# Xjh-UCAS/TAM-TR

Measured on AMD Instinct MI355X. Metric: images/sec fwd+bwd @640x640 bs=16/GPU, higher is better.
Workload: dtype bf16

## Files before the change

include/tamtr_hip.h:

```cpp
#ifndef TAMTR_HIP_H
#define TAMTR_HIP_H

#include <stdint.h>

#ifdef __cplusplus
extern "C" {
#endif

#define TAMTR_F32 0
#define TAMTR_BF16 1

#define TAMTR_OK 0
#define TAMTR_EINVAL (-1)
#define TAMTR_EUNSUP (-2)
#define TAMTR_ELAUNCH (-3)

int tamtr_abi_version(void);

int tamtr_maxsigmoid_gate_fwd(const void* x, const float* gk, const float* bias, const void* v, void* out, float* aw,
                              int32_t* arg, int B, int nh, int hc, int HW, int T, float scale, int dtype, void* stream);

int tamtr_maxsigmoid_gate_bwd(const void* dout, const void* x, const float* gk, const void* v, const float* aw,
                              const int32_t* arg, void* dx, void* dv, float* dlogit, int B, int nh, int hc, int HW, int T,
                              float scale, int dtype, void* stream);
int tamtr_maxsigmoid_gate_cl_fwd(const void* e, long long ld_e, const float* mean_rstd_e, const float* gamma_e, const float* beta_e,
                                 const void* v, const float* mean_rstd_v, const float* gamma_v, const float* beta_v, const float* gk,
                                 const float* bias, void* out, float* aw, int32_t* arg, int B, int nh, int hc, int HW, int T, float scale,
                                 int dtype, void* stream);

int tamtr_conv3x3_tiles(int B, int H, int W);
int tamtr_conv3x3_pack_weight(const void* w, void* wpk, int C1, int C2, int dtype, void* stream);
int tamtr_conv3x3_cl_stats_fwd(const void* x, long long ld_x, const void* wpk, void* y, float* running_mean, float* running_var,
                               float* mean_rstd, float* partials, int B, int H, int W, int C1, int C2, float eps, float momentum,
                               void* stream);
int tamtr_bn_finalize(const float* partials, float* mean_rstd, float* running_mean, float* running_var, int C, int S, float eps,
                      float momentum, void* stream);

int tamtr_msdeform_attn_fwd(const void* value, const int32_t* shapes_host, const float* loc, const float* aw, void* out,
                            int B, int L, int M, int D, int Q, int nl, int P, int dtype, void* stream);

int tamtr_msdeform_attn_bwd(const void* gout, const void* value, const int32_t* shapes_host, const float* loc,
                            const float* aw, float* gvalue, float* gloc, float* gaw, int B, int L, int M, int D, int Q,
                            int nl, int P, int dtype, void* stream);

int tamtr_msdeform_attn_bwd_sorted(const void* gout, const void* value, const int32_t* shapes_host, const float* loc,
                                   const float* aw, void* gvalue, float* gloc, float* gaw, float* colw, int B, int L, int M,
                                   int D, int Q, int nl, int P, long long ldg, int dtype, void* stream);

int tamtr_contrastive_logits_fwd(const void* x, const float* w, const float* logit_scale, const float* bias, float* logits,
                                 float* xinv, float* winv, int B, int Q, int K, int C, int dtype, void* stream);

int tamtr_contrastive_bwd_slabs(int Q);
int tamtr_contrastive_logits_bwd(const float* g, const void* x, const float* w, const float* logit_scale, const float* xinv,
                                 const float* winv, void* dx, float* dwhat, int B, int Q, int K, int C, int dtype,
                                 void* stream);

int tamtr_linear_bf16(const void* X, const void* W, const float* bias, void* Y, int M, int N, int K, void* stream);

int tamtr_selfattn_fwd(const void* q, const void* k, const void* v, const uint32_t* mask_bits, void* o, float* lse, int B,
                       int Q, int nh, int dh, int ldq, int ldk, int ldv, int dtype, void* stream);
int tamtr_selfattn_bwd(const void* go, const void* q, const void* k, const void* v, const void* o, const float* lse,
                       const uint32_t* mask_bits, void* gq, void* gk, void* gv, float* delta_ws, int B, int Q, int nh, int dh,
                       int ldq, int ldk, int ldv, int dtype, void* stream);

int tamtr_selective_scan_chunk(void);
int tamtr_selective_scan_fwd(const float* u, const float* delta, const float* A, const float* Bm, const float* Cm,
                             const float* D, const float* dbias, float* y, float* hstate, int B, int K, int Dk, int N, int L,
                             int xmode, void* stream);
int tamtr_selective_scan_bwd_slabs(int Dk);
int tamtr_selective_scan_row_sums(void);
int tamtr_selective_scan_bwd(const float* gy, const float* u, const float* delta, const float* A, const float* Bm,
                             const float* Cm, const float* D, const float* dbias, const float* hstate, float* gu,
                             float* gdelta, float* grow, float* gB, float* gC, float* ws, int B, int K, int Dk, int N, int L,
                             int xmode, void* stream);

int tamtr_selective_scan_dtproj_fwd(const void* u, const float* dtr, const float* Wdt, const float* A, const float* Bm,
                                    const float* Cm, const float* D, const float* dbias, void* y, float* hstate, int B, int K,
                                    int Dk, int N, int R, int L, int xmode, int planes_bf16, void* stream);
int tamtr_selective_scan_dtproj_bwd(const void* gy, const void* u, const float* dtr, const float* Wdt, const float* A,
                                    const float* Bm, const float* Cm, const float* D, const float* dbias, const float* hstate,
                                    void* gu, void* gdelta_ws, float* gdtr, float* grow, float* gB, float* gC, float* ws, int B,
                                    int K, int Dk, int N, int R, int L, int xmode, int bf16_flags, void* stream);

int tamtr_lsap_assign(const float* cost, const int32_t* group_sizes_host, int bs, int nq, int G, int64_t* batch_idx,
                      int64_t* query_idx, int64_t* gt_idx, void* stream);

int tamtr_cpam_fwd(const void* x, const void* p, void* out, float* s2, int32_t* arg, int B, int C, int H, int W, int dtype,
                   void* stream);

int tamtr_cpam_bwd(const void* gout, const void* x, const void* p, const float* s2, const int32_t* arg, void* dx_direct,
                   void* du_ws, void* dp, int B, int C, int H, int W, int dtype, void* stream);

int tamtr_cpam_cl_fwd(const void* x, void* p, uint8_t* code, void* out, float* s2, int32_t* arg, int B, int C, int H, int W, int dtype, void* stream);
int tamtr_cpam_cl_bwd(const void* gout, const void* x, const void* p, const uint8_t* code, const float* s2, const int32_t* arg, void* dxd_ws,
                      void* du_ws, void* dp_ws, void* dx, int B, int C, int H, int W, int dtype, void* stream);

int tamtr_dwconv_silu_cross_fwd(const void* x, long long x_pixel_stride, const float* weight, const float* bias, void* u2, int B,
                                int D, int H, int W, int dtype, int plane_dtype, void* stream);
int tamtr_dwconv_tiles(int H, int W);
int tamtr_dwconv_silu_cross_bwd(const void* g2, const void* x, long long x_pixel_stride, const float* weight, const float* bias,
                                void* gx, long long gx_pixel_stride, float* ws, int B, int D, int H, int W, int dtype, int plane_dtype,
                                void* stream);

int tamtr_cross_merge_fwd(const void* y4, float* ymT, int B, int D, int H, int W, int plane_dtype, void* stream);
int tamtr_cross_merge_bwd(const float* gymT, void* g2, int B, int D, int H, int W, int plane_dtype, void* stream);

int tamtr_ln_gate_blocks(long long ntok);
int tamtr_ln_gate_fwd(const float* x, const void* xz, long long xz_token_stride, const float* gamma, const float* beta, void* out,
                      float* stats, long long ntok, int D, float eps, int dtype, void* stream);
int tamtr_ln_gate_bwd(const void* gout, const float* x, const void* xz, long long xz_token_stride, const float* gamma,
                      const float* beta, const float* stats, float* gx, void* gxz, float* partials, long long ntok, int D, int dtype,
                      void* stream);

int tamtr_sum_n(const void* const* src, int n, void* out, long long n_elems, int dtype, void* stream);

int tamtr_colsum_blocks(long long M);
int tamtr_colsum_bf16(const void* X, float* partial, long long M, int N, void* stream);
int tamtr_slab_sum_rows(const void* in, float* out, int R, long long C, int dtype, void* stream);
int tamtr_fold_add(const float* g4, const void* m0, const void* m1, float* out, int B, long long n, int dtype, void* stream);

int tamtr_layernorm_fwd(const void* x, const float* gamma, const float* beta, void* out, float* stats, long long ntok, int D,
                        float eps, int dtype, void* stream);
int tamtr_layernorm_bwd(const void* gout, const void* x, const float* gamma, const float* stats, void* gx, float* partials,
                        long long ntok, int D, int dtype, void* stream);

int tamtr_bn_slices(int B, int HW);
int tamtr_bn_act_fwd(const void* x, const float* gamma, const float* beta, float* running_mean, float* running_var, void* y,
                     float* mean_rstd, float* partials, int B, int C, int HW, float eps, float momentum, int act, int dtype, void* stream);
int tamtr_bn_act_bwd(const void* gy, const void* x, const float* gamma, const float* beta, const float* mean_rstd, void* gx,
                     float* ggamma, float* gbeta, float* partials, int B, int C, int HW, int act, int dtype, void* stream);

int tamtr_bncl_blocks(long long N, int C, int dtype);
int tamtr_bncl_act_fwd(const void* x, const float* gamma, const float* beta, float* running_mean, float* running_var, const void* residual,
                       void* y, float* mean_rstd, float* partials, long long N, int C, float eps, float momentum, int act, int dtype,
                       void* stream);
int tamtr_bncl_stats(const void* x, float* running_mean, float* running_var, float* mean_rstd, float* partials, long long N, int C, float eps,
                     float momentum, int dtype, void* stream);
int tamtr_bncl2_act_fwd(const void* x1, const float* gamma1, const float* beta1, float* running_mean1, float* running_var1, const void* x2,
                        const float* gamma2, const float* beta2, float* running_mean2, float* running_var2, void* y, float* mean_rstd,
                        float* partials, long long N, int C, float eps, float momentum, int act, int dtype, void* stream);
int tamtr_bncl2_act_bwd(const void* gy, long long ldgy, const void* x1, const void* x2, const float* gamma1, const float* beta1,
                        const float* gamma2, const float* beta2, const float* mean_rstd, void* gx1, void* gx2, float* ggamma1, float* gbeta1,
                        float* ggamma2, float* gbeta2, float* partials, long long N, int C, int act, int dtype, void* stream);
int tamtr_bncl_act_bwd(const void* gy, long long ldgy, const void* x, const float* gamma, const float* beta, const float* mean_rstd,
                       void* gx, float* ggamma, float* gbeta, float* partials, long long N, int C, int act, int dtype, void* stream);

int tamtr_relayout(const void* src, void* dst, int B, int C, int HW, int ld, int to_nhwc, int dtype, void* stream);
int tamtr_resample2(const void* src, void* dst, int B, int H, int W, int C, int mode, int dtype, void* stream);
int tamtr_copy_rows(const void* src, long long lds, void* dst, long long ldd, long long N, int C, int dtype, void* stream);
int tamtr_cat_rows(const void* const* src, const long long* lds, const int* C, int n, void* dst, long long ldd, long long N, int dtype,
                   void* stream);

int tamtr_maxpool_out(int n, int k, int s, int p);
int tamtr_maxpool_fwd(const void* x, void* y, uint8_t* code, int B, int C, int H, int W, int k, int s, int p, int nhwc, int dtype,
                      void* stream);
int tamtr_maxpool_bwd(const void* gy, const uint8_t* code, const void* addend, void* gx, int B, int C, int H, int W, int k, int s, int p, int nhwc, int dtype,
                      void* stream);

int tamtr_img_augment_u8(const uint8_t* src, const double* inv_affine, const uint8_t* luts, const int32_t* flags, float* out, int B,
                         int SH, int SW, int H, int W, int border, void* stream);

int tamtr_optim_chunk(void);
int tamtr_optim_step(const void* const* p, const void* const* m, const void* const* v, const void* const* e, const void* const* shadow, float* step,
                     const long long* numel,
                     const unsigned char* group, const int* chunk_tensor, const long long* chunk_off, const void* const* grads, int ntensors,
                     int nchunks, float* partial, float* normcoef, const float* lr, const float* wd, int ngroups, float beta1, float beta2, float eps,
                     float max_norm, float ema_decay, int do_ema, void* stream);

int tamtr_xproj_dw_slices(int L);
int tamtr_xproj_fwd(const void* u2, const void* wcat, float* dtr, float* Bs, float* Cs, int B, int D, int L, int R, int plane_dtype, void* stream);
int tamtr_xproj_bwd_dx(const void* gu, const float* gdtr, const float* gB, const float* gC, const void* wT, void* gu2, int B, int D, int L, int R,
                       int plane_dtype, void* stream);
int tamtr_xproj_bwd_dw(const void* u2, const float* gdtr, const float* gB, const float* gC, float* part, int B, int D, int L, int R, int plane_dtype,
                       void* stream);

int tamtr_detr_blocks(int rows_per_layer);
int tamtr_detr_layers_fwd(const float* pb, const float* ps, const float* gt_bboxes, const long long* gt_cls, const long long* li, const long long* bi,
                          const long long* si, const long long* gi, int Lr, int B, int nq, int nc, int n, long long* tgt, float* score, float* pair_l1,
                          float* pair_riou, float* partial, float g_class, float g_bbox, float g_giou, float* out, void* stream);
int tamtr_detr_layers_bwd(const float* pb, const float* ps, const float* gt_bboxes, const long long* li, const long long* bi, const long long* si,
                          const long long* gi, const long long* tgt, const float* score, const float* up, int Lr, int B, int nq, int nc, int n,
                          float g_class, float g_bbox, float g_giou, float* gpb, float* gps, void* stream);
int tamtr_detr_match_cost(const float* ps, const float* pb, const float* gt_bboxes, const long long* gt_cls, long long rows, int nc, int G, float g_class,
                          float g_bbox, float g_giou, float alpha, float gamma, float* C, void* stream);

int tamtr_bncl_act_seg_fwd(const void* x, const float* gamma, const float* beta, float* running_mean, float* running_var, void* y, long long seg_rows,
                           long long seg_pitch, float* mean_rstd, float* partials, long long N, int C, float eps, float momentum, int act, int dtype,
                           void* stream);
int tamtr_bncl_act_seg_bwd(const void* gy, long long seg_rows, long long seg_pitch, const void* x, const float* gamma, const float* beta,
                           const float* mean_rstd, void* gx, float* ggamma, float* gbeta, float* partials, long long N, int C, int act, int dtype,
                           void* stream);

int tamtr_box_refine_fwd(const float* delta, const float* ref, float* out, long long n, void* stream);
int tamtr_box_refine_bwd(const float* gout, const float* out, const float* ref, float* gdelta, float* gref, long long n, void* stream);

int tamtr_graph_capture_census(void* stream, int* counts, int n_types);

int tamtr_detect_postprocess(const void* preds, int dtype, int B, int nq, int nd, const int32_t* orig_hw, float conf, float iou,
                             int single_cls, float max_wh, const int32_t* classes, int n_classes, float* out, int32_t* keep,
                             int32_t* counts, void* stream);

int tamtr_val_postprocess_match(const void* preds, int dtype, int B, int nq, int nd, float imgsz, float conf, float iou, int single_cls,
                                float max_wh, const float* lab_cls, const float* lab_box, const int32_t* lab_off, int M, const float* scale,
                                float* predn, uint8_t* correct, int32_t* counts, void* stream);

#ifdef __cplusplus
}
#endif
#endif
```

tam-tr_amd/_lib.py:

```python
import ctypes
import os
from ctypes import c_float, c_int, c_longlong, c_void_p

_HERE = os.path.dirname(os.path.abspath(__file__))
LIB_PATH = os.environ.get('TAMTR_HIP_LIB') or os.path.join(_HERE, 'csrc', 'libtamtr_hip.so')
ABI_VERSION = 36

F32, BF16 = 0, 1
_ERR = {-1: 'TAMTR_EINVAL (bad argument)', -2: 'TAMTR_EUNSUP (shape/dtype outside what the kernels are built for)',
        -3: 'TAMTR_ELAUNCH (HIP launch error)'}


class TamtrHipError(RuntimeError):
    pass


_P, _I, _F, _LL = c_void_p, c_int, c_float, c_longlong
_SIGS = {
    'tamtr_abi_version': [],
    'tamtr_maxsigmoid_gate_fwd': [_P, _P, _P, _P, _P, _P, _P, _I, _I, _I, _I, _I, _F, _I, _P],
    'tamtr_maxsigmoid_gate_bwd': [_P, _P, _P, _P, _P, _P, _P, _P, _P, _I, _I, _I, _I, _I, _F, _I, _P],
    'tamtr_msdeform_attn_fwd': [_P, _P, _P, _P, _P, _I, _I, _I, _I, _I, _I, _I, _I, _P],
    'tamtr_msdeform_attn_bwd': [_P, _P, _P, _P, _P, _P, _P, _P, _I, _I, _I, _I, _I, _I, _I, _I, _P],
    'tamtr_msdeform_attn_bwd_sorted': [_P, _P, _P, _P, _P, _P, _P, _P, _P, _I, _I, _I, _I, _I, _I, _I, _LL, _I, _P],
    'tamtr_contrastive_logits_fwd': [_P, _P, _P, _P, _P, _P, _P, _I, _I, _I, _I, _I, _P],
    'tamtr_contrastive_logits_bwd': [_P, _P, _P, _P, _P, _P, _P, _P, _I, _I, _I, _I, _I, _P],
    'tamtr_contrastive_bwd_slabs': [_I],
    'tamtr_linear_bf16': [_P, _P, _P, _P, _I, _I, _I, _P],
    'tamtr_selfattn_fwd': [_P, _P, _P, _P, _P, _P, _I, _I, _I, _I, _I, _I, _I, _I, _P],
    'tamtr_selfattn_bwd': [_P] * 11 + [_I, _I, _I, _I, _I, _I, _I, _I, _P],
    'tamtr_selective_scan_chunk': [],
    'tamtr_selective_scan_fwd': [_P, _P, _P, _P, _P, _P, _P, _P, _P, _I, _I, _I, _I, _I, _I, _P],
    'tamtr_selective_scan_bwd_slabs': [_I],
    'tamtr_selective_scan_row_sums': [],
    'tamtr_selective_scan_bwd': [_P] * 15 + [_I, _I, _I, _I, _I, _I, _P],
    'tamtr_selective_scan_dtproj_fwd': [_P] * 10 + [_I] * 8 + [_P],
    'tamtr_selective_scan_dtproj_bwd': [_P] * 17 + [_I] * 8 + [_P],
    'tamtr_lsap_assign': [_P, _P, _I, _I, _I, _P, _P, _P, _P],
    'tamtr_img_augment_u8': [_P, _P, _P, _P, _P, _I, _I, _I, _I, _I, _I, _P],
    'tamtr_cpam_fwd': [_P, _P, _P, _P, _P, _I, _I, _I, _I, _I, _P],
    'tamtr_cpam_cl_fwd': [_P, _P, _P, _P, _P, _P, _I, _I, _I, _I, _I, _P],
    'tamtr_cpam_bwd': [_P] * 8 + [_I, _I, _I, _I, _I, _P],
    'tamtr_cpam_cl_bwd': [_P] * 10 + [_I, _I, _I, _I, _I, _P],
    'tamtr_dwconv_silu_cross_fwd': [_P, _LL, _P, _P, _P, _I, _I, _I, _I, _I, _I, _P],
    'tamtr_dwconv_tiles': [_I, _I],
    'tamtr_cross_merge_fwd': [_P, _P, _I, _I, _I, _I, _I, _P],
    'tamtr_cross_merge_bwd': [_P, _P, _I, _I, _I, _I, _I, _P],
    'tamtr_ln_gate_blocks': [_LL],
    'tamtr_bn_slices': [_I, _I],
    'tamtr_maxpool_out': [_I, _I, _I, _I],
    'tamtr_maxpool_fwd': [_P, _P, _P, _I, _I, _I, _I, _I, _I, _I, _I, _I, _P],
    'tamtr_maxpool_bwd': [_P, _P, _P, _P, _I, _I, _I, _I, _I, _I, _I, _I, _I, _P],
    'tamtr_sum_n': [_P, _I, _P, _LL, _I, _P],
    'tamtr_colsum_blocks': [_LL],
    'tamtr_colsum_bf16': [_P, _P, _LL, _I, _P],
    'tamtr_fold_add': [_P, _P, _P, _P, _I, _LL, _I, _P],
    'tamtr_slab_sum_rows': [_P, _P, _I, _LL, _I, _P],
    'tamtr_graph_capture_census': [_P, _P, _I],
    'tamtr_box_refine_fwd': [_P, _P, _P, _LL, _P],
    'tamtr_box_refine_bwd': [_P, _P, _P, _P, _P, _LL, _P],
    'tamtr_bncl_act_seg_fwd': [_P, _P, _P, _P, _P, _P, _LL, _LL, _P, _P, _LL, _I, _F, _F, _I, _I, _P],
    'tamtr_bncl_act_seg_bwd': [_P, _LL, _LL, _P, _P, _P, _P, _P, _P, _P, _P, _LL, _I, _I, _I, _P],
    'tamtr_detr_blocks': [_I],
    'tamtr_detr_layers_fwd': [_P] * 8 + [_I] * 5 + [_P] * 5 + [_F, _F, _F, _P, _P],
    'tamtr_detr_layers_bwd': [_P] * 10 + [_I] * 5 + [_F, _F, _F, _P, _P, _P],
    'tamtr_detr_match_cost': [_P, _P, _P, _P, _LL, _I, _I, _F, _F, _F, _F, _F, _P, _P],
    'tamtr_xproj_dw_slices': [_I],
    'tamtr_xproj_fwd': [_P, _P, _P, _P, _P, _I, _I, _I, _I, _I, _P],
    'tamtr_xproj_bwd_dx': [_P, _P, _P, _P, _P, _P, _I, _I, _I, _I, _I, _P],
    'tamtr_xproj_bwd_dw': [_P, _P, _P, _P, _P, _I, _I, _I, _I, _I, _P],
    'tamtr_optim_chunk': [],
    'tamtr_optim_step': [_P] * 11 + [_I, _I, _P, _P, _P, _P, _I, _F, _F, _F, _F, _F, _I, _P],
    'tamtr_resample2': [_P, _P, _I, _I, _I, _I, _I, _I, _P],
    'tamtr_cat_rows': [_P, _P, _P, _I, _P, _LL, _LL, _I, _P],
    'tamtr_copy_rows': [_P, _LL, _P, _LL, _LL, _I, _I, _P],
    'tamtr_relayout': [_P, _P, _I, _I, _I, _I, _I, _I, _P],
    'tamtr_bncl_blocks': [_LL, _I, _I],
    'tamtr_bncl_act_fwd': [_P, _P, _P, _P, _P, _P, _P, _P, _P, _LL, _I, _F, _F, _I, _I, _P],
    'tamtr_bncl_stats': [_P, _P, _P, _P, _P, _LL, _I, _F, _F, _I, _P],
    'tamtr_bn_finalize': [_P, _P, _P, _P, _I, _I, _F, _F, _P],
    'tamtr_conv3x3_tiles': [_I, _I, _I],
    'tamtr_conv3x3_pack_weight': [_P, _P, _I, _I, _I, _P],
    'tamtr_conv3x3_cl_stats_fwd': [_P, _LL, _P, _P, _P, _P, _P, _P, _I, _I, _I, _I, _I, _F, _F, _P],
    'tamtr_maxsigmoid_gate_cl_fwd': [_P, _LL, _P, _P, _P, _P, _P, _P, _P, _P, _P, _P, _P, _P, _I, _I, _I, _I, _I, _F, _I, _P],
    'tamtr_bncl2_act_fwd': [_P, _P, _P, _P, _P, _P, _P, _P, _P, _P, _P, _P, _P, _LL, _I, _F, _F, _I, _I, _P],
    'tamtr_bncl2_act_bwd': [_P, _LL, _P, _P, _P, _P, _P, _P, _P, _P, _P, _P, _P, _P, _P, _P, _LL, _I, _I, _I, _P],
    'tamtr_bncl_act_bwd': [_P, _LL, _P, _P, _P, _P, _P, _P, _P, _P, _LL, _I, _I, _I, _P],
    'tamtr_bn_act_fwd': [_P, _P, _P, _P, _P, _P, _P, _P, _I, _I, _I, _F, _F, _I, _I, _P],
    'tamtr_bn_act_bwd': [_P, _P, _P, _P, _P, _P, _P, _P, _P, _I, _I, _I, _I, _I, _P],
    'tamtr_layernorm_fwd': [_P, _P, _P, _P, _P, _LL, _I, _F, _I, _P],
    'tamtr_layernorm_bwd': [_P, _P, _P, _P, _P, _P, _LL, _I, _I, _P],
    'tamtr_ln_gate_fwd': [_P, _P, _LL, _P, _P, _P, _P, _LL, _I, _F, _I, _P],
    'tamtr_ln_gate_bwd': [_P, _P, _P, _LL, _P, _P, _P, _P, _P, _P, _LL, _I, _I, _P],
    'tamtr_dwconv_silu_cross_bwd': [_P, _P, _LL, _P, _P, _P, _LL, _P, _I, _I, _I, _I, _I, _I, _P],
    'tamtr_detect_postprocess': [_P, _I, _I, _I, _I, _P, _F, _F, _I, _F, _P, _I, _P, _P, _P, _P],
    'tamtr_val_postprocess_match': [_P, _I, _I, _I, _I, _F, _F, _F, _I, _F, _P, _P, _P, _I, _P, _P, _P, _P, _P],
}
EXPORTS = tuple(_SIGS)
_lib = None


def lib():
    global _lib
    if _lib is None:
        if not os.path.exists(LIB_PATH):
            raise TamtrHipError(f'{LIB_PATH} not found: build it with `python -c "import __graft_entry__ as g; g.build()"` '
                                '(hipcc --offload-arch=gfx950). There is no CPU fallback.')
        h = ctypes.CDLL(LIB_PATH)
        for name, args in _SIGS.items():
            fn = getattr(h, name)
            fn.argtypes = args
            fn.restype = c_int
        if h.tamtr_abi_version() != ABI_VERSION:
            raise TamtrHipError(f'libtamtr_hip.so ABI {h.tamtr_abi_version()} != expected {ABI_VERSION}: rebuild')
        _lib = h
    return _lib


def call(name, *args):
    rc = getattr(lib(), name)(*args)
    if rc != 0:
        raise TamtrHipError(f'{name} failed: {_ERR.get(rc, rc)}')


def require_gpu(*tensors):
    for t in tensors:
        if t is not None and not t.is_cuda:
            raise TamtrHipError('TAM-TR HIP ops need tensors resident on an MI355X (got a CPU tensor); there is no CPU fallback')


def dtype_code(t):
    import torch
    if t.dtype == torch.float32:
        return F32
    if t.dtype == torch.bfloat16:
        return BF16
    raise TamtrHipError(f'unsupported activation dtype {t.dtype} (float32 and bfloat16 kernels are built)')


def stream_ptr():
    import torch
    return c_void_p(torch.cuda.current_stream().cuda_stream)


def ptr(t):
    return c_void_p(t.data_ptr()) if t is not None else c_void_p(0)
```

tam-tr_amd/backbone.py:

```python
import torch
import torch.nn as nn
import torch.nn.functional as F

def _conv(conv, x):
    if x.is_cuda:
        from . import ops
        return ops.conv2d_module(conv, x)
    return conv(x)


BN_EPS, BN_MOMENTUM = 1e-3, 0.03


def batchnorm(c):
    return nn.BatchNorm2d(c, eps=BN_EPS, momentum=BN_MOMENTUM)


def fold_bn(conv, bn):
    fused = nn.Conv2d(conv.in_channels, conv.out_channels, conv.kernel_size, conv.stride, conv.padding, conv.dilation, conv.groups,
                      bias=True).requires_grad_(False).to(conv.weight.device)
    with torch.no_grad():
        scale = bn.weight.div(torch.sqrt(bn.eps + bn.running_var))
        fused.weight.copy_((scale[:, None] * conv.weight.reshape(conv.out_channels, -1)).view(fused.weight.shape))
        b = torch.zeros(conv.out_channels, device=conv.weight.device) if conv.bias is None else conv.bias
        fused.bias.copy_(scale * b + (bn.bias - bn.weight.mul(bn.running_mean).div(torch.sqrt(bn.running_var + bn.eps))))
    return fused


class Conv(nn.Module):

    def __init__(self, c1, c2, k=1, s=1, p=None, g=1, d=1, act=True):
        super().__init__()
        if p is None:
            p = (d * (k - 1) + 1) // 2 if d > 1 else k // 2
        self.conv = nn.Conv2d(c1, c2, k, s, p, dilation=d, groups=g, bias=False)
        self.bn = batchnorm(c2)
        self.act = nn.SiLU() if act is True else act if isinstance(act, nn.Module) else nn.Identity()

    def fuse(self):
        if 'bn' in self._modules:
            self.conv = fold_bn(self.conv, self.bn)
            del self.bn

    def fusable(self, y):
        return ('bn' in self._modules and y.is_cuda and self.bn.training and self.bn.affine and type(self.act) in (nn.SiLU, nn.Identity)
                and y.dtype in (torch.bfloat16, torch.float32))

    def forward(self, x, residual=None):
        return self.post(_conv(self.conv, x), residual)

    def post(self, y, residual=None):
        if 'bn' not in self._modules:
            y = self.act(y)
            return y if residual is None else y + residual
        if self.fusable(y):
            from . import ops
            if ops.is_cl(y) and ops.bn_cl_ok(y.shape[1], y.dtype):
                B, C, H, W = y.shape
                res = None
                if residual is not None and ops.is_cl(residual) and residual.shape == y.shape:
                    res, residual = residual.permute(0, 2, 3, 1).reshape(B * H * W, C), None
                o = ops.bn_act(y.permute(0, 2, 3, 1).reshape(B * H * W, C), self.bn, isinstance(self.act, nn.SiLU), res)
                o = o.view(B, H, W, C).permute(0, 3, 1, 2)
                return o if residual is None else o + residual
            y = ops.bn_act(y, self.bn, isinstance(self.act, nn.SiLU))
        else:
            y = self.act(self.bn(y))
        return y if residual is None else y + residual


class RepConvN(nn.Module):

    def __init__(self, c1, c2, k=3, s=1, p=1, g=1, d=1, act=True, bn=False, deploy=False):
        super().__init__()
        assert k == 3 and p == 1
        self.conv1 = Conv(c1, c2, 3, s, p=1, g=g, act=False)
        self.conv2 = Conv(c1, c2, 1, s, p=0, g=g, act=False)
        self.act = nn.SiLU() if act is True else act if isinstance(act, nn.Module) else nn.Identity()

    def forward(self, x):
        if 'conv' in self._modules:
            return self.act(self.conv(x))
        c1, c2 = self.conv1, self.conv2
        if x.is_cuda and type(self.act) in (nn.SiLU, nn.Identity) and 'bn' in c1._modules and 'bn' in c2._modules:
            from . import ops
            y1, y2 = c1.conv(x), _conv(c2.conv, x)
            if (c1.fusable(y1) and c2.fusable(y2) and ops.is_cl(y1) and ops.is_cl(y2) and ops.bn_cl_ok(y1.shape[1], y1.dtype)
                    and c1.bn.track_running_stats and c2.bn.track_running_stats and c1.bn.eps == c2.bn.eps and c1.bn.momentum == c2.bn.momentum):
                B, C, H, W = y1.shape
                o = ops.bn2_act(y1.permute(0, 2, 3, 1).reshape(B * H * W, C), c1.bn, y2.permute(0, 2, 3, 1).reshape(B * H * W, C), c2.bn,
                                isinstance(self.act, nn.SiLU))
                return o.view(B, H, W, C).permute(0, 3, 1, 2)
            return self.act(c1.post(y1) + c2.post(y2))
        return self.act(self.conv1(x) + self.conv2(x))

    @staticmethod
    def _branch(branch):
        bn = branch.bn
        std = (bn.running_var + bn.eps).sqrt()
        return branch.conv.weight * (bn.weight / std).reshape(-1, 1, 1, 1), bn.bias - bn.running_mean * bn.weight / std

    def switch_to_deploy(self):
        if 'conv' in self._modules:
            return
        with torch.no_grad():
            (k3, b3), (k1, b1) = self._branch(self.conv1), self._branch(self.conv2)
            c = self.conv1.conv
            self.conv = nn.Conv2d(c.in_channels, c.out_channels, c.kernel_size, c.stride, c.padding, c.dilation, c.groups,
                                  bias=True).requires_grad_(False).to(c.weight.device)
            self.conv.weight.copy_(k3 + F.pad(k1, [1, 1, 1, 1]))
            self.conv.bias.copy_(b3 + b1)
        del self.conv1, self.conv2


class RepNBottleneck(nn.Module):
    def __init__(self, c1, c2, shortcut=True, g=1, k=(3, 3), e=0.5):
        super().__init__()
        c_ = int(c2 * e)
        self.cv1 = RepConvN(c1, c_, k[0], 1)
        self.cv2 = Conv(c_, c2, k[1], 1, g=g)
        self.add = shortcut and c1 == c2

    def forward(self, x):
        if self.add:
            return self.cv2(self.cv1(x), residual=x)
        return self.cv2(self.cv1(x))


class RepNCSP(nn.Module):
    def __init__(self, c1, c2, n=1, shortcut=True, g=1, e=0.5):
        super().__init__()
        c_ = int(c2 * e)
        self.cv1, self.cv2 = Conv(c1, c_, 1, 1), Conv(c1, c_, 1, 1)
        self.cv3 = Conv(2 * c_, c2, 1)
        self.m = nn.Sequential(*(RepNBottleneck(c_, c_, shortcut, g, e=1.0) for _ in range(n)))

    def forward(self, x):
        from . import ops
        return self.cv3(ops.cat_channels((self.m(self.cv1(x)), self.cv2(x))))


class RepNCSPELAN4(nn.Module):

    def __init__(self, c1, c2, c3, c4, c5=1):
        super().__init__()
        self.c = c3 // 2
        self.cv1 = Conv(c1, c3, 1, 1)
        self.cv2 = nn.Sequential(RepNCSP(c3 // 2, c4, c5), Conv(c4, c4, 3, 1))
        self.cv3 = nn.Sequential(RepNCSP(c4, c4, c5), Conv(c4, c4, 3, 1))
        self.cv4 = Conv(c3 + 2 * c4, c2, 1, 1)

    def branches(self, x):
        from . import ops
        y = list(ops.chunk2_channels(self.cv1(x)))
        y.append(self.cv2(ops.pack_channels(y[-1])))
        y.append(self.cv3(y[-1]))
        return y

    def forward(self, x):
        from . import ops
        return self.cv4(ops.cat_channels(self.branches(x)))


class SPPELAN(nn.Module):
    def __init__(self, c1, c2, c3):
        super().__init__()
        self.c = c3
        self.cv1 = Conv(c1, c3, 1, 1)
        self.cv5 = Conv(4 * c3, c2, 1, 1)

    def forward(self, x):
        from . import ops
        y = [self.cv1(x)]
        for _ in range(3):
            y.append(ops.max_pool2d(y[-1], 5, 1, 2) if y[-1].is_cuda else F.max_pool2d(y[-1], 5, 1, 2))
        return self.cv5(ops.cat_channels(y))


class CPAM(nn.Module):

    def __init__(self, c1, c2=None):
        super().__init__()

    def forward(self, x):
        from . import ops
        return ops.cpam(x)


class Upsample(nn.Upsample):

    def forward(self, x):
        if self.mode == 'nearest' and x.dim() == 4 and self.size is None and isinstance(self.scale_factor, (int, float)):
            if x.is_cuda and self.scale_factor in (0.5, 2.0):
                from . import ops
                y = ops.resample2(x, self.scale_factor == 2.0)
                if y is not None:
                    return y
            if self.scale_factor == 0.5 and x.shape[2] % 2 == 0 and x.shape[3] % 2 == 0:
                return x[..., ::2, ::2]
            if self.scale_factor == 2.0:
                B, C, H, W = x.shape
                if not x.is_contiguous() and x.is_contiguous(memory_format=torch.channels_last):
                    y = x.permute(0, 2, 3, 1)[:, :, None, :, None, :].expand(B, H, 2, W, 2, C).reshape(B, 2 * H, 2 * W, C)
                    return y.permute(0, 3, 1, 2)
                return x[:, :, :, None, :, None].expand(B, C, H, 2, W, 2).reshape(B, C, 2 * H, 2 * W)
        return super().forward(x)


class Concat(nn.Module):
    def __init__(self, dimension=1):
        super().__init__()
        self.d = dimension

    def forward(self, x):
        if self.d == 1:
            from . import ops
            return ops.cat_channels(x)
        return torch.cat(x, self.d)
```

tam-tr_amd/csrc/bn.hip:

```cpp
#include "common.h"

namespace {

constexpr int BN_THREADS = 256;
constexpr int BN_EPT = 16;
constexpr int BN_SLICE = BN_THREADS * BN_EPT;

template <typename T>
__device__ __forceinline__ void ld_slice(const T* __restrict__ p, int n, bool vec, float (&v)[BN_EPT], int (&cnt)) {
  const int base = threadIdx.x * BN_EPT;
  cnt = max(0, min(BN_EPT, n - base));
  if (vec && cnt == BN_EPT) {
#pragma unroll
    for (int q = 0; q < BN_EPT / 4; ++q) {
      float o[4];
      Elt<T>::ld4(p + base + 4 * q, o);
      v[4 * q] = o[0]; v[4 * q + 1] = o[1]; v[4 * q + 2] = o[2]; v[4 * q + 3] = o[3];
    }
  } else {
#pragma unroll
    for (int i = 0; i < BN_EPT; ++i) v[i] = i < cnt ? Elt<T>::ld(p + base + i) : 0.f;
  }
}

// ... 143 lines not shown
  const int n = min(BN_SLICE, HW - s * BN_SLICE);
  const size_t off = ((size_t)b * C + c) * HW + (size_t)s * BN_SLICE;
  const float mean = mean_rstd[2 * c], rstd = mean_rstd[2 * c + 1], g = gamma[c], be = beta[c];
  float xv[BN_EPT], gv[BN_EPT];
  int cnt;
  ld_slice<T>(x + off, n, vec, xv, cnt);
  ld_slice<T>(gy + off, n, vec, gv, cnt);
  float s1 = 0.f, s2 = 0.f;
#pragma unroll
  for (int i = 0; i < BN_EPT; ++i) {
    if (i < cnt) {
      const float xh = (xv[i] - mean) * rstd;
      const float dz = gv[i] * act_bwd(fmaf(xh, g, be), act);
      s1 += dz;
      s2 = fmaf(dz, xh, s2);
    }
  }
  s1 = block_sum(s1, s_red);
  s2 = block_sum(s2, s_red);
  if (threadIdx.x == 0) {
    float* o = part + ((size_t)c * S + (size_t)b * gridDim.x + s) * 2;
    o[0] = s1; o[1] = s2;
  }
}

template <typename T>
__global__ __launch_bounds__(BN_THREADS) void bn_bwd_apply_kernel(const T* __restrict__ gy, const T* __restrict__ x,
                                                                   const float* __restrict__ mean_rstd, const float* __restrict__ gamma,
                                                                   const float* __restrict__ beta, const float* __restrict__ part,
                                                                   T* __restrict__ gx, float* __restrict__ ggamma, float* __restrict__ gbeta,
                                                                   int C, int HW, int vec, int act, float inv_count) {
  __shared__ float s_red[BN_THREADS / WAVE];
  const int s = blockIdx.x, c = blockIdx.y, b = blockIdx.z, S = gridDim.x * gridDim.z;
  float p1 = 0.f, p2 = 0.f;
  for (int i = threadIdx.x; i < S; i += BN_THREADS) { p1 += part[((size_t)c * S + i) * 2]; p2 += part[((size_t)c * S + i) * 2 + 1]; }
  const float sum_dz = block_sum(p1, s_red), sum_dzx = block_sum(p2, s_red);
  if (s == 0 && b == 0 && threadIdx.x == 0) { ggamma[c] = sum_dzx; gbeta[c] = sum_dz; }
  const int n = min(BN_SLICE, HW - s * BN_SLICE);
  const size_t off = ((size_t)b * C + c) * HW + (size_t)s * BN_SLICE;
  const float mean = mean_rstd[2 * c], rstd = mean_rstd[2 * c + 1], g = gamma[c], be = beta[c];
  const float k1 = sum_dz * inv_count, k2 = sum_dzx * inv_count, gr = g * rstd;
  const int base = threadIdx.x * BN_EPT;
  const int cnt = max(0, min(BN_EPT, n - base));
  if (vec && cnt == BN_EPT) {
#pragma unroll
    for (int q = 0; q < BN_EPT / 4; ++q) {
      float xv[4], gv[4], o[4];
      Elt<T>::ld4(x + off + base + 4 * q, xv);
      Elt<T>::ld4(gy + off + base + 4 * q, gv);
#pragma unroll
      for (int i = 0; i < 4; ++i) {
        const float xh = (xv[i] - mean) * rstd;
        const float dz = gv[i] * act_bwd(fmaf(xh, g, be), act);
        o[i] = gr * (dz - k1 - xh * k2);
      }
      Elt<T>::st4(gx + off + base + 4 * q, o);
    }
  } else {
    for (int i = 0; i < cnt; ++i) {
      const float xh = (Elt<T>::ld(x + off + base + i) - mean) * rstd;
      const float dz = Elt<T>::ld(gy + off + base + i) * act_bwd(fmaf(xh, g, be), act);
      Elt<T>::st(gx + off + base + i, gr * (dz - k1 - xh * k2));
    }
  }
}

template <typename T, int V>
struct Vec;
template <>
struct Vec<float, 4> {
  static __device__ __forceinline__ void ld(const float* p, float (&o)[4]) { Elt<float>::ld4(p, o); }
  static __device__ __forceinline__ void st(float* p, const float (&v)[4]) { Elt<float>::st4(p, v); }
};
template <>
struct Vec<bf16_t, 4> {
  static __device__ __forceinline__ void ld(const bf16_t* p, float (&o)[4]) { Elt<bf16_t>::ld4(p, o); }
  static __device__ __forceinline__ void st(bf16_t* p, const float (&v)[4]) { Elt<bf16_t>::st4(p, v); }
};
template <>
struct Vec<bf16_t, 8> {
  static __device__ __forceinline__ void ld(const bf16_t* p, float (&o)[8]) {
    const uint4 t = *reinterpret_cast<const uint4*>(p);
    const uint32_t w[4] = {t.x, t.y, t.z, t.w};
#pragma unroll
    for (int i = 0; i < 4; ++i) { o[2 * i] = __uint_as_float(w[i] << 16); o[2 * i + 1] = __uint_as_float(w[i] & 0xffff0000u); }
  }
  static __device__ __forceinline__ void st(bf16_t* p, const float (&v)[8]) {
    uint32_t w[4];
#pragma unroll
    for (int i = 0; i < 4; ++i) w[i] = (uint32_t)f2bf(v[2 * i]) | ((uint32_t)f2bf(v[2 * i + 1]) << 16);
    *reinterpret_cast<uint4*>(p) = make_uint4(w[0], w[1], w[2], w[3]);
  }
};

constexpr int CL_UNROLL = 4;

template <int W>
__device__ __forceinline__ void fold_row_lanes(const float (&mine)[W], float* s_acc, float* s_col, int cg) {
#pragma unroll
  for (int j = 0; j < W; ++j) s_acc[threadIdx.x * W + j] = mine[j];
  __syncthreads();
  const int rl = BN_THREADS / cg;
  for (int o = threadIdx.x; o < cg * W; o += BN_THREADS) {
    const int g = o / W, j = o % W;
    float a = 0.f;
    for (int q = 0; q < rl; ++q) a += s_acc[(q * cg + g) * W + j];
    s_col[o] = a;
  }
  __syncthreads();
}

struct Seg { unsigned rows; size_t pitch; };
__device__ __forceinline__ size_t seg_addr(size_t e, int C, int cshift, size_t ld, Seg sg) {
  const size_t row = e >> cshift, col = e & (size_t)(C - 1);
  if (!sg.rows) return row * ld + col;
  const unsigned img = (unsigned)row / sg.rows;
  return (size_t)img * sg.pitch + ((unsigned)row - img * sg.rows) * ld + col;
}

template <typename T, int V>
__global__ __launch_bounds__(BN_THREADS) void bncl_stats_kernel(const T* __restrict__ x, float* __restrict__ part, size_t total, int C,
                                                                 int iters) {
  __shared__ float s_acc[BN_THREADS * 2 * V];
  __shared__ float s_col[2 * 1024];
  const size_t piece = (size_t)BN_THREADS * V, start = (size_t)blockIdx.x * iters * piece, end = min(total, start + iters * piece);
  const int cg = C / V, g = threadIdx.x % cg, S = gridDim.x;
  const T* home = x + start + (size_t)g * V;
  float k[V], acc[2 * V];
  Vec<T, V>::ld(home, k);
#pragma unroll
  for (int j = 0; j < 2 * V; ++j) acc[j] = 0.f;
  const size_t e0 = start + (size_t)threadIdx.x * V;
  for (int it = 0; it < iters; it += CL_UNROLL) {
    float v[CL_UNROLL][V];
#pragma unroll
    for (int u = 0; u < CL_UNROLL; ++u) {
      const size_t e = e0 + (size_t)(it + u) * piece;
      Vec<T, V>::ld(e < end ? x + e : home, v[u]);
    }
#pragma unroll
    for (int u = 0; u < CL_UNROLL; ++u)
#pragma unroll
      for (int j = 0; j < V; ++j) { const float d = v[u][j] - k[j]; acc[j] += d; acc[V + j] = fmaf(d, d, acc[V + j]); }
  }
  fold_row_lanes<2 * V>(acc, s_acc, s_col, cg);
  const float n = (float)((end - start) / C);
  for (int c = threadIdx.x; c < C; c += BN_THREADS) {
    const float s1 = s_col[(c / V) * 2 * V + c % V], s2 = s_col[(c / V) * 2 * V + V + c % V], m = s1 / n;
    float* o = part + ((size_t)c * S + blockIdx.x) * 3;
    o[0] = n; o[1] = Elt<T>::ld(x + start + c) + m; o[2] = s2 - s1 * m;
  }
}

template <typename T, int V>
__global__ __launch_bounds__(BN_THREADS) void bncl_apply_kernel(const T* __restrict__ x, const float* __restrict__ mean_rstd,
                                                                 const float* __restrict__ gamma, const float* __restrict__ beta,
                                                                 const T* __restrict__ res, T* __restrict__ y, size_t total, int C, int iters,
                                                                 int act, Seg ysg = Seg{0, 0}, int cshift = 0) {
  const size_t piece = (size_t)BN_THREADS * V, start = (size_t)blockIdx.x * iters * piece, end = min(total, start + iters * piece);
  const int c0 = (threadIdx.x % (C / V)) * V;
  const size_t home = start + c0;
  float mean[V], a[V], be[V];
#pragma unroll
  for (int j = 0; j < V; ++j) { mean[j] = mean_rstd[2 * (c0 + j)]; a[j] = mean_rstd[2 * (c0 + j) + 1] * gamma[c0 + j]; be[j] = beta[c0 + j]; }
  const size_t e0 = start + (size_t)threadIdx.x * V;
  for (int it = 0; it < iters; it += CL_UNROLL) {
    float v[CL_UNROLL][V];
#pragma unroll
    for (int u = 0; u < CL_UNROLL; ++u) {
      const size_t e = e0 + (size_t)(it + u) * piece;
      Vec<T, V>::ld(x + (e < end ? e : home), v[u]);
    }
#pragma unroll
    for (int u = 0; u < CL_UNROLL; ++u) {
      const size_t e = e0 + (size_t)(it + u) * piece;
#pragma unroll
      for (int j = 0; j < V; ++j) v[u][j] = act_fwd(fmaf(v[u][j] - mean[j], a[j], be[j]), act);
      if (res && e < end) {
        float r[V];
        Vec<T, V>::ld(res + e, r);
#pragma unroll
        for (int j = 0; j < V; ++j) v[u][j] += r[j];
      }
      if (e < end) Vec<T, V>::st(y + (ysg.rows ? seg_addr(e, C, cshift, (size_t)C, ysg) : e), v[u]);
    }
  }
}

template <typename T, int V>
__global__ __launch_bounds__(BN_THREADS) void bncl2_apply_kernel(const T* __restrict__ x1, const T* __restrict__ x2,
                                                                  const float* __restrict__ mr1, const float* __restrict__ mr2,
                                                                  const float* __restrict__ g1, const float* __restrict__ b1,
                                                                  const float* __restrict__ g2, const float* __restrict__ b2,
                                                                  T* __restrict__ y, size_t total, int C, int iters, int act) {
  const size_t piece = (size_t)BN_THREADS * V, start = (size_t)blockIdx.x * iters * piece, end = min(total, start + iters * piece);
  const int c0 = (threadIdx.x % (C / V)) * V;
  const size_t home = start + c0;
  float m1[V], a1[V], m2[V], a2[V], be[V];
#pragma unroll
  for (int j = 0; j < V; ++j) {
    m1[j] = mr1[2 * (c0 + j)]; a1[j] = mr1[2 * (c0 + j) + 1] * g1[c0 + j];
    m2[j] = mr2[2 * (c0 + j)]; a2[j] = mr2[2 * (c0 + j) + 1] * g2[c0 + j];
    be[j] = b1[c0 + j] + b2[c0 + j];
  }
  const size_t e0 = start + (size_t)threadIdx.x * V;
  for (int it = 0; it < iters; it += CL_UNROLL) {
    float v[CL_UNROLL][V], w[CL_UNROLL][V];
#pragma unroll
    for (int u = 0; u < CL_UNROLL; ++u) {
      const size_t e = e0 + (size_t)(it + u) * piece, ee = e < end ? e : home;
      Vec<T, V>::ld(x1 + ee, v[u]);
      Vec<T, V>::ld(x2 + ee, w[u]);
    }
#pragma unroll
    for (int u = 0; u < CL_UNROLL; ++u) {
      const size_t e = e0 + (size_t)(it + u) * piece;
#pragma unroll
      for (int j = 0; j < V; ++j) v[u][j] = act_fwd(fmaf(w[u][j] - m2[j], a2[j], fmaf(v[u][j] - m1[j], a1[j], be[j])), act);
      if (e < end) Vec<T, V>::st(y + e, v[u]);
    }
  }
}

template <typename T, int V>
__global__ __launch_bounds__(BN_THREADS) void bncl2_bwd_reduce_kernel(const T* __restrict__ gy, const T* __restrict__ x1, const T* __restrict__ x2,
                                                                       const float* __restrict__ mr1, const float* __restrict__ mr2,
                                                                       const float* __restrict__ g1, const float* __restrict__ b1,
                                                                       const float* __restrict__ g2, const float* __restrict__ b2,
                                                                       float* __restrict__ part, size_t total, int C, int iters, int act,
                                                                       size_t ldgy, int cshift) {
  __shared__ float s_acc[BN_THREADS * 3 * V];
  __shared__ float s_col[3 * 1024];
  const size_t piece = (size_t)BN_THREADS * V, start = (size_t)blockIdx.x * iters * piece, end = min(total, start + iters * piece);
  const int cg = C / V, c0 = (threadIdx.x % cg) * V, S = gridDim.x;
  const size_t home = start + c0;
  float m1[V], r1[V], m2[V], r2[V], ga1[V], ga2[V], be[V], acc[3 * V];
#pragma unroll
  for (int j = 0; j < V; ++j) {
    m1[j] = mr1[2 * (c0 + j)]; r1[j] = mr1[2 * (c0 + j) + 1]; m2[j] = mr2[2 * (c0 + j)]; r2[j] = mr2[2 * (c0 + j) + 1];
    ga1[j] = g1[c0 + j]; ga2[j] = g2[c0 + j]; be[j] = b1[c0 + j] + b2[c0 + j];
    acc[j] = 0.f; acc[V + j] = 0.f; acc[2 * V + j] = 0.f;
  }
  const size_t e0 = start + (size_t)threadIdx.x * V;
  for (int it = 0; it < iters; it += CL_UNROLL) {
    float xa[CL_UNROLL][V], xb[CL_UNROLL][V], gv[CL_UNROLL][V];
#pragma unroll
    for (int u = 0; u < CL_UNROLL; ++u) {
      const size_t e = e0 + (size_t)(it + u) * piece, ee = e < end ? e : home;
      Vec<T, V>::ld(x1 + ee, xa[u]);
      Vec<T, V>::ld(x2 + ee, xb[u]);
      Vec<T, V>::ld(gy + (ee >> cshift) * ldgy + (ee & (size_t)(C - 1)), gv[u]);
    }
#pragma unroll
    for (int u = 0; u < CL_UNROLL; ++u) {
      const float live = e0 + (size_t)(it + u) * piece < end ? 1.f : 0.f;
#pragma unroll
      for (int j = 0; j < V; ++j) {
        const float h1 = (xa[u][j] - m1[j]) * r1[j], h2 = (xb[u][j] - m2[j]) * r2[j];
        const float dz = live * gv[u][j] * act_bwd(fmaf(h2, ga2[j], fmaf(h1, ga1[j], be[j])), act);
        acc[j] += dz; acc[V + j] = fmaf(dz, h1, acc[V + j]); acc[2 * V + j] = fmaf(dz, h2, acc[2 * V + j]);
      }
    }
  }
  fold_row_lanes<3 * V>(acc, s_acc, s_col, cg);
  for (int c = threadIdx.x; c < C; c += BN_THREADS) {
    float* o = part + ((size_t)c * S + blockIdx.x) * 3;
    o[0] = s_col[(c / V) * 3 * V + c % V]; o[1] = s_col[(c / V) * 3 * V + V + c % V]; o[2] = s_col[(c / V) * 3 * V + 2 * V + c % V];
  }
}

__global__ __launch_bounds__(BN_THREADS) void bncl2_sum_kernel(const float* __restrict__ part, float* __restrict__ sums, float* __restrict__ gg1,
                                                                float* __restrict__ gb1, float* __restrict__ gg2, float* __restrict__ gb2, int S) {
  __shared__ float s_red[BN_THREADS / WAVE];
  const int c = blockIdx.x;
  float a = 0.f, b = 0.f, d = 0.f;
  for (int s = threadIdx.x; s < S; s += BN_THREADS) {
    const float* p = part + ((size_t)c * S + s) * 3;
    a += p[0]; b += p[1]; d += p[2];
  }
  a = block_sum(a, s_red); b = block_sum(b, s_red); d = block_sum(d, s_red);
  if (threadIdx.x == 0) { sums[3 * c] = a; sums[3 * c + 1] = b; sums[3 * c + 2] = d; gb1[c] = a; gb2[c] = a; gg1[c] = b; gg2[c] = d; }
}

template <typename T, int V>
__global__ __launch_bounds__(BN_THREADS) void bncl2_bwd_apply_kernel(const T* __restrict__ gy, const T* __restrict__ x1, const T* __restrict__ x2,
                                                                      const float* __restrict__ mr1, const float* __restrict__ mr2,
                                                                      const float* __restrict__ g1, const float* __restrict__ b1,
                                                                      const float* __restrict__ g2, const float* __restrict__ b2,
                                                                      const float* __restrict__ sums, T* __restrict__ gx1, T* __restrict__ gx2,
                                                                      size_t total, int C, int iters, int act, float inv_count, size_t ldgy,
                                                                      int cshift) {
  const size_t piece = (size_t)BN_THREADS * V, start = (size_t)blockIdx.x * iters * piece, end = min(total, start + iters * piece);
  const int c0 = (threadIdx.x % (C / V)) * V;
  const size_t home = start + c0;
  float m1[V], r1[V], m2[V], r2[V], ga1[V], ga2[V], be[V], k1[V], k2[V], k3[V];
#pragma unroll
  for (int j = 0; j < V; ++j) {
    m1[j] = mr1[2 * (c0 + j)]; r1[j] = mr1[2 * (c0 + j) + 1]; m2[j] = mr2[2 * (c0 + j)]; r2[j] = mr2[2 * (c0 + j) + 1];
    ga1[j] = g1[c0 + j]; ga2[j] = g2[c0 + j]; be[j] = b1[c0 + j] + b2[c0 + j];
    k1[j] = sums[3 * (c0 + j)] * inv_count; k2[j] = sums[3 * (c0 + j) + 1] * inv_count; k3[j] = sums[3 * (c0 + j) + 2] * inv_count;
  }
  const size_t e0 = start + (size_t)threadIdx.x * V;
  for (int it = 0; it < iters; it += CL_UNROLL / 2) {
    float xa[CL_UNROLL / 2][V], xb[CL_UNROLL / 2][V], gv[CL_UNROLL / 2][V];
#pragma unroll
    for (int u = 0; u < CL_UNROLL / 2; ++u) {
      const size_t e = e0 + (size_t)(it + u) * piece, ee = e < end ? e : home;
      Vec<T, V>::ld(x1 + ee, xa[u]);
      Vec<T, V>::ld(x2 + ee, xb[u]);
      Vec<T, V>::ld(gy + (ee >> cshift) * ldgy + (ee & (size_t)(C - 1)), gv[u]);
    }
#pragma unroll
    for (int u = 0; u < CL_UNROLL / 2; ++u) {
      const size_t e = e0 + (size_t)(it + u) * piece;
#pragma unroll
      for (int j = 0; j < V; ++j) {
        const float h1 = (xa[u][j] - m1[j]) * r1[j], h2 = (xb[u][j] - m2[j]) * r2[j];
        const float dz = gv[u][j] * act_bwd(fmaf(h2, ga2[j], fmaf(h1, ga1[j], be[j])), act);
        xa[u][j] = ga1[j] * r1[j] * (dz - k1[j] - h1 * k2[j]);
        xb[u][j] = ga2[j] * r2[j] * (dz - k1[j] - h2 * k3[j]);
      }
      if (e < end) { Vec<T, V>::st(gx1 + e, xa[u]); Vec<T, V>::st(gx2 + e, xb[u]); }
    }
  }
}

template <typename T, int V>
__global__ __launch_bounds__(BN_THREADS) void bncl_bwd_reduce_kernel(const T* __restrict__ gy, const T* __restrict__ x,
                                                                      const float* __restrict__ mean_rstd, const float* __restrict__ gamma,
                                                                      const float* __restrict__ beta, float* __restrict__ part, size_t total,
                                                                      int C, int iters, int act, size_t ldgy, int cshift, Seg gsg = Seg{0, 0}) {
  __shared__ float s_acc[BN_THREADS * 2 * V];
  __shared__ float s_col[2 * 1024];
  const size_t piece = (size_t)BN_THREADS * V, start = (size_t)blockIdx.x * iters * piece, end = min(total, start + iters * piece);
  const int cg = C / V, c0 = (threadIdx.x % cg) * V, S = gridDim.x;
  const size_t home = start + c0;
  float mean[V], rstd[V], gm[V], be[V], acc[2 * V];
#pragma unroll
  for (int j = 0; j < V; ++j) {
    mean[j] = mean_rstd[2 * (c0 + j)]; rstd[j] = mean_rstd[2 * (c0 + j) + 1]; gm[j] = gamma[c0 + j]; be[j] = beta[c0 + j];
    acc[j] = 0.f; acc[V + j] = 0.f;
  }
  const size_t e0 = start + (size_t)threadIdx.x * V;
  for (int it = 0; it < iters; it += CL_UNROLL) {
    float xv[CL_UNROLL][V], gv[CL_UNROLL][V];
#pragma unroll
    for (int u = 0; u < CL_UNROLL; ++u) {
      const size_t e = e0 + (size_t)(it + u) * piece, ee = e < end ? e : home;
      Vec<T, V>::ld(x + ee, xv[u]);
      Vec<T, V>::ld(gy + seg_addr(ee, C, cshift, ldgy, gsg), gv[u]);
    }
#pragma unroll
    for (int u = 0; u < CL_UNROLL; ++u) {
      const float live = e0 + (size_t)(it + u) * piece < end ? 1.f : 0.f;
#pragma unroll
      for (int j = 0; j < V; ++j) {
        const float xh = (xv[u][j] - mean[j]) * rstd[j];
        const float dz = live * gv[u][j] * act_bwd(fmaf(xh, gm[j], be[j]), act);
        acc[j] += dz; acc[V + j] = fmaf(dz, xh, acc[V + j]);
      }
    }
  }
  fold_row_lanes<2 * V>(acc, s_acc, s_col, cg);
  for (int c = threadIdx.x; c < C; c += BN_THREADS) {
    float* o = part + ((size_t)c * S + blockIdx.x) * 2;
    o[0] = s_col[(c / V) * 2 * V + c % V]; o[1] = s_col[(c / V) * 2 * V + V + c % V];
  }
}

__global__ __launch_bounds__(BN_THREADS) void bncl_sum_kernel(const float* __restrict__ part, float* __restrict__ sums, float* __restrict__ ggamma,
                                                               float* __restrict__ gbeta, int S) {
  __shared__ float s_red[BN_THREADS / WAVE];
  const int c = blockIdx.x;
  float a = 0.f, b = 0.f;
  for (int s = threadIdx.x; s < S; s += BN_THREADS) { a += part[((size_t)c * S + s) * 2]; b += part[((size_t)c * S + s) * 2 + 1]; }
  a = block_sum(a, s_red); b = block_sum(b, s_red);
  if (threadIdx.x == 0) { sums[2 * c] = a; sums[2 * c + 1] = b; gbeta[c] = a; ggamma[c] = b; }
}

template <typename T, int V>
__global__ __launch_bounds__(BN_THREADS) void bncl_bwd_apply_kernel(const T* __restrict__ gy, const T* __restrict__ x,
                                                                     const float* __restrict__ mean_rstd, const float* __restrict__ gamma,
                                                                     const float* __restrict__ beta, const float* __restrict__ sums,
                                                                     T* __restrict__ gx, size_t total, int C, int iters, int act,
                                                                     float inv_count, size_t ldgy, int cshift, Seg gsg = Seg{0, 0}) {
  const size_t piece = (size_t)BN_THREADS * V, start = (size_t)blockIdx.x * iters * piece, end = min(total, start + iters * piece);
  const int c0 = (threadIdx.x % (C / V)) * V;
  const size_t home = start + c0;
  float mean[V], rstd[V], gm[V], be[V], k1[V], k2[V];
#pragma unroll
  for (int j = 0; j < V; ++j) {
    mean[j] = mean_rstd[2 * (c0 + j)]; rstd[j] = mean_rstd[2 * (c0 + j) + 1]; gm[j] = gamma[c0 + j]; be[j] = beta[c0 + j];
    k1[j] = sums[2 * (c0 + j)] * inv_count; k2[j] = sums[2 * (c0 + j) + 1] * inv_count;
  }
  const size_t e0 = start + (size_t)threadIdx.x * V;
  for (int it = 0; it < iters; it += CL_UNROLL) {
    float xv[CL_UNROLL][V], gv[CL_UNROLL][V];
#pragma unroll
    for (int u = 0; u < CL_UNROLL; ++u) {
      const size_t e = e0 + (size_t)(it + u) * piece, ee = e < end ? e : home;
      Vec<T, V>::ld(x + ee, xv[u]);
      Vec<T, V>::ld(gy + seg_addr(ee, C, cshift, ldgy, gsg), gv[u]);
    }
#pragma unroll
    for (int u = 0; u < CL_UNROLL; ++u) {
      const size_t e = e0 + (size_t)(it + u) * piece;
#pragma unroll
      for (int j = 0; j < V; ++j) {
        const float xh = (xv[u][j] - mean[j]) * rstd[j];
        const float dz = gv[u][j] * act_bwd(fmaf(xh, gm[j], be[j]), act);
        gv[u][j] = gm[j] * rstd[j] * (dz - k1[j] - xh * k2[j]);
      }
      if (e < end) Vec<T, V>::st(gx + e, gv[u]);
    }
  }
}

}

extern "C" int tamtr_bn_slices(int B, int HW) { return B * ((HW + BN_SLICE - 1) / BN_SLICE); }

static int bn_check(const void* a, const void* b, int B, int C, int HW, int dtype, int act) {
  if (!a || !b || B <= 0 || C <= 0 || HW <= 0) return TAMTR_EINVAL;
  if ((dtype != TAMTR_F32 && dtype != TAMTR_BF16) || (act != 0 && act != 1)) return TAMTR_EINVAL;
  if (B > 65535 || C > 65535) return TAMTR_EUNSUP;
  return TAMTR_OK;
}
static int bn_vec(const void* p, const void* q, int HW, int dtype) {
  const int e = dtype == TAMTR_F32 ? 4 : 2;
  return HW % 4 == 0 && ((uintptr_t)p % (4 * e)) == 0 && (!q || ((uintptr_t)q % (4 * e)) == 0);
}

extern "C" int tamtr_bn_act_fwd(const void* x, const float* gamma, const float* beta, float* running_mean, float* running_var, void* y,
                                float* mean_rstd, float* partials, int B, int C, int HW, float eps, float momentum, int act, int dtype,
                                void* stream) {
  const int rc = bn_check(x, y, B, C, HW, dtype, act);
  if (rc) return rc;
  if (!gamma || !beta || !mean_rstd || !partials) return TAMTR_EINVAL;
  const int sh = (HW + BN_SLICE - 1) / BN_SLICE, vec = bn_vec(x, y, HW, dtype);
  const dim3 grid(sh, C, B);
  hipStream_t s = (hipStream_t)stream;
  if (dtype == TAMTR_F32) hipLaunchKernelGGL(bn_stats_kernel<float>, grid, dim3(BN_THREADS), 0, s, (const float*)x, partials, C, HW, vec);
  else hipLaunchKernelGGL(bn_stats_kernel<bf16_t>, grid, dim3(BN_THREADS), 0, s, (const bf16_t*)x, partials, C, HW, vec);
  if (dtype == TAMTR_F32)
    hipLaunchKernelGGL(bn_apply_kernel<float>, grid, dim3(BN_THREADS), 0, s, (const float*)x, partials, mean_rstd, running_mean, running_var,
                       gamma, beta, (float*)y, C, HW, vec, act, eps, momentum);
  else
    hipLaunchKernelGGL(bn_apply_kernel<bf16_t>, grid, dim3(BN_THREADS), 0, s, (const bf16_t*)x, partials, mean_rstd, running_mean,
                       running_var, gamma, beta, (bf16_t*)y, C, HW, vec, act, eps, momentum);
  return tamtr_launch_status();
}

extern "C" int tamtr_bn_act_bwd(const void* gy, const void* x, const float* gamma, const float* beta, const float* mean_rstd, void* gx,
                                float* ggamma, float* gbeta, float* partials, int B, int C, int HW, int act, int dtype, void* stream) {
  const int rc = bn_check(gy, x, B, C, HW, dtype, act);
  if (rc) return rc;
  if (!gamma || !beta || !mean_rstd || !gx || !ggamma || !gbeta || !partials) return TAMTR_EINVAL;
  const int sh = (HW + BN_SLICE - 1) / BN_SLICE, vec = bn_vec(x, gy, HW, dtype) && bn_vec(gx, nullptr, HW, dtype);
  const dim3 grid(sh, C, B);
  hipStream_t s = (hipStream_t)stream;
  const float inv = 1.f / ((float)B * (float)HW);
  if (dtype == TAMTR_F32) {
    hipLaunchKernelGGL(bn_bwd_reduce_kernel<float>, grid, dim3(BN_THREADS), 0, s, (const float*)gy, (const float*)x, mean_rstd, gamma, beta,
                       partials, C, HW, vec, act);
    hipLaunchKernelGGL(bn_bwd_apply_kernel<float>, grid, dim3(BN_THREADS), 0, s, (const float*)gy, (const float*)x, mean_rstd, gamma, beta,
                       partials, (float*)gx, ggamma, gbeta, C, HW, vec, act, inv);
  } else {
    hipLaunchKernelGGL(bn_bwd_reduce_kernel<bf16_t>, grid, dim3(BN_THREADS), 0, s, (const bf16_t*)gy, (const bf16_t*)x, mean_rstd, gamma,
                       beta, partials, C, HW, vec, act);
    hipLaunchKernelGGL(bn_bwd_apply_kernel<bf16_t>, grid, dim3(BN_THREADS), 0, s, (const bf16_t*)gy, (const bf16_t*)x, mean_rstd, gamma,
                       beta, partials, (bf16_t*)gx, ggamma, gbeta, C, HW, vec, act, inv);
  }
  return tamtr_launch_status();
}

static int bncl_vec(int C, int dtype) { return dtype == TAMTR_BF16 && C % 8 == 0 ? 8 : 4; }
static int bncl_iters(long long N, int C, int dtype) {
  const long long piece = (long long)BN_THREADS * bncl_vec(C, dtype), total = N * C;
  const long long it = (total / piece / 1024 + CL_UNROLL - 1) / CL_UNROLL * CL_UNROLL;
  return (int)(it < 4 ? 4 : it > 64 ? 64 : it);
}
extern "C" int tamtr_bncl_blocks(long long N, int C, int dtype) {
  if (N <= 0 || C <= 0) return 0;
  const long long chunk = (long long)bncl_iters(N, C, dtype) * BN_THREADS * bncl_vec(C, dtype);
  return (int)((N * C + chunk - 1) / chunk);
}

static int bncl_check(const void* a, const void* b, long long N, int C, int dtype, int act) {
  if (!a || !b || N <= 0 || C <= 0) return TAMTR_EINVAL;
  if ((dtype != TAMTR_F32 && dtype != TAMTR_BF16) || (act != 0 && act != 1)) return TAMTR_EINVAL;
  const int cg = C / bncl_vec(C, dtype);
  if (C % 4 || C > 1024 || cg > BN_THREADS || (BN_THREADS % cg) || N > 2000000000LL / C) return TAMTR_EUNSUP;
  if (((uintptr_t)a | (uintptr_t)b) % 16) return TAMTR_EUNSUP;
  return TAMTR_OK;
}

static int bncl_act_fwd_impl(const void* x, const float* gamma, const float* beta, float* running_mean, float* running_var,
                             const void* residual, void* y, float* mean_rstd, float* partials, long long N, int C, float eps,
                             float momentum, int act, int dtype, void* stream, Seg ysg, int cshift) {
  const int rc = bncl_check(x, y, N, C, dtype, act);
  if (rc) return rc;
  if (!gamma || !beta || !mean_rstd || !partials) return TAMTR_EINVAL;
  if (residual && (uintptr_t)residual % 16) return TAMTR_EUNSUP;
  const int S = tamtr_bncl_blocks(N, C, dtype), V = bncl_vec(C, dtype), iters = bncl_iters(N, C, dtype);
  const size_t total = (size_t)N * C;
  hipStream_t s = (hipStream_t)stream;
  if (dtype == TAMTR_F32) hipLaunchKernelGGL((bncl_stats_kernel<float, 4>), dim3(S), dim3(BN_THREADS), 0, s, (const float*)x, partials, total, C, iters);
  else if (V == 8) hipLaunchKernelGGL((bncl_stats_kernel<bf16_t, 8>), dim3(S), dim3(BN_THREADS), 0, s, (const bf16_t*)x, partials, total, C, iters);
  else hipLaunchKernelGGL((bncl_stats_kernel<bf16_t, 4>), dim3(S), dim3(BN_THREADS), 0, s, (const bf16_t*)x, partials, total, C, iters);
  hipLaunchKernelGGL(bn_finalize_kernel, dim3(C), dim3(BN_THREADS), 0, s, partials, mean_rstd, running_mean, running_var, S, eps, momentum);
  if (dtype == TAMTR_F32)
    hipLaunchKernelGGL((bncl_apply_kernel<float, 4>), dim3(S), dim3(BN_THREADS), 0, s, (const float*)x, mean_rstd, gamma, beta, (const float*)residual, (float*)y, total, C, iters, act, ysg, cshift);
  else if (V == 8)
    hipLaunchKernelGGL((bncl_apply_kernel<bf16_t, 8>), dim3(S), dim3(BN_THREADS), 0, s, (const bf16_t*)x, mean_rstd, gamma, beta, (const bf16_t*)residual, (bf16_t*)y, total, C, iters, act, ysg, cshift);
  else
    hipLaunchKernelGGL((bncl_apply_kernel<bf16_t, 4>), dim3(S), dim3(BN_THREADS), 0, s, (const bf16_t*)x, mean_rstd, gamma, beta, (const bf16_t*)residual, (bf16_t*)y, total, C, iters, act, ysg, cshift);
  return tamtr_launch_status();
}

extern "C" int tamtr_bncl_act_fwd(const void* x, const float* gamma, const float* beta, float* running_mean, float* running_var,
                                  const void* residual, void* y, float* mean_rstd, float* partials, long long N, int C, float eps,
                                  float momentum, int act, int dtype, void* stream) {
  return bncl_act_fwd_impl(x, gamma, beta, running_mean, running_var, residual, y, mean_rstd, partials, N, C, eps, momentum, act, dtype, stream,
                           Seg{0, 0}, 0);
}

extern "C" int tamtr_bncl_act_seg_fwd(const void* x, const float* gamma, const float* beta, float* running_mean, float* running_var, void* y,
                                      long long seg_rows, long long seg_pitch, float* mean_rstd, float* partials, long long N, int C, float eps,
                                      float momentum, int act, int dtype, void* stream) {
  if (seg_rows <= 0 || N % seg_rows || seg_pitch < seg_rows * C || seg_pitch % 8 || (C & (C - 1)) || seg_rows > 0x7fffffffLL) return TAMTR_EUNSUP;
  int cshift = 0;
  while ((1 << cshift) < C) ++cshift;
  return bncl_act_fwd_impl(x, gamma, beta, running_mean, running_var, nullptr, y, mean_rstd, partials, N, C, eps, momentum, act, dtype, stream,
                           Seg{(unsigned)seg_rows, (size_t)seg_pitch}, cshift);
}

static int bncl_act_bwd_impl(const void* gy, long long ldgy, const void* x, const float* gamma, const float* beta,
                             const float* mean_rstd, void* gx, float* ggamma, float* gbeta, float* partials, long long N, int C, int act,
                             int dtype, void* stream, Seg gsg) {
  const int rc = bncl_check(gy, x, N, C, dtype, act);
  if (rc) return rc;
  if (ldgy < C || ldgy % bncl_vec(C, dtype) || (C & (C - 1))) return TAMTR_EUNSUP;
  int cshift = 0;
  while ((1 << cshift) < C) ++cshift;
  if (!gamma || !beta || !mean_rstd || !gx || !ggamma || !gbeta || !partials || (uintptr_t)gx % 16) return TAMTR_EINVAL;
  const int S = tamtr_bncl_blocks(N, C, dtype), V = bncl_vec(C, dtype), iters = bncl_iters(N, C, dtype);
  const size_t total = (size_t)N * C;
  hipStream_t s = (hipStream_t)stream;
  float* sums = partials + (size_t)C * S * 2;
  const float inv = 1.f / (float)N;
  if (dtype == TAMTR_F32)
    hipLaunchKernelGGL((bncl_bwd_reduce_kernel<float, 4>), dim3(S), dim3(BN_THREADS), 0, s, (const float*)gy, (const float*)x, mean_rstd, gamma, beta, partials, total, C, iters, act, (size_t)ldgy, cshift, gsg);
  else if (V == 8)
    hipLaunchKernelGGL((bncl_bwd_reduce_kernel<bf16_t, 8>), dim3(S), dim3(BN_THREADS), 0, s, (const bf16_t*)gy, (const bf16_t*)x, mean_rstd, gamma, beta, partials, total, C, iters, act, (size_t)ldgy, cshift, gsg);
  else
    hipLaunchKernelGGL((bncl_bwd_reduce_kernel<bf16_t, 4>), dim3(S), dim3(BN_THREADS), 0, s, (const bf16_t*)gy, (const bf16_t*)x, mean_rstd, gamma, beta, partials, total, C, iters, act, (size_t)ldgy, cshift, gsg);
  hipLaunchKernelGGL(bncl_sum_kernel, dim3(C), dim3(BN_THREADS), 0, s, partials, sums, ggamma, gbeta, S);
  if (dtype == TAMTR_F32)
    hipLaunchKernelGGL((bncl_bwd_apply_kernel<float, 4>), dim3(S), dim3(BN_THREADS), 0, s, (const float*)gy, (const float*)x, mean_rstd, gamma, beta, sums, (float*)gx, total, C, iters, act, inv, (size_t)ldgy, cshift, gsg);
  else if (V == 8)
    hipLaunchKernelGGL((bncl_bwd_apply_kernel<bf16_t, 8>), dim3(S), dim3(BN_THREADS), 0, s, (const bf16_t*)gy, (const bf16_t*)x, mean_rstd, gamma, beta, sums, (bf16_t*)gx, total, C, iters, act, inv, (size_t)ldgy, cshift, gsg);
  else
    hipLaunchKernelGGL((bncl_bwd_apply_kernel<bf16_t, 4>), dim3(S), dim3(BN_THREADS), 0, s, (const bf16_t*)gy, (const bf16_t*)x, mean_rstd, gamma, beta, sums, (bf16_t*)gx, total, C, iters, act, inv, (size_t)ldgy, cshift, gsg);
  return tamtr_launch_status();
}

extern "C" int tamtr_bncl_act_bwd(const void* gy, long long ldgy, const void* x, const float* gamma, const float* beta,
                                  const float* mean_rstd, void* gx, float* ggamma, float* gbeta, float* partials, long long N, int C, int act,
                                  int dtype, void* stream) {
  return bncl_act_bwd_impl(gy, ldgy, x, gamma, beta, mean_rstd, gx, ggamma, gbeta, partials, N, C, act, dtype, stream, Seg{0, 0});
}

extern "C" int tamtr_bncl_act_seg_bwd(const void* gy, long long seg_rows, long long seg_pitch, const void* x, const float* gamma, const float* beta,
                                      const float* mean_rstd, void* gx, float* ggamma, float* gbeta, float* partials, long long N, int C, int act,
                                      int dtype, void* stream) {
  if (seg_rows <= 0 || N % seg_rows || seg_pitch < seg_rows * C || seg_pitch % 8 || seg_rows > 0x7fffffffLL) return TAMTR_EUNSUP;
  return bncl_act_bwd_impl(gy, C, x, gamma, beta, mean_rstd, gx, ggamma, gbeta, partials, N, C, act, dtype, stream,
                           Seg{(unsigned)seg_rows, (size_t)seg_pitch});
}

extern "C" int tamtr_bncl2_act_fwd(const void* x1, const float* gamma1, const float* beta1, float* running_mean1, float* running_var1,
                                   const void* x2, const float* gamma2, const float* beta2, float* running_mean2, float* running_var2,
                                   void* y, float* mean_rstd, float* partials, long long N, int C, float eps, float momentum, int act,
                                   int dtype, void* stream) {
  int rc = bncl_check(x1, y, N, C, dtype, act);
  if (!rc) rc = bncl_check(x2, y, N, C, dtype, act);
  if (rc) return rc;
  if (!gamma1 || !beta1 || !gamma2 || !beta2 || !mean_rstd || !partials) return TAMTR_EINVAL;
  const int S = tamtr_bncl_blocks(N, C, dtype), V = bncl_vec(C, dtype), iters = bncl_iters(N, C, dtype);
  const size_t total = (size_t)N * C;
  hipStream_t s = (hipStream_t)stream;
  float* mr2 = mean_rstd + 2 * (size_t)C;
  float* part2 = partials + (size_t)C * S * 3;
#define STATS(T, VV, X, P) hipLaunchKernelGGL((bncl_stats_kernel<T, VV>), dim3(S), dim3(BN_THREADS), 0, s, (const T*)X, P, total, C, iters)
#define APPLY(T, VV)                                                                                                                   \
  hipLaunchKernelGGL((bncl2_apply_kernel<T, VV>), dim3(S), dim3(BN_THREADS), 0, s, (const T*)x1, (const T*)x2, mean_rstd, mr2, gamma1, beta1, \
                     gamma2, beta2, (T*)y, total, C, iters, act)
  if (dtype == TAMTR_F32) { STATS(float, 4, x1, partials); STATS(float, 4, x2, part2); }
  else if (V == 8) { STATS(bf16_t, 8, x1, partials); STATS(bf16_t, 8, x2, part2); }
  else { STATS(bf16_t, 4, x1, partials); STATS(bf16_t, 4, x2, part2); }
  hipLaunchKernelGGL(bn_finalize_kernel, dim3(C), dim3(BN_THREADS), 0, s, partials, mean_rstd, running_mean1, running_var1, S, eps, momentum);
  hipLaunchKernelGGL(bn_finalize_kernel, dim3(C), dim3(BN_THREADS), 0, s, part2, mr2, running_mean2, running_var2, S, eps, momentum);
  if (dtype == TAMTR_F32) APPLY(float, 4); else if (V == 8) APPLY(bf16_t, 8); else APPLY(bf16_t, 4);
#undef STATS
#undef APPLY
  return tamtr_launch_status();
}

extern "C" int tamtr_bncl2_act_bwd(const void* gy, long long ldgy, const void* x1, const void* x2, const float* gamma1, const float* beta1,
                                   const float* gamma2, const float* beta2, const float* mean_rstd, void* gx1, void* gx2, float* ggamma1,
                                   float* gbeta1, float* ggamma2, float* gbeta2, float* partials, long long N, int C, int act, int dtype,
                                   void* stream) {
  int rc = bncl_check(gy, x1, N, C, dtype, act);
  if (!rc) rc = bncl_check(x2, gx1, N, C, dtype, act);
  if (rc) return rc;
  if (!gamma1 || !beta1 || !gamma2 || !beta2 || !mean_rstd || !gx2 || !ggamma1 || !gbeta1 || !ggamma2 || !gbeta2 || !partials ||
      (uintptr_t)gx2 % 16)
    return TAMTR_EINVAL;
  if (ldgy < C || ldgy % bncl_vec(C, dtype) || (C & (C - 1))) return TAMTR_EUNSUP;
  int cshift = 0;
  while ((1 << cshift) < C) ++cshift;
  const int S = tamtr_bncl_blocks(N, C, dtype), V = bncl_vec(C, dtype), iters = bncl_iters(N, C, dtype);
  const size_t total = (size_t)N * C;
  hipStream_t s = (hipStream_t)stream;
  const float* mr2 = mean_rstd + 2 * (size_t)C;
  float* sums = partials + (size_t)C * S * 3;
  const float inv = 1.f / (float)N;
#define RED(T, VV)                                                                                                                       \
  hipLaunchKernelGGL((bncl2_bwd_reduce_kernel<T, VV>), dim3(S), dim3(BN_THREADS), 0, s, (const T*)gy, (const T*)x1, (const T*)x2, mean_rstd, mr2, \
                     gamma1, beta1, gamma2, beta2, partials, total, C, iters, act, (size_t)ldgy, cshift)
#define APP(T, VV)                                                                                                                       \
  hipLaunchKernelGGL((bncl2_bwd_apply_kernel<T, VV>), dim3(S), dim3(BN_THREADS), 0, s, (const T*)gy, (const T*)x1, (const T*)x2, mean_rstd, mr2,  \
                     gamma1, beta1, gamma2, beta2, sums, (T*)gx1, (T*)gx2, total, C, iters, act, inv, (size_t)ldgy, cshift)
  if (dtype == TAMTR_F32) RED(float, 4); else if (V == 8) RED(bf16_t, 8); else RED(bf16_t, 4);
  hipLaunchKernelGGL(bncl2_sum_kernel, dim3(C), dim3(BN_THREADS), 0, s, partials, sums, ggamma1, gbeta1, ggamma2, gbeta2, S);
  if (dtype == TAMTR_F32) APP(float, 4); else if (V == 8) APP(bf16_t, 8); else APP(bf16_t, 4);
#undef RED
#undef APP
  return tamtr_launch_status();
}

extern "C" int tamtr_bn_finalize(const float* partials, float* mean_rstd, float* running_mean, float* running_var, int C, int S, float eps,
                                 float momentum, void* stream) {
  if (!partials || !mean_rstd || C <= 0 || S <= 0 || (!running_mean) != (!running_var)) return TAMTR_EINVAL;
  hipLaunchKernelGGL(bn_finalize_kernel, dim3(C), dim3(BN_THREADS), 0, (hipStream_t)stream, partials, mean_rstd, running_mean, running_var, S, eps,
                     momentum);
  return tamtr_launch_status();
}

extern "C" int tamtr_bncl_stats(const void* x, float* running_mean, float* running_var, float* mean_rstd, float* partials, long long N, int C,
                                float eps, float momentum, int dtype, void* stream) {
  const int rc = bncl_check(x, mean_rstd, N, C, dtype, 0);
  if (rc) return rc;
  if (!partials) return TAMTR_EINVAL;
  const int S = tamtr_bncl_blocks(N, C, dtype), V = bncl_vec(C, dtype), iters = bncl_iters(N, C, dtype);
  const size_t total = (size_t)N * C;
  hipStream_t s = (hipStream_t)stream;
  if (dtype == TAMTR_F32) hipLaunchKernelGGL((bncl_stats_kernel<float, 4>), dim3(S), dim3(BN_THREADS), 0, s, (const float*)x, partials, total, C, iters);
  else if (V == 8) hipLaunchKernelGGL((bncl_stats_kernel<bf16_t, 8>), dim3(S), dim3(BN_THREADS), 0, s, (const bf16_t*)x, partials, total, C, iters);
  else hipLaunchKernelGGL((bncl_stats_kernel<bf16_t, 4>), dim3(S), dim3(BN_THREADS), 0, s, (const bf16_t*)x, partials, total, C, iters);
  hipLaunchKernelGGL(bn_finalize_kernel, dim3(C), dim3(BN_THREADS), 0, s, partials, mean_rstd, running_mean, running_var, S, eps, momentum);
  return tamtr_launch_status();
}
```

tam-tr_amd/csrc/layout.hip:

```cpp
#include "common.h"

namespace {

constexpr int LT = 64;
constexpr int L_THREADS = 256;

template <typename E>
__global__ __launch_bounds__(L_THREADS) void transpose_tiles_kernel(const E* __restrict__ src, E* __restrict__ dst, int R, int S, int lds,
                                                                    int ldd, int vec) {
  __shared__ E tile[LT][LT + 4 / sizeof(E) + 1];
  const int s0 = blockIdx.x * LT, r0 = blockIdx.y * LT;
  const size_t splane = (size_t)blockIdx.z * R * lds, dplane = (size_t)blockIdx.z * S * ldd;
  const int q = (threadIdx.x % 16) * 4, row = threadIdx.x / 16;
#pragma unroll
  for (int k = 0; k < LT; k += 16) {
    const int r = r0 + row + k, s = s0 + q;
    if (r < R) {
      const E* p = src + splane + (size_t)r * lds + s;
      if (vec && s + 3 < S) {
        E v[4];
        __builtin_memcpy(v, __builtin_assume_aligned(p, 4 * sizeof(E)), 4 * sizeof(E));
#pragma unroll
        for (int i = 0; i < 4; ++i) tile[row + k][q + i] = v[i];
      } else {
        for (int i = 0; i < 4; ++i) if (s + i < S) tile[row + k][q + i] = p[i];
      }
    }
  }
  __syncthreads();
#pragma unroll
  for (int k = 0; k < LT; k += 16) {
    const int s = s0 + row + k, r = r0 + q;
    if (s < S) {
      E* p = dst + dplane + (size_t)s * ldd + r;
      if (vec && r + 3 < R) {
        E v[4];
#pragma unroll
        for (int i = 0; i < 4; ++i) v[i] = tile[q + i][row + k];
        __builtin_memcpy(__builtin_assume_aligned(p, 4 * sizeof(E)), v, 4 * sizeof(E));
      } else {
        for (int i = 0; i < 4; ++i) if (r + i < R) p[i] = tile[q + i][row + k];
      }
    }
  }
}

template <typename V>
__global__ __launch_bounds__(L_THREADS) void copy_rows_kernel(const V* __restrict__ src, V* __restrict__ dst, size_t n, int per_row, size_t lds,
                                                              size_t ldd) {
  const size_t i = (size_t)blockIdx.x * L_THREADS + threadIdx.x;
  if (i >= n) return;
  const size_t r = i / per_row, c = i % per_row;
  dst[r * ldd + c] = src[r * lds + c];
}

template <typename T, int V>
__global__ __launch_bounds__(L_THREADS) void resample2_kernel(const T* __restrict__ src, T* __restrict__ dst, int H, int W, int cv, int mode,
                                                              size_t n) {
  const size_t i = (size_t)blockIdx.x * L_THREADS + threadIdx.x;
  if (i >= n) return;
  const int c = (int)(i % cv);
  size_t r = i / cv;
  const int dw_ = (mode == 0) ? 2 * W : (mode == 2) ? W / 2 : W, dh_ = (mode == 0) ? 2 * H : (mode == 2) ? H / 2 : H;
  const int w = (int)(r % dw_); r /= dw_;
  const int h = (int)(r % dh_);
  const size_t b = r / dh_;
  typedef T vec_t __attribute__((ext_vector_type(V)));
  const vec_t* s = reinterpret_cast<const vec_t*>(src);
  vec_t* d = reinterpret_cast<vec_t*>(dst);
  if (mode == 0) {
    d[i] = s[((b * H + h / 2) * W + w / 2) * cv + c];
  } else if (mode == 2) {
    d[i] = s[((b * H + 2 * h) * W + 2 * w) * cv + c];
  } else if (mode == 3) {
    vec_t z;
#pragma unroll
    for (int u = 0; u < V; ++u) z[u] = 0;
    d[i] = ((h | w) & 1) ? z : s[((b * (H / 2) + h / 2) * (W / 2) + w / 2) * cv + c];
  } else {
    float acc[V];
#pragma unroll
    for (int u = 0; u < V; ++u) acc[u] = 0.f;
#pragma unroll
    for (int q = 0; q < 4; ++q) {
      const vec_t v = s[((b * 2 * H + 2 * h + q / 2) * (2 * W) + 2 * w + q % 2) * cv + c];
#pragma unroll
      for (int u = 0; u < V; ++u) acc[u] += sizeof(T) == 2 ? bf2f((bf16_t)v[u]) : __builtin_bit_cast(float, (uint32_t)v[u]);
    }
    vec_t o;
#pragma unroll
    for (int u = 0; u < V; ++u) o[u] = sizeof(T) == 2 ? (T)f2bf(acc[u]) : (T)__builtin_bit_cast(uint32_t, acc[u]);
    d[i] = o;
  }
}

}

extern "C" int tamtr_resample2(const void* src, void* dst, int B, int H, int W, int C, int mode, int dtype, void* stream) {
  if (!src || !dst || B <= 0 || H <= 0 || W <= 0 || C <= 0 || mode < 0 || mode > 3) return TAMTR_EINVAL;
  if (dtype != TAMTR_F32 && dtype != TAMTR_BF16) return TAMTR_EINVAL;
  const int v = dtype == TAMTR_F32 ? 4 : 8;
  if (C % v || ((uintptr_t)src | (uintptr_t)dst) % 16 || ((mode == 2 || mode == 3) && ((H | W) & 1))) return TAMTR_EUNSUP;
  const size_t rows = mode == 0 ? (size_t)B * 2 * H * 2 * W : mode == 2 ? (size_t)B * (H / 2) * (W / 2) : (size_t)B * H * W;
  const size_t n = rows * (C / v);
  const unsigned blocks = (unsigned)((n + L_THREADS - 1) / L_THREADS);
  hipStream_t s = (hipStream_t)stream;
  if (dtype == TAMTR_F32)
    hipLaunchKernelGGL((resample2_kernel<uint32_t, 4>), dim3(blocks), dim3(L_THREADS), 0, s, (const uint32_t*)src, (uint32_t*)dst, H, W, C / v, mode, n);
  else
    hipLaunchKernelGGL((resample2_kernel<uint16_t, 8>), dim3(blocks), dim3(L_THREADS), 0, s, (const uint16_t*)src, (uint16_t*)dst, H, W, C / v, mode, n);
  return tamtr_launch_status();
}

namespace {

struct CatArgs {
  const void* src[4];
  unsigned long long lds[4];
  unsigned int per_row[4];
  unsigned int off[4];
};
__global__ __launch_bounds__(L_THREADS) void cat_rows_kernel(CatArgs a, uint4* __restrict__ dst, size_t ldd, size_t N) {
  const int k = blockIdx.y;
  const size_t i = (size_t)blockIdx.x * L_THREADS + threadIdx.x, per = a.per_row[k];
  if (i >= N * per) return;
  const size_t r = i / per, c = i - r * per;
  dst[r * ldd + a.off[k] + c] = reinterpret_cast<const uint4*>(a.src[k])[r * a.lds[k] + c];
}

}

extern "C" int tamtr_cat_rows(const void* const* src, const long long* lds, const int* C, int n, void* dst, long long ldd, long long N, int dtype,
                              void* stream) {
  if (!src || !lds || !C || !dst || n < 1 || n > 4 || N <= 0) return TAMTR_EINVAL;
  if (dtype != TAMTR_F32 && dtype != TAMTR_BF16) return TAMTR_EINVAL;
  const int v = dtype == TAMTR_F32 ? 4 : 8;
  CatArgs a;
  unsigned off = 0, widest = 0;
  if (ldd % v || (uintptr_t)dst % 16) return TAMTR_EUNSUP;
  for (int k = 0; k < 4; ++k) {
    const int kk = k < n ? k : 0;
    if (k < n && (!src[k] || C[k] <= 0 || lds[k] < C[k])) return TAMTR_EINVAL;
    if (k < n && (C[k] % v || lds[k] % v || (uintptr_t)src[k] % 16)) return TAMTR_EUNSUP;
    a.src[k] = src[kk]; a.lds[k] = (unsigned long long)(lds[kk] / v); a.per_row[k] = k < n ? (unsigned)(C[k] / v) : 0u; a.off[k] = off;
    if (k < n) { off += (unsigned)(C[k] / v); widest = a.per_row[k] > widest ? a.per_row[k] : widest; }
  }
  if ((long long)off * v > ldd) return TAMTR_EINVAL;
  const size_t items = (size_t)N * widest;
  hipLaunchKernelGGL(cat_rows_kernel, dim3((unsigned)((items + L_THREADS - 1) / L_THREADS), n), dim3(L_THREADS), 0, (hipStream_t)stream, a,
                     (uint4*)dst, (size_t)ldd / v, (size_t)N);
  return tamtr_launch_status();
}

extern "C" int tamtr_copy_rows(const void* src, long long lds, void* dst, long long ldd, long long N, int C, int dtype, void* stream) {
  if (!src || !dst || N <= 0 || C <= 0 || lds < C || ldd < C) return TAMTR_EINVAL;
  if (dtype != TAMTR_F32 && dtype != TAMTR_BF16) return TAMTR_EINVAL;
  const int e = dtype == TAMTR_F32 ? 4 : 2, v = 16 / e;
  hipStream_t s = (hipStream_t)stream;
  const bool vec = C % v == 0 && lds % v == 0 && ldd % v == 0 && ((uintptr_t)src % 16) == 0 && ((uintptr_t)dst % 16) == 0;
  if (vec) {
    const size_t n = (size_t)N * (C / v);
    hipLaunchKernelGGL(copy_rows_kernel<uint4>, dim3((unsigned)((n + L_THREADS - 1) / L_THREADS)), dim3(L_THREADS), 0, s, (const uint4*)src,
                       (uint4*)dst, n, C / v, (size_t)lds / v, (size_t)ldd / v);
  } else if (e == 4) {
    const size_t n = (size_t)N * C;
    hipLaunchKernelGGL(copy_rows_kernel<uint32_t>, dim3((unsigned)((n + L_THREADS - 1) / L_THREADS)), dim3(L_THREADS), 0, s, (const uint32_t*)src,
                       (uint32_t*)dst, n, C, (size_t)lds, (size_t)ldd);
  } else {
    const size_t n = (size_t)N * C;
    hipLaunchKernelGGL(copy_rows_kernel<uint16_t>, dim3((unsigned)((n + L_THREADS - 1) / L_THREADS)), dim3(L_THREADS), 0, s, (const uint16_t*)src,
                       (uint16_t*)dst, n, C, (size_t)lds, (size_t)ldd);
  }
  return tamtr_launch_status();
}

extern "C" int tamtr_relayout(const void* src, void* dst, int B, int C, int HW, int ld, int to_nhwc, int dtype, void* stream) {
  if (!src || !dst || B <= 0 || C <= 0 || HW <= 0 || ld < C) return TAMTR_EINVAL;
  if (dtype != TAMTR_F32 && dtype != TAMTR_BF16) return TAMTR_EINVAL;
  const int R = to_nhwc ? C : HW, S = to_nhwc ? HW : C;
  const unsigned gx = (S + LT - 1) / LT, gy = (R + LT - 1) / LT;
  if (B > 65535 || gy > 65535) return TAMTR_EUNSUP;
  const int e = dtype == TAMTR_F32 ? 4 : 2;
  const int lds = to_nhwc ? HW : ld, ldd = to_nhwc ? ld : HW;
  const int vec = R % 4 == 0 && S % 4 == 0 && ld % 4 == 0 && ((uintptr_t)src % (4 * e)) == 0 && ((uintptr_t)dst % (4 * e)) == 0;
  hipStream_t s = (hipStream_t)stream;
  if (dtype == TAMTR_F32)
    hipLaunchKernelGGL(transpose_tiles_kernel<uint32_t>, dim3(gx, gy, B), dim3(L_THREADS), 0, s, (const uint32_t*)src, (uint32_t*)dst, R, S, lds, ldd, vec);
  else
    hipLaunchKernelGGL(transpose_tiles_kernel<uint16_t>, dim3(gx, gy, B), dim3(L_THREADS), 0, s, (const uint16_t*)src, (uint16_t*)dst, R, S, lds, ldd, vec);
  return tamtr_launch_status();
}
```

tam-tr_amd/csrc/pool.hip:

```cpp
#include "common.h"

namespace {

constexpr int P_THREADS = 256;

struct PoolGeom {
  int C, H, W, Ho, Wo, k, s, p, nhwc;
};

struct Where {
  int c, h, w;
  int unit;
};
__device__ __forceinline__ bool locate(const PoolGeom& g, int HH, int WW, Where& q) {
  const int i = blockIdx.x * P_THREADS + threadIdx.x;
  if (g.nhwc) {
    if (i >= WW * g.C) return false;
    q.c = i % g.C; q.w = i / g.C; q.h = blockIdx.y % HH;
    q.unit = blockIdx.y / HH;
  } else {
    if (i >= HH * WW) return false;
    q.w = i % WW; q.h = i / WW; q.c = 0;
    q.unit = blockIdx.y;
  }
  return true;
}
__device__ __forceinline__ size_t off(const PoolGeom& g, int WW, int c, int h, int w) {
  return g.nhwc ? ((size_t)h * WW + w) * g.C + c : (size_t)h * WW + w;
}
__device__ __forceinline__ size_t base(const PoolGeom& g, int unit, int HH, int WW) {
  return (size_t)unit * HH * WW * (g.nhwc ? g.C : 1);
}

template <typename T, int KS>
__global__ __launch_bounds__(P_THREADS) void maxpool_fwd_kernel(const T* __restrict__ x, T* __restrict__ y, uint8_t* __restrict__ code,
                                                                PoolGeom g) {
  if (KS) { g.k = KS / 16; g.s = KS % 16; g.p = g.k / 2; }
  Where q;
  if (!locate(g, g.Ho, g.Wo, q)) return;
  const T* xp = x + base(g, q.unit, g.H, g.W);
  const int h0 = q.h * g.s - g.p, w0 = q.w * g.s - g.p;
  float best = -INFINITY;
  int win = max(0, -h0) * g.k + max(0, -w0);
  for (int dh = 0; dh < g.k; ++dh) {
    const int h = h0 + dh;
    if (h < 0 || h >= g.H) continue;
    for (int dw = 0; dw < g.k; ++dw) {
      const int w = w0 + dw;
      if (w < 0 || w >= g.W) continue;
      const float v = Elt<T>::ld(xp + off(g, g.W, q.c, h, w));
      if (v > best || v != v) { best = v; win = dh * g.k + dw; }
    }
  }
  const size_t o = base(g, q.unit, g.Ho, g.Wo) + off(g, g.Wo, q.c, q.h, q.w);
  Elt<T>::st(y + o, best);
  code[o] = (uint8_t)win;
}

template <typename T, int KS>
__global__ __launch_bounds__(P_THREADS) void maxpool_bwd_kernel(const T* __restrict__ gy, const uint8_t* __restrict__ code,
                                                                const T* __restrict__ addend, T* __restrict__ gx, PoolGeom g) {
  if (KS) { g.k = KS / 16; g.s = KS % 16; g.p = g.k / 2; }
  Where q;
  if (!locate(g, g.H, g.W, q)) return;
  const size_t out_base = base(g, q.unit, g.Ho, g.Wo);
  const T* gyp = gy + out_base;
  const uint8_t* cp = code + out_base;
  const int h = q.h, w = q.w;
  const int oh_lo = max(0, (h + g.p - g.k + g.s) / g.s), oh_hi = min(g.Ho - 1, (h + g.p) / g.s);
  const int ow_lo = max(0, (w + g.p - g.k + g.s) / g.s), ow_hi = min(g.Wo - 1, (w + g.p) / g.s);
  const size_t i = base(g, q.unit, g.H, g.W) + off(g, g.W, q.c, h, w);
  float acc = addend ? Elt<T>::ld(addend + i) : 0.f;
  for (int oh = oh_lo; oh <= oh_hi; ++oh)
    for (int ow = ow_lo; ow <= ow_hi; ++ow) {
      const size_t o = off(g, g.Wo, q.c, oh, ow);
      const int mine = (h - (oh * g.s - g.p)) * g.k + (w - (ow * g.s - g.p));
      if (cp[o] == mine) acc += Elt<T>::ld(gyp + o);
    }
  Elt<T>::st(gx + i, acc);
}

template <typename T, int KS>
__global__ __launch_bounds__(P_THREADS) void maxpool_bwd4_kernel(const T* __restrict__ gy, const uint8_t* __restrict__ code,
                                                                 const T* __restrict__ addend, T* __restrict__ gx, PoolGeom g) {
  if (KS) { g.k = KS / 16; g.s = KS % 16; g.p = g.k / 2; }
  const int i4 = blockIdx.x * P_THREADS + threadIdx.x, w4 = g.W / 4;
  if (i4 >= g.H * w4) return;
  const int h = i4 / w4, wb = (i4 - h * w4) * 4;
  const size_t in_base = (size_t)blockIdx.y * g.H * g.W, out_base = (size_t)blockIdx.y * g.Ho * g.Wo;
  const T* gyp = gy + out_base;
  const uint8_t* cp = code + out_base;
  const int oh_lo = max(0, (h + g.p - g.k + g.s) / g.s), oh_hi = min(g.Ho - 1, (h + g.p) / g.s);
  float acc[4] = {0.f, 0.f, 0.f, 0.f};
  if (addend) Elt<T>::ld4(addend + in_base + (size_t)h * g.W + wb, acc);
#pragma unroll
  for (int j = 0; j < 4; ++j) {
    const int w = wb + j;
    const int ow_lo = max(0, (w + g.p - g.k + g.s) / g.s), ow_hi = min(g.Wo - 1, (w + g.p) / g.s);
    for (int oh = oh_lo; oh <= oh_hi; ++oh)
      for (int ow = ow_lo; ow <= ow_hi; ++ow) {
        const size_t o = (size_t)oh * g.Wo + ow;
        const int mine = (h - (oh * g.s - g.p)) * g.k + (w - (ow * g.s - g.p));
        if (cp[o] == mine) acc[j] += Elt<T>::ld(gyp + o);
      }
  }
  Elt<T>::st4(gx + in_base + (size_t)h * g.W + wb, acc);
}

int pool_geom(PoolGeom& g, int B, int C, int H, int W, int k, int s, int p, int nhwc) {
  if (B <= 0 || C <= 0 || H <= 0 || W <= 0 || k <= 0 || s <= 0 || p < 0) return TAMTR_EINVAL;
  if (k > 15 || 2 * p > k || H + 2 * p < k || W + 2 * p < k) return TAMTR_EUNSUP;
  g = PoolGeom{C, H, W, (H + 2 * p - k) / s + 1, (W + 2 * p - k) / s + 1, k, s, p, nhwc ? 1 : 0};
  return TAMTR_OK;
}

dim3 pool_grid(const PoolGeom& g, int B, int HH, int WW) {
  const long long per = g.nhwc ? (long long)WW * g.C : (long long)HH * WW, rows = g.nhwc ? (long long)B * HH : (long long)B * g.C;
  if (per > 0x7fffffffLL - P_THREADS || rows > 65535LL * 65535LL) return dim3(0);
  if (rows > 65535) return dim3(0);
  return dim3((unsigned)((per + P_THREADS - 1) / P_THREADS), (unsigned)rows);
}

}

extern "C" int tamtr_maxpool_out(int n, int k, int s, int p) { return (n + 2 * p - k) / s + 1; }

extern "C" int tamtr_maxpool_fwd(const void* x, void* y, uint8_t* code, int B, int C, int H, int W, int k, int s, int p, int nhwc,
                                 int dtype, void* stream) {
  PoolGeom g;
  const int rc = pool_geom(g, B, C, H, W, k, s, p, nhwc);
  if (rc) return rc;
  if (!x || !y || !code || (dtype != TAMTR_F32 && dtype != TAMTR_BF16)) return TAMTR_EINVAL;
  const dim3 grid = pool_grid(g, B, g.Ho, g.Wo);
  if (!grid.x) return TAMTR_EUNSUP;
  hipStream_t st = (hipStream_t)stream;
  const int ks = (p == k / 2 && ((k == 3 && s == 2) || (k == 5 && s == 1))) ? 16 * k + s : 0;
#define FWD(T, KS) hipLaunchKernelGGL((maxpool_fwd_kernel<T, KS>), grid, dim3(P_THREADS), 0, st, (const T*)x, (T*)y, code, g)
  if (dtype == TAMTR_F32) { if (ks == 50) FWD(float, 50); else if (ks == 81) FWD(float, 81); else FWD(float, 0); }
  else { if (ks == 50) FWD(bf16_t, 50); else if (ks == 81) FWD(bf16_t, 81); else FWD(bf16_t, 0); }
#undef FWD
  return tamtr_launch_status();
}

extern "C" int tamtr_maxpool_bwd(const void* gy, const uint8_t* code, const void* addend, void* gx, int B, int C, int H, int W, int k, int s, int p, int nhwc,
                                 int dtype, void* stream) {
  PoolGeom g;
  const int rc = pool_geom(g, B, C, H, W, k, s, p, nhwc);
  if (rc) return rc;
  if (!gy || !gx || !code || (dtype != TAMTR_F32 && dtype != TAMTR_BF16)) return TAMTR_EINVAL;
  const dim3 grid = pool_grid(g, B, H, W);
  if (!grid.x) return TAMTR_EUNSUP;
  hipStream_t st = (hipStream_t)stream;
  const int ks = (p == k / 2 && ((k == 3 && s == 2) || (k == 5 && s == 1))) ? 16 * k + s : 0;
  const int al = dtype == TAMTR_F32 ? 16 : 8;
  if (!g.nhwc && W % 4 == 0 && ((uintptr_t)gx % al) == 0 && (!addend || ((uintptr_t)addend % al) == 0) && (long long)B * C <= 65535) {
    const dim3 g4((unsigned)(((long long)H * (W / 4) + P_THREADS - 1) / P_THREADS), (unsigned)(B * C));
#define BWD4(T, KS) hipLaunchKernelGGL((maxpool_bwd4_kernel<T, KS>), g4, dim3(P_THREADS), 0, st, (const T*)gy, code, (const T*)addend, (T*)gx, g)
    if (dtype == TAMTR_F32) { if (ks == 50) BWD4(float, 50); else if (ks == 81) BWD4(float, 81); else BWD4(float, 0); }
    else { if (ks == 50) BWD4(bf16_t, 50); else if (ks == 81) BWD4(bf16_t, 81); else BWD4(bf16_t, 0); }
#undef BWD4
    return tamtr_launch_status();
  }
#define BWD(T, KS) hipLaunchKernelGGL((maxpool_bwd_kernel<T, KS>), grid, dim3(P_THREADS), 0, st, (const T*)gy, code, (const T*)addend, (T*)gx, g)
  if (dtype == TAMTR_F32) { if (ks == 50) BWD(float, 50); else if (ks == 81) BWD(float, 81); else BWD(float, 0); }
  else { if (ks == 50) BWD(bf16_t, 50); else if (ks == 81) BWD(bf16_t, 81); else BWD(bf16_t, 0); }
#undef BWD
  return tamtr_launch_status();
}
```

tam-tr_amd/model.py:

```python
import torch
import torch.nn as nn

from .backbone import CPAM, Concat, Conv, RepNCSPELAN4, SPPELAN, Upsample
from .head import ManbaWorldDecoder
from .hostio import stager
from .loss import RTDETRDetectionLoss
from .modules import TIAGELAN

TAMTR_SPEC = [
    [-1, 'Conv', [64, 3, 2]], [-1, 'Conv', [128, 3, 2]], [-1, 'RepNCSPELAN4', [256, 128, 64, 1]],
    [-1, 'Conv', [256, 3, 2]], [-1, 'RepNCSPELAN4', [512, 256, 128, 1]], [-1, 'Conv', [512, 3, 2]],
    [-1, 'RepNCSPELAN4', [512, 512, 256, 1]], [-1, 'Conv', [512, 3, 2]], [-1, 'RepNCSPELAN4', [512, 512, 256, 1]],
    [-1, 'SPPELAN', [512, 256]],
    [-1, 'Conv', [512, 1, 1]], [-1, 'Upsample', [2.0]], [6, 'Conv', [512, 1, 1]], [4, 'Conv', [512, 1, 1]],
    [-1, 'Upsample', [0.5]], [[-1, -3, -4], 'Concat', [1]], [-1, 'TIAGELAN', [512, 512, 256, 1, 8]], [-1, 'CPAM', []],
    [-1, 'Conv', [256, 1, 1]], [-1, 'Upsample', [2.0]], [4, 'Conv', [256, 1, 1]], [2, 'Conv', [256, 1, 1]],
    [-1, 'Upsample', [0.5]], [[-1, -3, -4], 'Concat', [1]], [-1, 'TIAGELAN', [256, 256, 128, 1, 4]], [-1, 'CPAM', []],
    [-1, 'Conv', [128, 1, 1]], [-1, 'Upsample', [2.0]], [2, 'Conv', [128, 1, 1]], [0, 'Conv', [128, 1, 1]],
    [-1, 'Upsample', [0.5]], [[-1, -3, -4], 'Concat', [1]], [-1, 'TIAGELAN', [128, 128, 64, 1, 2]], [-1, 'CPAM', []],
    [-1, 'Conv', [128, 3, 2]], [[-1, 24], 'Concat', [1]], [-1, 'TIAGELAN', [256, 256, 128, 1, 4]], [-1, 'CPAM', []],
    [-1, 'Conv', [256, 3, 2]], [[-1, 16], 'Concat', [1]], [-1, 'TIAGELAN', [512, 512, 256, 1, 8]],
    [[32, 36, 40], 'ManbaWorldDecoder', ['nc', 512, 100, 4, 8, 3]],
]


def build_graph(spec, ch=3, nc=10):
    chans, layers, save = [], [], []
    for i, (f, name, args) in enumerate(spec):
        cin = ch if i == 0 else (chans[f] if isinstance(f, int) else None)
        if name == 'Conv':
            m, c2 = Conv(cin, *args), args[0]
        elif name == 'RepNCSPELAN4':
            m, c2 = RepNCSPELAN4(cin, *args), args[0]
        elif name == 'TIAGELAN':
            m, c2 = TIAGELAN(cin, *args), args[0]
        elif name == 'SPPELAN':
            m, c2 = SPPELAN(cin, *args), args[0]
        elif name == 'Upsample':
            m, c2 = Upsample(None, args[0], 'nearest'), cin
        elif name == 'Concat':
            m, c2 = Concat(*args), sum(chans[j] for j in f)
        elif name == 'CPAM':
            m, c2 = CPAM(cin), cin
        elif name == 'ManbaWorldDecoder':
            a = [nc if v == 'nc' else v for v in args]
            m, c2 = ManbaWorldDecoder(a[0], [chans[j] for j in f], *a[1:]), None
        elif name == 'Detect':
            from .detect import Detect
            m, c2 = Detect(nc if args[0] == 'nc' else args[0], [chans[j] for j in f]), None
        else:
            raise ValueError(name)
        m.i, m.f, m.type = i, f, name
        m.np = sum(p.numel() for p in m.parameters())
        save.extend(x % i for x in ([f] if isinstance(f, int) else f) if x != -1)
        layers.append(m)
        chans.append(c2)
    return nn.Sequential(*layers), sorted(set(save))


import os
_CHANNELS_LAST = os.environ.get('TAMTR_CHANNELS_LAST', '0' if os.environ.get('TAMTR_DETERMINISTIC') == '1' else '1') != '0'


class _CastGroup(torch.autograd.Function):

    @staticmethod
    def forward(ctx, *ws):
        ctx.set_materialize_grads(False)
        outs = [torch.empty_like(w, dtype=torch.bfloat16) for w in ws]
        torch._foreach_copy_(outs, list(ws))
        return tuple(outs)

    @staticmethod
    def backward(ctx, *gs):
        live = [i for i, g in enumerate(gs) if g is not None]
        outs = [torch.empty_like(gs[i], dtype=torch.float32) for i in live]
        if live:
            torch._foreach_copy_(outs, [gs[i] for i in live])
        res = [None] * len(gs)
        for i, o in zip(live, outs):
            res[i] = o
        return tuple(res)


class _ShadowGroup(torch.autograd.Function):

    @staticmethod
    def forward(ctx, n, *ts):
        ctx.set_materialize_grads(False)
        return tuple(s.view_as(s) for s in ts[n:])

    @staticmethod
    def backward(ctx, *gs):
        return (None,) + _CastGroup.backward(ctx, *gs) + (None,) * len(gs)


def _cast_group(masters):
    from . import ops
    sh = [ops.bf16_shadow(p) for p in masters]
    if all(s is not None for s in sh):
        return _ShadowGroup.apply(len(masters), *masters, *sh)
    return _CastGroup.apply(*masters)


def _conv_weight_names(m):
    names = getattr(m, '_tamtr_conv_names', None)
    if names is None:
        names = [f'{n}.weight' if n else 'weight' for n, sub in m.named_modules() if isinstance(sub, nn.Conv2d)]
        m._tamtr_conv_names = names
    return names


class _StaticPart(nn.Module):

    def __init__(self, model):
        super().__init__()
        head = model.model[-1]
        self.trunk, self.vss, self.proj = nn.ModuleList(model.model[:-1]), head.VSSBlocks, head.input_proj
        object.__setattr__(self, '_owner', model)

    def forward(self, img, txt, drop_scales):
        return self._owner.token_memory(img, txt, autocast_cache=False, drop_scales=drop_scales)[0]


class RTDETRDetectionWorldModel(nn.Module):

    def __init__(self, cfg=None, ch=3, nc=10, verbose=False):
        super().__init__()
        self.yaml = {'nc': nc, 'ch': ch, 'spec': 'TAMTR'}
        self.nc = nc
        self.names = {i: f'{i}' for i in range(nc)}
        self.txt_feats = torch.randn(1, nc, 512)
        self.model, self.save = build_graph(cfg or TAMTR_SPEC, ch, nc)
        self.channels_last = False
        self.set_channels_last(_CHANNELS_LAST)
        self.stride = torch.Tensor([32])
        self.autocast_dtype = None

    def set_channels_last(self, flag=True):
        self.release_static_part()
        fmt = torch.channels_last if flag else torch.contiguous_format
        for m in self.model[:-1].modules():
            if isinstance(m, nn.Conv2d) and m.kernel_size != (1, 1):
                m.weight.data = m.weight.data.contiguous(memory_format=fmt)
        self.channels_last = bool(flag)
        return self

    def forward(self, x, *args, **kwargs):
        if isinstance(x, dict):
            return self.loss(x, *args, **kwargs)
        return self.predict(x, *args, **kwargs)

    def init_criterion(self):
        return RTDETRDetectionLoss(nc=self.nc, use_vfl=True)

    def set_text_features(self, txt_feats):
        self.txt_feats = txt_feats.reshape(-1, txt_feats.shape[-2], txt_feats.shape[-1])
        self.model[-1].nc = self.txt_feats.shape[1]

    def fuse(self, verbose=False):
        from .backbone import Conv, RepConvN
        if not self.is_fused():
            for m in list(self.modules()):
                if isinstance(m, RepConvN):
                    m.switch_to_deploy()
            for m in list(self.modules()):
                if isinstance(m, Conv):
                    m.fuse()
                if hasattr(m, '_tamtr_conv_names'):
                    del m._tamtr_conv_names
        return self

    def is_fused(self, thresh=10):
        return sum(isinstance(v, nn.BatchNorm2d) for v in self.modules()) < thresh

    def token_memory(self, x, txt, autocast_cache=True, drop_scales=None):
        head = self.model[-1]
        with torch.autocast('cuda', dtype=self.autocast_dtype or torch.bfloat16, enabled=self.autocast_dtype is not None,
                            cache_enabled=autocast_cache):
            if self.channels_last and x.is_cuda:
                x = x.contiguous(memory_format=torch.channels_last)
            from . import ops
            counters = ops.begin_bn_counter_batch() if self.training else None
            y = []
            grouped_cast = self.autocast_dtype == torch.bfloat16 and x.is_cuda and torch.is_grad_enabled()
            for m in self.model[:-1]:
                if m.f != -1:
                    x = y[m.f] if isinstance(m.f, int) else [x if j == -1 else y[j] for j in m.f]
                args = (x, txt) if isinstance(m, TIAGELAN) else (x,)
                names = _conv_weight_names(m) if grouped_cast else ()
                if names:
                    masters = [m.get_parameter(n) for n in names]
                    w16 = _cast_group(masters)
                    for c, p in zip(w16, masters):
                        c._tamtr_master = p
                    x = torch.func.functional_call(m, dict(zip(names, w16)), args)
                else:
                    x = m(*args)
                y.append(x if m.i in self.save else None)
            feats, shapes = head.encode([y[j] for j in head.f], drop_scales)
            if counters is not None:
                ops.end_bn_counter_batch()
        return feats, shapes

    def capture_static_part(self, img, txt_feats, warmup=3, verify=True, log=None):
        import torch.version
        from .graphs import GraphedPart, VALIDATED_HIP
        self.release_static_part()
        part = _StaticPart(self)
        part.train(self.training)
        txt = txt_feats.to(device=img.device, dtype=torch.float32)
        if len(txt) != len(img):
            txt = txt.repeat(len(img), 1, 1)
        saved = [b.detach().clone() for b in part.buffers()]
        head = self.model[-1]
        dp = torch.ones(head.num_Blocks, 2, len(img), device=img.device)
        with torch.no_grad():
            _, shapes = self.token_memory(img, txt, drop_scales=dp)
        graphed = GraphedPart(part, (img.detach(), txt.detach(), dp), warmup=warmup, log=log)
        try:
            import time
            t0 = time.perf_counter()
            self.static_part_check = graphed.verify() if verify else None
            if log is not None and verify:
                log(f'graph capture: replay check against eager execution {time.perf_counter() - t0:.1f} s')
        finally:
            with torch.no_grad():
                for b, v in zip(part.buffers(), saved):
                    b.copy_(v)
        if verify and not self.static_part_check['ok']:
            chk = self.static_part_check
            msg = (f"HIP-graph replay of the static part does not reproduce eager execution (token memory rel {chk['out_rel_max']:.2e} / bound "
                   f"{chk['bound_out']:.1e}, all gradients rel {chk['grad_l2_rel_max']:.2e} / bound {chk['bound_grad_l2']:.1e}, worst informative tensor "
                   f"{chk['replays'][-1]['worst_informative_grad']} at {chk['replays'][-1]['worst_informative_over_bound']:.1f} x its bound; "
                   f"HIP {torch.version.hip}): running eagerly")
            (log or print)(msg)
            raise RuntimeError(msg)
        if verify and not self.static_part_check['conclusive']:
            chk = self.static_part_check
            msg = (f"HIP-graph replay check inconclusive: eager execution itself is not reproducible here (whole-gradient difference between two "
                   f"eager runs {chk['eager_noise_grad_l2']:.2e}, replay against eager {chk['grad_l2_rel_max']:.2e}); only finiteness and order of "
                   "magnitude could be checked - TAMTR_DETERMINISTIC=1 or the shipped convolution tables give a conclusive comparison")
            if verify != 'loose':
                (log or print)(msg + ": running eagerly (capture_static_part(verify='loose') accepts such a capture)")
                raise RuntimeError(msg)
            if log is not None:
                log(msg + " - accepted (verify='loose')")
        if log is not None and not any(str(torch.version.hip).startswith(v) for v in VALIDATED_HIP):
            log(f'HIP-graph replay: runtime {torch.version.hip} is not one this package was validated on {VALIDATED_HIP}; the replay check passed')
        self._static = (graphed, tuple(img.shape), img.dtype, self.autocast_dtype, self.training, shapes, tuple(txt.shape))
        return self

    def release_static_part(self):
        self._static = None

    def predict(self, x, profile=False, visualize=False, batch=None, augment=False, txt_feats=None):
        txt = (self.txt_feats if txt_feats is None else txt_feats).to(device=x.device, dtype=torch.float32)
        if len(txt) != len(x):
            txt = txt.repeat(len(x), 1, 1)
        head = self.model[-1]
        st = getattr(self, '_static', None)
        dp = head.draw_drop_scales(len(x), x.device) if self.training and x.is_cuda else None
        if st is not None and st[1:5] == (tuple(x.shape), x.dtype, self.autocast_dtype, self.training) and st[6] == tuple(txt.shape) \
                and torch.is_grad_enabled():
            feats, shapes = st[0](x, txt, dp), st[5]
        else:
            feats, shapes = self.token_memory(x, txt, drop_scales=dp)
        with torch.autocast('cuda', dtype=self.autocast_dtype or torch.bfloat16, enabled=self.autocast_dtype is not None):
            return head.decode(feats, shapes, txt.clone(), batch)

    def loss(self, batch, preds=None):
        if not hasattr(self, 'criterion'):
            self.criterion = self.init_criterion()
        img = batch['img']
        dev = img.device
        host = {'cls': batch['cls'].detach().cpu().long().view(-1), 'bboxes': batch['bboxes'].detach().cpu().float(),
                'batch_idx': batch['batch_idx'].detach().cpu().long().view(-1)}
        counts = torch.bincount(host['batch_idx'], minlength=len(img)).tolist()
        st = stager()
        st.next_step()
        targets = {k: (batch[k].to(dev, host[k].dtype).view(host[k].shape) if batch[k].is_cuda else st.h2d(host[k], dev)) for k in host}
        targets.update(gt_groups=counts, host=host)
        preds = self.predict(img, batch=targets, txt_feats=batch['txt_feats']) if preds is None else preds
        dec_bboxes, dec_scores, enc_bboxes, enc_scores, dn_meta = preds if self.training else preds[1]
        dn_bboxes = dn_scores = None
        if dn_meta is not None:
            dn_bboxes, dec_bboxes = torch.split(dec_bboxes, dn_meta['dn_num_split'], dim=2)
            dn_scores, dec_scores = torch.split(dec_scores, dn_meta['dn_num_split'], dim=2)
        dec_bboxes = torch.cat([enc_bboxes.unsqueeze(0).to(dec_bboxes.dtype), dec_bboxes])
        dec_scores = torch.cat([enc_scores.unsqueeze(0).to(dec_scores.dtype), dec_scores])
        terms = self.criterion((dec_bboxes, dec_scores), targets, dn_bboxes=dn_bboxes, dn_scores=dn_scores, dn_meta=dn_meta)
        self.last_loss_terms = {k: v.detach() for k, v in terms.items()}
        items = torch.stack([terms[k].detach() for k in ('loss_giou', 'loss_class', 'loss_bbox')])
        return torch.stack(list(terms.values())).sum(), items
```

tam-tr_amd/modules.py:

```python
import copy
import math

import torch
import torch.nn as nn
import torch.nn.functional as F

from . import ops
from .backbone import Conv, RepNCSPELAN4


class MaxSigmoidAttnBlock(nn.Module):

    def __init__(self, c1, c2, nh=1, ec=128, gc=512, scale=False):
        super().__init__()
        self.nh = nh
        self.hc = c2 // nh
        self.ec = Conv(c1, ec, k=1, act=False) if c1 != ec else None
        self.gl = nn.Linear(gc, ec)
        self.bias = nn.Parameter(torch.zeros(nh))
        self.proj_conv = Conv(c1, c2, k=3, s=1, act=False)
        self.scale = nn.Parameter(torch.ones(1, nh, 1, 1)) if scale else 1.0

    def forward(self, x, guide):
        bs, _, h, w = x.shape
        gk = self.gl(guide)
        pc = self.proj_conv
        if (self.ec is None and not torch.is_grad_enabled() and not isinstance(self.scale, torch.Tensor) and 'bn' in pc._modules
                and pc.bn.training and pc.bn.affine and isinstance(pc.act, nn.Identity) and ops.gate_cl_ok(x, x.shape[1], self.nh)):
            if ops.conv3x3_cl_ok(x, pc.conv) and ops.bn_cl_ok(pc.conv.out_channels, x.dtype):
                v_raw, stats = ops.conv3x3_cl_stats(x, pc.conv, pc.bn)
                return ops.maxsigmoid_gate_cl(x, gk, self.bias, v_raw, stats, pc.bn, self.nh, 1.0)
            v_raw = pc.conv(x)
            if ops.is_cl(v_raw) and v_raw.dtype == x.dtype and ops.bn_cl_ok(v_raw.shape[1], v_raw.dtype):
                stats = ops.bn_stats_cl(v_raw.permute(0, 2, 3, 1).reshape(bs * h * w, -1), pc.bn)
                return ops.maxsigmoid_gate_cl(x, gk, self.bias, v_raw, stats, pc.bn, self.nh, 1.0)
            v = pc.post(v_raw)
            return ops.maxsigmoid_gate(x if x.dtype == v.dtype else x.to(v.dtype), gk, self.bias, v, self.nh, 1.0)
        embed = self.ec(x) if self.ec is not None else x
        v = self.proj_conv(x)
        if embed.dtype != v.dtype:
            embed = embed.to(v.dtype)
        out = ops.maxsigmoid_gate(embed, gk, self.bias, v, self.nh, 1.0)
        if isinstance(self.scale, torch.Tensor):
            out = (out.view(bs, self.nh, -1, h, w) * self.scale.unsqueeze(2).to(out.dtype)).view(bs, -1, h, w)
        return out


class TIAGELAN(RepNCSPELAN4):
    use_attn_output = False

    def __init__(self, c1, c2, c3, c4, c5=1, nh=8):
        super().__init__(c1, c2, c3, c4, c5)
        self.attn = MaxSigmoidAttnBlock(c4, c4, nh=nh, ec=c4)

    def forward(self, x, guide):
        y = self.branches(x)
        if self.use_attn_output:
            y[-3] = self.attn(y[-3], guide)
        else:
            with torch.no_grad():
                self.attn(y[-3].detach(), guide.detach())
        return self.cv4(ops.cat_channels(y))


class MLP(nn.Module):
    def __init__(self, input_dim, hidden_dim, output_dim, num_layers):
        super().__init__()
        self.num_layers = num_layers
        dims = [input_dim] + [hidden_dim] * (num_layers - 1) + [output_dim]
        self.layers = nn.ModuleList(nn.Linear(a, b) for a, b in zip(dims[:-1], dims[1:]))

    def forward(self, x):
        for i, lin in enumerate(self.layers):
            x = ops.linear(x, lin)
            if i + 1 < self.num_layers:
                x = F.relu(x)
        return x


class ContrastiveHeadMLP(nn.Module):

    def __init__(self):
        super().__init__()
        self.bias = nn.Parameter(torch.tensor([-10.0]))
        self.logit_scale = nn.Parameter(torch.ones([]) * math.log(1 / 0.07))

    def forward(self, x, w):
        return ops.contrastive_logits(x, w, self.logit_scale, self.bias)


class MSDeformAttn(nn.Module):

    def __init__(self, d_model=256, n_levels=4, n_heads=8, n_points=4):
        super().__init__()
        if d_model % n_heads != 0:
            raise ValueError(f'd_model must be divisible by n_heads, but got {d_model} and {n_heads}')
        self.im2col_step = 64
        self.d_model, self.n_levels, self.n_heads, self.n_points = d_model, n_levels, n_heads, n_points
        self.sampling_offsets = nn.Linear(d_model, n_heads * n_levels * n_points * 2)
        self.attention_weights = nn.Linear(d_model, n_heads * n_levels * n_points)
        self.value_proj = nn.Linear(d_model, d_model)
        self.output_proj = nn.Linear(d_model, d_model)
        self._reset_parameters()

    def _reset_parameters(self):
        nn.init.zeros_(self.sampling_offsets.weight)
        th = torch.arange(self.n_heads, dtype=torch.float32) * (2.0 * math.pi / self.n_heads)
        ring = torch.stack([th.cos(), th.sin()], -1)
        ring = ring / ring.abs().max(-1, keepdim=True).values
        ring = ring.view(self.n_heads, 1, 1, 2) * torch.arange(1, self.n_points + 1, dtype=torch.float32).view(1, 1, -1, 1)
        with torch.no_grad():
            self.sampling_offsets.bias.copy_(ring.expand(-1, self.n_levels, -1, -1).reshape(-1))
        nn.init.zeros_(self.attention_weights.weight)
        nn.init.zeros_(self.attention_weights.bias)
        for lin in (self.value_proj, self.output_proj):
            nn.init.xavier_uniform_(lin.weight)
            nn.init.zeros_(lin.bias)

    def project_value(self, value):
        bs, len_v = value.shape[:2]
        if value.dtype == torch.bfloat16:
            v = ops.linear_bf16(value, self.value_proj.weight, self.value_proj.bias)
        else:
            v = F.linear(value, self.value_proj.weight, self.value_proj.bias)
        return v.view(bs, len_v, self.n_heads, self.d_model // self.n_heads)

    def forward(self, query, refer_bbox, value, value_shapes, value_mask=None):
        bs, len_q = query.shape[:2]
        len_v = value.shape[1]
        assert sum(s[0] * s[1] for s in value_shapes) == len_v
        paired = value_mask is None and ops.value_proj_msda_ok(value, self.value_proj, self.n_heads, len_q, self.n_points)
        if paired:
            v = None
        elif value_mask is not None:
            v = F.linear(value, self.value_proj.weight, self.value_proj.bias).masked_fill(value_mask[..., None], 0.0)
            v = v.view(bs, len_v, self.n_heads, -1)
        else:
            v = self.project_value(value)
        q32 = ops.shared_bf16(query.float(), self.sampling_offsets, self.attention_weights)
        off = ops.linear(q32, self.sampling_offsets) if q32.dtype == torch.bfloat16 else \
            F.linear(q32, self.sampling_offsets.weight.float(), self.sampling_offsets.bias.float())
        off = off.float().view(bs, len_q, self.n_heads, self.n_levels, self.n_points, 2)
        aw = ops.linear(q32, self.attention_weights) if q32.dtype == torch.bfloat16 else \
            F.linear(q32, self.attention_weights.weight.float(), self.attention_weights.bias.float())
        aw = F.softmax(aw.float().view(bs, len_q, self.n_heads, -1), -1).view(bs, len_q, self.n_heads, self.n_levels, self.n_points)
        ref = refer_bbox.float()
        n = ref.shape[-1]
        if n == 2:
            norm = torch.as_tensor(value_shapes, dtype=torch.float32, device=query.device).flip(-1)
            loc = ref[:, :, None, :, None, :] + off / norm[None, None, None, :, None, :]
        elif n == 4:
            loc = torch.addcmul(ref[:, :, None, :, None, :2], off, ref[:, :, None, :, None, 2:] * (0.5 / self.n_points))
        else:
            raise ValueError(f'Last dim of reference_points must be 2 or 4, but got {n}.')
        out = ops.value_proj_msda(value, self.value_proj, self.n_heads, value_shapes, loc, aw) if paired else ops.ms_deform_attn_core(v, value_shapes, loc, aw)
        return ops.linear(out.to(query.dtype), self.output_proj)


class _SelfAttention(nn.Module):

    def __init__(self, d_model, n_heads):
        super().__init__()
        self.embed_dim, self.num_heads = d_model, n_heads
        self.in_proj_weight = nn.Parameter(torch.empty(3 * d_model, d_model))
        self.in_proj_bias = nn.Parameter(torch.zeros(3 * d_model))
        self.out_proj = nn.Linear(d_model, d_model)
        nn.init.xavier_uniform_(self.in_proj_weight)
        nn.init.zeros_(self.out_proj.bias)

    def forward(self, qk, v, attn_mask=None):
        B, Q, C = qk.shape
        w, b = self.in_proj_weight, self.in_proj_bias
        qk_p = ops.linear_rows(qk, w, b, 0, 2 * C)
        v_p = ops.linear_rows(v, w, b, 2 * C, 3 * C)
        q, k = qk_p[..., :C], qk_p[..., C:]
        o = ops.self_attention(q, k, v_p, self.num_heads, attn_mask)
        return ops.linear(o, self.out_proj)


class DeformableTransformerDecoderLayer(nn.Module):
    def __init__(self, d_model=256, n_heads=8, d_ffn=1024, dropout=0., act=nn.ReLU(), n_levels=4, n_points=4):
        super().__init__()
        if dropout != 0.:
            raise NotImplementedError('TAM-TR trains with dropout=0 (head.py:1026); non-zero dropout is not built')
        self.self_attn = _SelfAttention(d_model, n_heads)
        self.norm1 = nn.LayerNorm(d_model)
        self.cross_attn = MSDeformAttn(d_model, n_levels, n_heads, n_points)
        self.norm2 = nn.LayerNorm(d_model)
        self.linear1 = nn.Linear(d_model, d_ffn)
        self.act = act
        self.linear2 = nn.Linear(d_ffn, d_model)
        self.norm3 = nn.LayerNorm(d_model)

    @staticmethod
    def with_pos_embed(tensor, pos):
        return tensor if pos is None else tensor + pos

    def forward_ffn(self, tgt):
        return ops.layer_norm_module(self.norm3, tgt + ops.linear(self.act(ops.linear(tgt, self.linear1)), self.linear2))

    def forward(self, embed, refer_bbox, feats, shapes, padding_mask=None, attn_mask=None, query_pos=None):
        qk = self.with_pos_embed(embed, query_pos)
        embed = ops.layer_norm_module(self.norm1, embed + self.self_attn(qk, embed, attn_mask))
        t = self.cross_attn(self.with_pos_embed(embed, query_pos), refer_bbox.unsqueeze(2), feats, shapes, padding_mask)
        embed = ops.layer_norm_module(self.norm2, embed + t)
        return self.forward_ffn(embed)


def inverse_sigmoid(x, eps=1e-5):
    x = x.clamp(min=0, max=1)
    return torch.log(x.clamp(min=eps) / (1 - x).clamp(min=eps))


class TextDeformableTransformerDecoder(nn.Module):
    def __init__(self, hidden_dim, decoder_layer, num_layers, eval_idx=-1):
# ... 70 lines not shown
```

tam-tr_amd/ops.py:

```python
import ctypes
import math

import torch

from . import _lib
from ._lib import call, dtype_code, ptr, require_gpu, stream_ptr
import os as _os

_PROJ_CONV_LIB = _os.environ.get('TAMTR_PROJ_CONV') == 'miopen'

_I, _F = ctypes.c_int, ctypes.c_float

KERNEL_EVENTS = {}


def _c(t):
    return t if t.is_contiguous() else t.contiguous()


def _is_cl(t):
    return t.dim() == 4 and not t.is_contiguous() and t.is_contiguous(memory_format=torch.channels_last)


def is_cl(t):
    return _is_cl(t)


def _cl_pitch(t):
    if t.dim() != 4:
        return 0
    B, C, H, W = t.shape
    sb, sc, sh, sw = t.stride()
    ok = sc == 1 and sw >= C and sh == W * sw and (B == 1 or sb == H * W * sw)
    return sw if ok else 0


class _Relayout(torch.autograd.Function):

    @staticmethod
    def forward(ctx, x, to_nchw):
        require_gpu(x)
        ctx.to_nchw = to_nchw
        return _relayout(x, to_nchw)

    @staticmethod
    def backward(ctx, g):
        if ctx.to_nchw:
            return (_relayout(g, False) if g.is_contiguous() else g.contiguous(memory_format=torch.channels_last)), None
        return (_relayout(g, True) if _cl_pitch(g) else g.contiguous()), None


def _relayout(x, to_nchw):
    B, C, H, W = x.shape
    if x.dtype not in (torch.float32, torch.bfloat16):
        return x.contiguous() if to_nchw else x.contiguous(memory_format=torch.channels_last)
    out = torch.empty(x.shape, dtype=x.dtype, device=x.device, memory_format=torch.contiguous_format if to_nchw else torch.channels_last)
    call('tamtr_relayout', ptr(x), ptr(out), B, C, H * W, _cl_pitch(x) if to_nchw else C, 0 if to_nchw else 1, dtype_code(x), stream_ptr())
    return out


def to_nchw(x):
    if x.is_contiguous():
        return x
    return _Relayout.apply(x, True) if (x.is_cuda and _cl_pitch(x)) else x.contiguous()


class _CatChannels(torch.autograd.Function):

    @staticmethod
    def forward(ctx, *maps):
        B, _, H, W = maps[0].shape
        widths = [m.shape[1] for m in maps]
        out = torch.empty((B, sum(widths), H, W), dtype=maps[0].dtype, device=maps[0].device, memory_format=torch.channels_last)
        ct, e, v = sum(widths), maps[0].element_size(), 16 // maps[0].element_size()
        N = B * H * W
        pitches = [_cl_pitch(m) for m in maps]
        if all(c % v == 0 and ld % v == 0 and m.data_ptr() % 16 == 0 for m, c, ld in zip(maps, widths, pitches)):
            for i in range(0, len(maps), 4):
                grp = list(range(i, min(i + 4, len(maps))))
                n = len(grp)
                src = (ctypes.c_void_p * n)(*[maps[j].data_ptr() for j in grp])
                lds = (ctypes.c_longlong * n)(*[pitches[j] for j in grp])
                cs = (ctypes.c_int * n)(*[widths[j] for j in grp])
                call('tamtr_cat_rows', ctypes.cast(src, ctypes.c_void_p), ctypes.cast(lds, ctypes.c_void_p), ctypes.cast(cs, ctypes.c_void_p), n,
                     out.data_ptr() + sum(widths[:i]) * e, ct, N, dtype_code(maps[0]), stream_ptr())
        else:
            off = 0
            for m, c, ld in zip(maps, widths, pitches):
                call('tamtr_copy_rows', ptr(m), ld, out.data_ptr() + off * e, ct, N, c, dtype_code(m), stream_ptr())
                off += c
        ctx.widths = widths
        return out

    @staticmethod
    def backward(ctx, g):
        return tuple(g.split(ctx.widths, 1))


def cat_channels(maps):
    maps = list(maps)
    if len(maps) > 1 and all(m.is_cuda and m.dim() == 4 and m.dtype == maps[0].dtype and m.dtype in (torch.float32, torch.bfloat16)
                             and m.shape[0] == maps[0].shape[0] and m.shape[2:] == maps[0].shape[2:] and _cl_pitch(m) and not m.is_contiguous()
                             for m in maps):
        return _CatChannels.apply(*maps)
    return torch.cat(maps, 1)


class _ChunkChannels(torch.autograd.Function):

    @staticmethod
    def forward(ctx, x):
        h = x.shape[1] // 2
        return x[:, :h], x[:, h:]

    @staticmethod
    def backward(ctx, g0, g1):
        return cat_channels([g0, g1])


def chunk2_channels(x):
    if x.is_cuda and _is_cl(x) and x.shape[1] % 2 == 0 and x.dtype in (torch.float32, torch.bfloat16) and x.requires_grad:
        return _ChunkChannels.apply(x)
    return x.chunk(2, 1)


class _PackChannels(torch.autograd.Function):

    @staticmethod
    def forward(ctx, x):
        B, C, H, W = x.shape
        out = torch.empty((B, C, H, W), dtype=x.dtype, device=x.device, memory_format=torch.channels_last)
        call('tamtr_copy_rows', ptr(x), _cl_pitch(x), ptr(out), C, B * H * W, C, dtype_code(x), stream_ptr())
        return out

    @staticmethod
    def backward(ctx, g):
        return g


def pack_channels(x):
    if x.is_cuda and x.dim() == 4 and not _is_cl(x) and not x.is_contiguous() and _cl_pitch(x) and x.dtype in (torch.float32, torch.bfloat16):
        return _PackChannels.apply(x)
    return x


class _Resample2(torch.autograd.Function):

    @staticmethod
    def forward(ctx, x, up):
        B, C, H, W = x.shape
        ctx.cfg = (up, B, C, H, W)
        Ho, Wo = (2 * H, 2 * W) if up else (H // 2, W // 2)
        out = torch.empty((B, C, Ho, Wo), dtype=x.dtype, device=x.device, memory_format=torch.channels_last)
        call('tamtr_resample2', ptr(x), ptr(out), B, H, W, C, 0 if up else 2, dtype_code(x), stream_ptr())
        return out

    @staticmethod
    def backward(ctx, g):
        up, B, C, H, W = ctx.cfg
        g = g if _is_cl(g) else (pack_channels(g) if _cl_pitch(g) else g.contiguous(memory_format=torch.channels_last))
        gx = torch.empty((B, C, H, W), dtype=g.dtype, device=g.device, memory_format=torch.channels_last)
        call('tamtr_resample2', ptr(g), ptr(gx), B, H, W, C, 1 if up else 3, dtype_code(g), stream_ptr())
        return gx, None


def resample2(x, up):
    v = 8 if x.dtype == torch.bfloat16 else 4
    if x.is_cuda and _is_cl(x) and x.dtype in (torch.float32, torch.bfloat16) and x.shape[1] % v == 0 and (up or (x.shape[2] % 2 == 0 and x.shape[3] % 2 == 0)):
        return _Resample2.apply(x, bool(up))
    return None


def to_channels_last(x):
    if x.dim() != 4 or _is_cl(x):
        return x
    return _Relayout.apply(x, False) if (x.is_contiguous() and x.is_cuda) else x.contiguous(memory_format=torch.channels_last)


class _MaxPool(torch.autograd.Function):

    @staticmethod
    def forward(ctx, x, k, s, p):
        require_gpu(x)
        nhwc = _is_cl(x)
        if not nhwc:
            x = _c(x)
        B, C, H, W = x.shape
        Ho, Wo = (H + 2 * p - k) // s + 1, (W + 2 * p - k) // s + 1
        fmt = torch.channels_last if nhwc else torch.contiguous_format
        y = torch.empty((B, C, Ho, Wo), dtype=x.dtype, device=x.device, memory_format=fmt)
        code = torch.empty((B, C, Ho, Wo), dtype=torch.uint8, device=x.device, memory_format=fmt)
        call('tamtr_maxpool_fwd', ptr(x), ptr(y), ptr(code), B, C, H, W, k, s, p, int(nhwc), dtype_code(x), stream_ptr())
        ctx.save_for_backward(code)
        ctx.cfg = (B, C, H, W, k, s, p, nhwc, x.dtype)
        return y

    @staticmethod
    def backward(ctx, gy):
        code, = ctx.saved_tensors
        B, C, H, W, k, s, p, nhwc, dt = ctx.cfg
        gy = gy.to(dt)
        gy = (pack_channels(gy) if _cl_pitch(gy) else gy.contiguous(memory_format=torch.channels_last)) if nhwc else _c(gy)
        gx = torch.empty((B, C, H, W), dtype=dt, device=gy.device, memory_format=torch.channels_last if nhwc else torch.contiguous_format)
        call('tamtr_maxpool_bwd', ptr(gy), ptr(code), None, ptr(gx), B, C, H, W, k, s, p, int(nhwc), dtype_code(gy), stream_ptr())
        return gx, None, None, None


def max_pool2d(x, k, s, p):
    if x.is_cuda and x.dim() == 4 and x.dtype in (torch.float32, torch.bfloat16) and k <= 15 and 2 * p <= k:
        return _MaxPool.apply(x, int(k), int(s), int(p))
    return torch.nn.functional.max_pool2d(x, k, s, p)


class _MaxSigmoidGate(torch.autograd.Function):

    @staticmethod
    def forward(ctx, x, gk, bias, v, nh, scale):
        require_gpu(x, gk, bias, v)
        B, C, H, W = x.shape
        T = gk.shape[1]
        hc = C // nh
        x, v = to_nchw(x), to_nchw(v)
        gk32, b32 = _c(gk.float()), _c(bias.float())
        out = torch.empty_like(x)
        aw = torch.empty(B, nh, H * W, device=x.device, dtype=torch.float32)
        arg = torch.empty(B, nh, H * W, device=x.device, dtype=torch.int32)
        call('tamtr_maxsigmoid_gate_fwd', ptr(x), ptr(gk32), ptr(b32), ptr(v), ptr(out), ptr(aw), ptr(arg), B, nh, hc, H * W, T,
             _F(scale), dtype_code(x), stream_ptr())
        ctx.save_for_backward(x, gk32, v, aw, arg)
        ctx.cfg = (nh, hc, T, scale, gk.dtype, bias.dtype)
        return out

    @staticmethod
    def backward(ctx, dout):
        x, gk32, v, aw, arg = ctx.saved_tensors
        nh, hc, T, scale, gk_dt, b_dt = ctx.cfg
        B, C, H, W = x.shape
        HW = H * W
        dout = _c(dout.to(x.dtype))
        dx, dv = torch.empty_like(x), torch.empty_like(x)
        dlogit = torch.empty(B, nh, HW, device=x.device, dtype=torch.float32)
        call('tamtr_maxsigmoid_gate_bwd', ptr(dout), ptr(x), ptr(gk32), ptr(v), ptr(aw), ptr(arg), ptr(dx), ptr(dv), ptr(dlogit),
             B, nh, hc, HW, T, _F(scale), dtype_code(x), stream_ptr())
        sel = torch.zeros(B, nh, T, HW, device=x.device, dtype=torch.float32)
        sel.scatter_(2, arg.long().unsqueeze(2), dlogit.unsqueeze(2))
        dgk = torch.matmul(sel, x.view(B, nh, hc, HW).float().transpose(2, 3))
        dgk = dgk.permute(0, 2, 1, 3).reshape(B, T, C)
        dbias = dlogit.sum((0, 2)) * math.sqrt(hc)
        return dx, dgk.to(gk_dt), dbias.to(b_dt), dv, None, None


def gate_cl_ok(x, C, nh):
    hc = C // nh if nh else 0
    lpr, lph = C // 8, hc // 8
    return (x.is_cuda and x.dtype in (torch.float32, torch.bfloat16) and _cl_pitch(x) and nh * hc == C and C % 8 == 0 and hc % 8 == 0
            and 0 < lpr <= 64 and lpr & (lpr - 1) == 0 and lph & (lph - 1) == 0 and _cl_pitch(x) % (16 // x.element_size()) == 0
            and x.data_ptr() % 16 == 0)


@torch.no_grad()
def bn_stats_cl(x2d, bn):
    require_gpu(x2d)
    x2d = _c(x2d)
    N, C = x2d.shape
    mom = _bn_tick(bn)
    mr = torch.empty(C, 2, device=x2d.device, dtype=torch.float32)
    part = torch.empty(C * _lib.lib().tamtr_bncl_blocks(N, C, dtype_code(x2d)) * 3, device=x2d.device, dtype=torch.float32)
    rm, rv = (bn.running_mean, bn.running_var) if bn.track_running_stats else (None, None)
    call('tamtr_bncl_stats', ptr(x2d), ptr(rm), ptr(rv), ptr(mr), ptr(part), N, C, float(bn.eps), float(mom), dtype_code(x2d), stream_ptr())
    return mr


def conv3x3_cl_ok(x, conv):
    if _PROJ_CONV_LIB or not (x.is_cuda and x.dtype == torch.bfloat16 and x.dim() == 4):
        return False
    ld = _cl_pitch(x)
    return (isinstance(conv, torch.nn.Conv2d) and conv.kernel_size == (3, 3) and conv.stride == (1, 1) and conv.padding == (1, 1)
            and conv.dilation == (1, 1) and conv.groups == 1 and conv.bias is None and conv.padding_mode == 'zeros'
            and conv.in_channels == x.shape[1] and conv.in_channels % 32 == 0 and conv.out_channels % 64 == 0
            and ld and ld % 8 == 0 and x.data_ptr() % 16 == 0 and conv.weight.dtype in (torch.float32, torch.bfloat16))


@torch.no_grad()
def conv3x3_cl_stats(x, conv, bn):
    require_gpu(x)
    B, C1, H, W = x.shape
    C2 = conv.out_channels
    w = _c(conv.weight)
    wpk = torch.empty(9 * C1 * C2, device=x.device, dtype=torch.bfloat16)
    call('tamtr_conv3x3_pack_weight', ptr(w), ptr(wpk), C1, C2, dtype_code(w), stream_ptr())
    y = torch.empty((B, C2, H, W), dtype=torch.bfloat16, device=x.device, memory_format=torch.channels_last)
    mom = _bn_tick(bn)
    mr = torch.empty(C2, 2, device=x.device, dtype=torch.float32)
    part = torch.empty(C2 * _lib.lib().tamtr_conv3x3_tiles(B, H, W) * 3, device=x.device, dtype=torch.float32)
    rm, rv = (bn.running_mean, bn.running_var) if bn.track_running_stats else (None, None)
    call('tamtr_conv3x3_cl_stats_fwd', ptr(x), _cl_pitch(x), ptr(wpk), ptr(y), ptr(rm), ptr(rv), ptr(mr), ptr(part), B, H, W, C1, C2,
         float(bn.eps), float(mom), stream_ptr())
    return y, mr


@torch.no_grad()
def maxsigmoid_gate_cl(e, gk, bias, v_raw, v_stats, v_bn, nh, scale=1.0):
    require_gpu(e, gk, bias, v_raw)
    B, C, H, W = e.shape
    v_raw = v_raw if _is_cl(v_raw) else v_raw.contiguous(memory_format=torch.channels_last)
    out = torch.empty((B, C, H, W), dtype=e.dtype, device=e.device, memory_format=torch.channels_last)
    gk32, b32 = _c(gk.float()), _c(bias.float())
    ga, be = _c(v_bn.weight.float()), _c(v_bn.bias.float())
    call('tamtr_maxsigmoid_gate_cl_fwd', ptr(e), _cl_pitch(e), None, None, None, ptr(v_raw), ptr(v_stats), ptr(ga), ptr(be), ptr(gk32), ptr(b32),
         ptr(out), None, None, B, nh, C // nh, H * W, gk.shape[1], _F(scale), dtype_code(e), stream_ptr())
    return out


def maxsigmoid_gate(x, gk, bias, v, nh, scale=1.0):
    return _MaxSigmoidGate.apply(x, gk, bias, v, int(nh), float(scale))


_MSDA_ATOMICS = _os.environ.get('TAMTR_MSDA_ATOMICS') == '1'


def deterministic():
    return _os.environ.get('TAMTR_DETERMINISTIC') == '1' or torch.are_deterministic_algorithms_enabled()


_WARNED = set()


def _atomic_fallback(what):
    if not deterministic():
        return
    if torch.are_deterministic_algorithms_enabled() and not torch.is_deterministic_algorithms_warn_only_enabled():
        raise _lib.TamtrHipError(f'deterministic mode: {what}')
    if what not in _WARNED:
        _WARNED.add(what)
        import warnings
        warnings.warn(f'{what}; running the float-atomic kernel, this step is not bitwise reproducible '
                      '(torch.use_deterministic_algorithms(True) without warn_only raises here instead)', UserWarning, stacklevel=3)


def msda_sorted_ok(Q, P, D):
    return Q * P * 4 <= 8192 and D % 8 == 0 and D <= 256


class _MSDeformCore(torch.autograd.Function):
    @staticmethod
    def forward(ctx, value, shapes, loc, aw):
        require_gpu(value, loc, aw)
        B, L, M, D = value.shape
        _, Q, _, nl, P, _ = loc.shape
        value = _c(value)
        loc32, aw32 = _c(loc.float()), _c(aw.float())
        sh = (ctypes.c_int32 * (2 * nl))(*[int(v) for hw in shapes for v in hw])
        out = torch.empty(B, Q, M * D, device=value.device, dtype=value.dtype)
        call('tamtr_msdeform_attn_fwd', ptr(value), ctypes.cast(sh, ctypes.c_void_p), ptr(loc32), ptr(aw32), ptr(out), B, L, M, D,
             Q, nl, P, dtype_code(value), stream_ptr())
        ctx.save_for_backward(value, loc32, aw32)
        ctx.cfg = (sh, nl, P, loc.dtype, aw.dtype)
        return out

    @staticmethod
    def backward(ctx, gout):
        value, loc32, aw32 = ctx.saved_tensors
        sh, nl, P, loc_dt, aw_dt = ctx.cfg
# ... 1297 lines not shown
        x = _c(x)
        B, C, H, W = x.shape
        Hp, Wp = (H - 1) // 2 + 1, (W - 1) // 2 + 1
        p = torch.empty(B, C, Hp, Wp, dtype=x.dtype, device=x.device)
        idx = torch.empty(B, C, Hp, Wp, dtype=torch.uint8, device=x.device)
        call('tamtr_maxpool_fwd', ptr(x), ptr(p), ptr(idx), B, C, H, W, 3, 2, 1, 0, dtype_code(x), stream_ptr())
        out = torch.empty_like(x)
        s2 = torch.empty(B, 8, H, W, device=x.device, dtype=torch.float32)
        arg = torch.empty(B, 8, H, W, device=x.device, dtype=torch.int32)
        call('tamtr_cpam_fwd', ptr(x), ptr(p), ptr(out), ptr(s2), ptr(arg), B, C, H, W, dtype_code(x), stream_ptr())
        ctx.save_for_backward(x, p, idx, s2, arg)
        return out

    @staticmethod
    def backward(ctx, gout):
        x, p, idx, s2, arg = ctx.saved_tensors
        B, C, H, W = x.shape
        gout = _c(gout.to(x.dtype))
        dxd, du, dp = torch.empty_like(x), torch.empty_like(x), torch.empty_like(p)
        call('tamtr_cpam_bwd', ptr(gout), ptr(x), ptr(p), ptr(s2), ptr(arg), ptr(dxd), ptr(du), ptr(dp), B, C, H, W, dtype_code(x),
             stream_ptr())
        dx = torch.empty_like(x)
        call('tamtr_maxpool_bwd', ptr(dp), ptr(idx), ptr(dxd), ptr(dx), B, C, H, W, 3, 2, 1, 0, dtype_code(x), stream_ptr())
        return dx


class _CPAMCL(torch.autograd.Function):

    @staticmethod
    def forward(ctx, x):
        require_gpu(x)
        B, C, H, W = x.shape
        Hp, Wp = H // 2, W // 2
        cl = torch.channels_last
        p = torch.empty((B, C, Hp, Wp), dtype=x.dtype, device=x.device, memory_format=cl)
        idx = torch.empty((B, C, Hp, Wp), dtype=torch.uint8, device=x.device, memory_format=cl)
        out = torch.empty_like(x, memory_format=cl)
        s2 = torch.empty(B, H, W, 8, device=x.device, dtype=torch.float32)
        arg = torch.empty(B, H, W, 8, device=x.device, dtype=torch.int32)
        call('tamtr_cpam_cl_fwd', ptr(x), ptr(p), ptr(idx), ptr(out), ptr(s2), ptr(arg), B, C, H, W, dtype_code(x), stream_ptr())
        ctx.save_for_backward(x, p, idx, s2, arg)
        return out

    @staticmethod
    def backward(ctx, gout):
        x, p, idx, s2, arg = ctx.saved_tensors
        B, C, H, W = x.shape
        gout = gout.to(x.dtype)
        if not _is_cl(gout):
            gout = gout.contiguous(memory_format=torch.channels_last)
        cl = torch.channels_last
        dxd, du, dp = torch.empty_like(x, memory_format=cl), torch.empty_like(x, memory_format=cl), torch.empty_like(p, memory_format=cl)
        dx = torch.empty_like(x, memory_format=cl)
        call('tamtr_cpam_cl_bwd', ptr(gout), ptr(x), ptr(p), ptr(idx), ptr(s2), ptr(arg), ptr(dxd), ptr(du), ptr(dp), ptr(dx), B, C, H, W, dtype_code(x),
             stream_ptr())
        return dx


def cpam_cl_ok(x):
    if not (x.is_cuda and x.dim() == 4 and x.dtype in (torch.float32, torch.bfloat16) and _is_cl(x) and x.data_ptr() % 16 == 0):
        return False
    B, C, H, W = x.shape
    V = 8 if x.dtype == torch.bfloat16 else 4
    lpc = C // (8 * V)
    return (H % 2 == 0 and W % 2 == 0 and C % (8 * V) == 0 and lpc >= 1 and lpc & (lpc - 1) == 0 and lpc <= 64 and C // V <= 256 and 256 % (C // V) == 0
            and _os.environ.get('TAMTR_CPAM') != 'nchw')


def cpam(x):
    if cpam_cl_ok(x):
        return _CPAMCL.apply(x)
    if _is_cl(x):
        return to_channels_last(_CPAM.apply(to_nchw(x)))
    return _CPAM.apply(x)


class _LayerNorm(torch.autograd.Function):

    @staticmethod
    def forward(ctx, x, gamma, beta, eps):
        require_gpu(x, gamma, beta)
        x = _c(x)
        D = x.shape[-1]
        ntok = x.numel() // D
        g32, b32 = _c(gamma.float()), _c(beta.float())
        out = torch.empty_like(x)
        stats = torch.empty(ntok, 2, device=x.device, dtype=torch.float32)
        call('tamtr_layernorm_fwd', ptr(x), ptr(g32), ptr(b32), ptr(out), ptr(stats), ntok, D, float(eps), dtype_code(x), stream_ptr())
        ctx.save_for_backward(x, g32, stats)
        ctx.cfg = (gamma.dtype, beta.dtype)
        return out

    @staticmethod
    def backward(ctx, gout):
        x, g32, stats = ctx.saved_tensors
        D = x.shape[-1]
        ntok = x.numel() // D
        gout = _c(gout.to(x.dtype))
        gx = torch.empty_like(x)
        part = torch.empty(_lib.lib().tamtr_ln_gate_blocks(ntok), 2, D, device=x.device, dtype=torch.float32)
        call('tamtr_layernorm_bwd', ptr(gout), ptr(x), ptr(g32), ptr(stats), ptr(gx), ptr(part), ntok, D, dtype_code(x), stream_ptr())
        gsum = slab_sum(part)
        return gx, gsum[0].to(ctx.cfg[0]), gsum[1].to(ctx.cfg[1]), None


def layer_norm(x, gamma, beta, eps=1e-5):
    return _LayerNorm.apply(x, gamma, beta, eps)


def layer_norm_module(norm, x):
    D = x.shape[-1]
    if (x.is_cuda and x.dtype in (torch.float32, torch.bfloat16) and len(norm.normalized_shape) == 1 and norm.elementwise_affine and norm.bias is not None
            and D in (32, 64, 128, 256, 512, 1024) and _os.environ.get('TAMTR_DECODER_LN') != 'torch'):
        return _LayerNorm.apply(x, norm.weight, norm.bias, norm.eps)
    return norm(x)


class _BNAct(torch.autograd.Function):

    @staticmethod
    def forward(ctx, x, gamma, beta, running_mean, running_var, eps, momentum, silu):
        require_gpu(x, gamma, beta)
        x = _c(x)
        B, C = x.shape[:2]
        HW = x.numel() // (B * C)
        g32, b32 = _c(gamma.float()), _c(beta.float())
        y = torch.empty_like(x)
        mr = torch.empty(C, 2, device=x.device, dtype=torch.float32)
        part = torch.empty(C * _lib.lib().tamtr_bn_slices(B, HW) * 3, device=x.device, dtype=torch.float32)
        call('tamtr_bn_act_fwd', ptr(x), ptr(g32), ptr(b32), ptr(running_mean), ptr(running_var), ptr(y), ptr(mr), ptr(part), B, C, HW,
             float(eps), float(momentum), int(bool(silu)), dtype_code(x), stream_ptr())
        ctx.save_for_backward(x, g32, b32, mr)
        ctx.cfg = (int(bool(silu)), gamma.dtype, beta.dtype)
        return y

    @staticmethod
    def backward(ctx, gy):
        x, g32, b32, mr = ctx.saved_tensors
        act, g_dt, b_dt = ctx.cfg
        B, C = x.shape[:2]
        HW = x.numel() // (B * C)
        gy = _c(gy.to(x.dtype))
        gx = torch.empty_like(x)
        gg, gb = torch.empty(C, device=x.device, dtype=torch.float32), torch.empty(C, device=x.device, dtype=torch.float32)
        part = torch.empty(C * _lib.lib().tamtr_bn_slices(B, HW) * 2, device=x.device, dtype=torch.float32)
        call('tamtr_bn_act_bwd', ptr(gy), ptr(x), ptr(g32), ptr(b32), ptr(mr), ptr(gx), ptr(gg), ptr(gb), ptr(part), B, C, HW, act,
             dtype_code(x), stream_ptr())
        return gx, gg.to(g_dt), gb.to(b_dt), None, None, None, None, None


class _BNActCL(torch.autograd.Function):

    @staticmethod
    def forward(ctx, x, gamma, beta, running_mean, running_var, eps, momentum, silu, residual=None):
        require_gpu(x, gamma, beta)
        x = _c(x)
        N, C = x.shape
        g32, b32 = _c(gamma.float()), _c(beta.float())
        y = torch.empty_like(x)
        mr = torch.empty(C, 2, device=x.device, dtype=torch.float32)
        part = torch.empty(C * _lib.lib().tamtr_bncl_blocks(N, C, dtype_code(x)) * 3, device=x.device, dtype=torch.float32)
        res = None if residual is None else _c(residual.to(x.dtype))
        call('tamtr_bncl_act_fwd', ptr(x), ptr(g32), ptr(b32), ptr(running_mean), ptr(running_var), ptr(res), ptr(y), ptr(mr), ptr(part), N, C,
             float(eps), float(momentum), int(bool(silu)), dtype_code(x), stream_ptr())
        ctx.save_for_backward(x, g32, b32, mr)
        ctx.cfg = (int(bool(silu)), gamma.dtype, beta.dtype, None if residual is None else residual.dtype)
        return y

    @staticmethod
    def backward(ctx, gy):
        x, g32, b32, mr = ctx.saved_tensors
        act, g_dt, b_dt, res_dt = ctx.cfg
        N, C = x.shape
        g_res = None if res_dt is None else gy.to(res_dt)
        gy = _gy_rows(gy, x)
        gx = torch.empty_like(x)
        gg, gb = torch.empty(C, device=x.device, dtype=torch.float32), torch.empty(C, device=x.device, dtype=torch.float32)
        part = torch.empty(C * _lib.lib().tamtr_bncl_blocks(N, C, dtype_code(x)) * 2 + 2 * C, device=x.device, dtype=torch.float32)
        call('tamtr_bncl_act_bwd', ptr(gy), gy.stride(0), ptr(x), ptr(g32), ptr(b32), ptr(mr), ptr(gx), ptr(gg), ptr(gb), ptr(part), N, C, act,
             dtype_code(x), stream_ptr())
        return gx, gg.to(g_dt), gb.to(b_dt), None, None, None, None, None, g_res


def _gy_rows(gy, x):
    C = x.shape[1]
    gy = gy.to(x.dtype)
    v = 8 if (x.dtype == torch.bfloat16 and C % 8 == 0) else 4
    if not (gy.stride(1) == 1 and gy.stride(0) >= C and gy.stride(0) % v == 0 and gy.data_ptr() % 16 == 0 and (C & (C - 1)) == 0):
        gy = gy.contiguous()
    return gy


class _BN2ActCL(torch.autograd.Function):

    @staticmethod
    def forward(ctx, x1, ga1, be1, rm1, rv1, x2, ga2, be2, rm2, rv2, eps, momentum, silu):
        require_gpu(x1, x2, ga1, ga2)
        x1, x2 = _c(x1), _c(x2)
        N, C = x1.shape
        p1 = [_c(t.float()) for t in (ga1, be1, ga2, be2)]
        y = torch.empty_like(x1)
        mr = torch.empty(2, C, 2, device=x1.device, dtype=torch.float32)
        part = torch.empty(2 * C * _lib.lib().tamtr_bncl_blocks(N, C, dtype_code(x1)) * 3, device=x1.device, dtype=torch.float32)
        call('tamtr_bncl2_act_fwd', ptr(x1), ptr(p1[0]), ptr(p1[1]), ptr(rm1), ptr(rv1), ptr(x2), ptr(p1[2]), ptr(p1[3]), ptr(rm2), ptr(rv2),
             ptr(y), ptr(mr), ptr(part), N, C, float(eps), float(momentum), int(bool(silu)), dtype_code(x1), stream_ptr())
        ctx.save_for_backward(x1, x2, *p1, mr)
        ctx.cfg = (int(bool(silu)), ga1.dtype, be1.dtype, ga2.dtype, be2.dtype)
        return y

    @staticmethod
    def backward(ctx, gy):
        x1, x2, g1, b1, g2, b2, mr = ctx.saved_tensors
        act, dt_g1, dt_b1, dt_g2, dt_b2 = ctx.cfg
        N, C = x1.shape
        gy = _gy_rows(gy, x1)
        gx1, gx2 = torch.empty_like(x1), torch.empty_like(x2)
        gg = torch.empty(4, C, device=x1.device, dtype=torch.float32)
        part = torch.empty(C * _lib.lib().tamtr_bncl_blocks(N, C, dtype_code(x1)) * 3 + 3 * C, device=x1.device, dtype=torch.float32)
        call('tamtr_bncl2_act_bwd', ptr(gy), gy.stride(0), ptr(x1), ptr(x2), ptr(g1), ptr(b1), ptr(g2), ptr(b2), ptr(mr), ptr(gx1), ptr(gx2),
             gg[0].data_ptr(), gg[1].data_ptr(), gg[2].data_ptr(), gg[3].data_ptr(), ptr(part), N, C, act, dtype_code(x1), stream_ptr())
        return (gx1, gg[0].to(dt_g1), gg[1].to(dt_b1), None, None, gx2, gg[2].to(dt_g2), gg[3].to(dt_b2), None, None, None, None, None)


class _BNCatCL(torch.autograd.Function):

    @staticmethod
    def forward(ctx, B, eps, moms, n, *args):
        ys, gammas, betas, rms, rvs = (args[k * n:(k + 1) * n] for k in range(5))
        require_gpu(*ys)
        ys = [_c(y) for y in ys]
        C, dt = ys[0].shape[1], ys[0].dtype
        Ls = [y.shape[0] // B for y in ys]
        Lt = sum(Ls)
        feats = torch.empty(B, Lt, C, device=ys[0].device, dtype=dt)
        saved, off = [], 0
        for y, ga, be, rm, rv, mom, L in zip(ys, gammas, betas, rms, rvs, moms, Ls):
            N = B * L
            g32, b32 = _c(ga.float()), _c(be.float())
            mr = torch.empty(C, 2, device=y.device, dtype=torch.float32)
            part = torch.empty(C * _lib.lib().tamtr_bncl_blocks(N, C, dtype_code(y)) * 3, device=y.device, dtype=torch.float32)
            call('tamtr_bncl_act_seg_fwd', ptr(y), ptr(g32), ptr(b32), ptr(rm), ptr(rv), feats.data_ptr() + off * C * feats.element_size(), L, Lt * C,
                 ptr(mr), ptr(part), N, C, float(eps), float(mom), 0, dtype_code(y), stream_ptr())
            saved += [y, g32, b32, mr]
            off += L
        ctx.save_for_backward(*saved)
        ctx.cfg = (B, n, Ls, [g.dtype for g in gammas], [b.dtype for b in betas])
        return feats

    @staticmethod
    def backward(ctx, gf):
        B, n, Ls, gdt, bdt = ctx.cfg
        saved = ctx.saved_tensors
        Lt = sum(Ls)
        C = saved[0].shape[1]
        gf = _c(gf.to(saved[0].dtype))
        gxs, ggs, gbs, off = [], [], [], 0
        for i, L in enumerate(Ls):
            y, g32, b32, mr = saved[4 * i:4 * i + 4]
            N = B * L
            gx = torch.empty_like(y)
            gg, gb = torch.empty(C, device=y.device, dtype=torch.float32), torch.empty(C, device=y.device, dtype=torch.float32)
            part = torch.empty(C * _lib.lib().tamtr_bncl_blocks(N, C, dtype_code(y)) * 2 + 2 * C, device=y.device, dtype=torch.float32)
            call('tamtr_bncl_act_seg_bwd', gf.data_ptr() + off * C * gf.element_size(), L, Lt * C, ptr(y), ptr(g32), ptr(b32), ptr(mr), ptr(gx), ptr(gg),
                 ptr(gb), ptr(part), N, C, 0, dtype_code(y), stream_ptr())
            gxs.append(gx); ggs.append(gg.to(gdt[i])); gbs.append(gb.to(bdt[i]))
            off += L
        return (None, None, None, None, *gxs, *ggs, *gbs, *([None] * (2 * n)))


def bn_cat_cl(ys, bns, B):
    moms = [_bn_tick(bn) for bn in bns]
    n = len(ys)
    return _BNCatCL.apply(int(B), float(bns[0].eps), tuple(float(m) for m in moms), n, *ys, *[bn.weight for bn in bns], *[bn.bias for bn in bns],
                          *[bn.running_mean for bn in bns], *[bn.running_var for bn in bns])


def bn_cat_cl_ok(ys, bns):
    C = ys[0].shape[1]
    return (all(y.is_cuda and y.dim() == 2 and y.shape[1] == C and y.dtype == ys[0].dtype and y.dtype in (torch.float32, torch.bfloat16) for y in ys)
            and C & (C - 1) == 0 and bn_cl_ok(C, ys[0].dtype) and all(bn.training and bn.track_running_stats and bn.affine and bn.eps == bns[0].eps for bn in bns)
            and _os.environ.get('TAMTR_BN_CAT') != 'torch')


_BN_COUNTERS = None


def begin_bn_counter_batch():
    global _BN_COUNTERS
    _BN_COUNTERS = []
    return _BN_COUNTERS


def end_bn_counter_batch():
    global _BN_COUNTERS
    pending, _BN_COUNTERS = _BN_COUNTERS, None
    if pending:
        torch._foreach_add_(pending, 1)


def bn_cl_ok(C, dtype):
    v = 8 if dtype == torch.bfloat16 and C % 8 == 0 else 4
    return C % 4 == 0 and C <= 1024 and C // v <= 256 and 256 % (C // v) == 0


def _bn_tick(bn):
    if bn.track_running_stats:
        if _BN_COUNTERS is not None and bn.momentum is not None:
            _BN_COUNTERS.append(bn.num_batches_tracked)
        else:
            bn.num_batches_tracked += 1
    return bn.momentum if bn.momentum is not None else 1.0 / float(bn.num_batches_tracked)


def bn_act(x, bn, silu, residual=None):
    mom = _bn_tick(bn)
    rm, rv = (bn.running_mean, bn.running_var) if bn.track_running_stats else (None, None)
    if x.dim() == 2:
        return _BNActCL.apply(x, bn.weight, bn.bias, rm, rv, bn.eps, mom, silu, residual)
    y = _BNAct.apply(x, bn.weight, bn.bias, rm, rv, bn.eps, mom, silu)
    return y if residual is None else y + residual


def bn2_act(x1, bn1, x2, bn2, silu):
    if bn1.eps != bn2.eps or bn1.momentum != bn2.momentum or not (bn1.track_running_stats and bn2.track_running_stats):
        raise _lib.TamtrHipError('bn2_act: the two BatchNorms must share eps / momentum and track running statistics')
    mom = _bn_tick(bn1)
    _bn_tick(bn2)
    return _BN2ActCL.apply(x1, bn1.weight, bn1.bias, bn1.running_mean, bn1.running_var, x2, bn2.weight, bn2.bias, bn2.running_mean,
                           bn2.running_var, bn1.eps, mom, silu)
```

Before: 214.8.

## Write branch outputs directly into preallocated concat buffers to skip channel concat copies

```diff
diff --git a/include/tamtr_hip.h b/include/tamtr_hip.h
--- a/include/tamtr_hip.h
+++ b/include/tamtr_hip.h
@@ -134,6 +134,12 @@
 int tamtr_bncl_act_fwd(const void* x, const float* gamma, const float* beta, float* running_mean, float* running_var, const void* residual,
                        void* y, float* mean_rstd, float* partials, long long N, int C, float eps, float momentum, int act, int dtype,
                        void* stream);
+int tamtr_bncl_act_ld_fwd(const void* x, const float* gamma, const float* beta, float* running_mean, float* running_var, const void* residual,
+                          void* y, long long ldy, float* mean_rstd, float* partials, long long N, int C, float eps, float momentum, int act,
+                          int dtype, void* stream);
+int tamtr_bncl2_act_ld_fwd(const void* x1, const float* gamma1, const float* beta1, float* running_mean1, float* running_var1, const void* x2,
+                           const float* gamma2, const float* beta2, float* running_mean2, float* running_var2, void* y, long long ldy,
+                           float* mean_rstd, float* partials, long long N, int C, float eps, float momentum, int act, int dtype, void* stream);
 int tamtr_bncl_stats(const void* x, float* running_mean, float* running_var, float* mean_rstd, float* partials, long long N, int C, float eps,
                      float momentum, int dtype, void* stream);
 int tamtr_bncl2_act_fwd(const void* x1, const float* gamma1, const float* beta1, float* running_mean1, float* running_var1, const void* x2,
@@ -147,6 +153,7 @@
 
 int tamtr_relayout(const void* src, void* dst, int B, int C, int HW, int ld, int to_nhwc, int dtype, void* stream);
 int tamtr_resample2(const void* src, void* dst, int B, int H, int W, int C, int mode, int dtype, void* stream);
+int tamtr_resample2_ld(const void* src, void* dst, long long ldd, int B, int H, int W, int C, int mode, int dtype, void* stream);
 int tamtr_copy_rows(const void* src, long long lds, void* dst, long long ldd, long long N, int C, int dtype, void* stream);
 int tamtr_cat_rows(const void* const* src, const long long* lds, const int* C, int n, void* dst, long long ldd, long long N, int dtype,
                    void* stream);
@@ -154,6 +161,8 @@
 int tamtr_maxpool_out(int n, int k, int s, int p);
 int tamtr_maxpool_fwd(const void* x, void* y, uint8_t* code, int B, int C, int H, int W, int k, int s, int p, int nhwc, int dtype,
                       void* stream);
+int tamtr_maxpool_fwd_ld(const void* x, long long ldx, void* y, long long ldy, uint8_t* code, int B, int C, int H, int W, int k, int s, int p,
+                         int dtype, void* stream);
 int tamtr_maxpool_bwd(const void* gy, const uint8_t* code, const void* addend, void* gx, int B, int C, int H, int W, int k, int s, int p, int nhwc, int dtype,
                       void* stream);
 
diff --git a/tam-tr_amd/_lib.py b/tam-tr_amd/_lib.py
--- a/tam-tr_amd/_lib.py
+++ b/tam-tr_amd/_lib.py
@@ -77,6 +77,10 @@
     'tamtr_relayout': [_P, _P, _I, _I, _I, _I, _I, _I, _P],
     'tamtr_bncl_blocks': [_LL, _I, _I],
     'tamtr_bncl_act_fwd': [_P, _P, _P, _P, _P, _P, _P, _P, _P, _LL, _I, _F, _F, _I, _I, _P],
+    'tamtr_bncl_act_ld_fwd': [_P, _P, _P, _P, _P, _P, _P, _LL, _P, _P, _LL, _I, _F, _F, _I, _I, _P],
+    'tamtr_bncl2_act_ld_fwd': [_P, _P, _P, _P, _P, _P, _P, _P, _P, _P, _P, _LL, _P, _P, _LL, _I, _F, _F, _I, _I, _P],
+    'tamtr_resample2_ld': [_P, _P, _LL, _I, _I, _I, _I, _I, _I, _P],
+    'tamtr_maxpool_fwd_ld': [_P, _LL, _P, _LL, _P, _I, _I, _I, _I, _I, _I, _I, _I, _P],
     'tamtr_bncl_stats': [_P, _P, _P, _P, _P, _LL, _I, _F, _F, _I, _P],
     'tamtr_bn_finalize': [_P, _P, _P, _P, _I, _I, _F, _F, _P],
     'tamtr_conv3x3_tiles': [_I, _I, _I],
diff --git a/tam-tr_amd/backbone.py b/tam-tr_amd/backbone.py
--- a/tam-tr_amd/backbone.py
+++ b/tam-tr_amd/backbone.py
@@ -46,10 +46,10 @@
         return ('bn' in self._modules and y.is_cuda and self.bn.training and self.bn.affine and type(self.act) in (nn.SiLU, nn.Identity)
                 and y.dtype in (torch.bfloat16, torch.float32))
 
-    def forward(self, x, residual=None):
-        return self.post(_conv(self.conv, x), residual)
-
-    def post(self, y, residual=None):
+    def forward(self, x, residual=None, out=None):
+        return self.post(_conv(self.conv, x), residual, out)
+
+    def post(self, y, residual=None, out=None):
         if 'bn' not in self._modules:
             y = self.act(y)
             return y if residual is None else y + residual
@@ -60,7 +60,9 @@
                 res = None
                 if residual is not None and ops.is_cl(residual) and residual.shape == y.shape:
                     res, residual = residual.permute(0, 2, 3, 1).reshape(B * H * W, C), None
-                o = ops.bn_act(y.permute(0, 2, 3, 1).reshape(B * H * W, C), self.bn, isinstance(self.act, nn.SiLU), res)
+                if residual is not None:
+                    out = None
+                o = ops.bn_act(y.permute(0, 2, 3, 1).reshape(B * H * W, C), self.bn, isinstance(self.act, nn.SiLU), res, out)
                 o = o.view(B, H, W, C).permute(0, 3, 1, 2)
                 return o if residual is None else o + residual
             y = ops.bn_act(y, self.bn, isinstance(self.act, nn.SiLU))
@@ -78,7 +80,7 @@
         self.conv2 = Conv(c1, c2, 1, s, p=0, g=g, act=False)
         self.act = nn.SiLU() if act is True else act if isinstance(act, nn.Module) else nn.Identity()
 
-    def forward(self, x):
+    def forward(self, x, out=None):
         if 'conv' in self._modules:
             return self.act(self.conv(x))
         c1, c2 = self.conv1, self.conv2
@@ -89,7 +91,7 @@
                     and c1.bn.track_running_stats and c2.bn.track_running_stats and c1.bn.eps == c2.bn.eps and c1.bn.momentum == c2.bn.momentum):
                 B, C, H, W = y1.shape
                 o = ops.bn2_act(y1.permute(0, 2, 3, 1).reshape(B * H * W, C), c1.bn, y2.permute(0, 2, 3, 1).reshape(B * H * W, C), c2.bn,
-                                isinstance(self.act, nn.SiLU))
+                                isinstance(self.act, nn.SiLU), out)
                 return o.view(B, H, W, C).permute(0, 3, 1, 2)
             return self.act(c1.post(y1) + c2.post(y2))
         return self.act(self.conv1(x) + self.conv2(x))
@@ -121,10 +123,10 @@
         self.cv2 = Conv(c_, c2, k[1], 1, g=g)
         self.add = shortcut and c1 == c2
 
-    def forward(self, x):
+    def forward(self, x, out=None):
         if self.add:
-            return self.cv2(self.cv1(x), residual=x)
-        return self.cv2(self.cv1(x))
+            return self.cv2(self.cv1(x), residual=x, out=out)
+        return self.cv2(self.cv1(x), out=out)
 
 
 class RepNCSP(nn.Module):
@@ -137,7 +139,12 @@
 
     def forward(self, x):
         from . import ops
-        return self.cv3(ops.cat_channels((self.m(self.cv1(x)), self.cv2(x))))
+        c_ = self.cv2.conv.out_channels
+        buf = ops.cat_buffer(x, (c_, c_))
+        a = self.cv1(x) if len(self.m) else self.cv1(x, out=(buf, 0))
+        for i, b in enumerate(self.m):
+            a = b(a, out=(buf, 0)) if i == len(self.m) - 1 else b(a)
+        return self.cv3(ops.cat_channels((a, self.cv2(x, out=(buf, c_))), out=buf))
 
 
 class RepNCSPELAN4(nn.Module):
@@ -152,14 +159,20 @@
 
     def branches(self, x):
         from . import ops
-        y = list(ops.chunk2_channels(self.cv1(x)))
+        c3, c4 = self.cv1.conv.out_channels, self.cv3[-1].conv.out_channels
+        buf = ops.cat_buffer(x, (c3, c4, c4))
+        y = list(ops.chunk2_channels(self.cv1(x, out=(buf, 0))))
         y.append(self.cv2(ops.pack_channels(y[-1])))
-        y.append(self.cv3(y[-1]))
-        return y
-
-    def forward(self, x):
-        from . import ops
-        return self.cv4(ops.cat_channels(self.branches(x)))
+        t = y[-1]
+        for i, m in enumerate(self.cv3):
+            t = m(t, out=(buf, c3 + c4)) if i == len(self.cv3) - 1 else m(t)
+        y.append(t)
+        return y, buf
+
+    def forward(self, x):
+        from . import ops
+        y, buf = self.branches(x)
+        return self.cv4(ops.cat_channels(y, out=buf))
 
 
 class SPPELAN(nn.Module):
@@ -171,10 +184,12 @@
 
     def forward(self, x):
         from . import ops
-        y = [self.cv1(x)]
-        for _ in range(3):
-            y.append(ops.max_pool2d(y[-1], 5, 1, 2) if y[-1].is_cuda else F.max_pool2d(y[-1], 5, 1, 2))
-        return self.cv5(ops.cat_channels(y))
+        c = self.cv1.conv.out_channels
+        buf = ops.cat_buffer(x, (c,) * 4)
+        y = [self.cv1(x, out=(buf, 0))]
+        for i in range(3):
+            y.append(ops.max_pool2d(y[-1], 5, 1, 2, out=(buf, (i + 1) * c)) if y[-1].is_cuda else F.max_pool2d(y[-1], 5, 1, 2))
+        return self.cv5(ops.cat_channels(y, out=buf))
 
 
 class CPAM(nn.Module):
@@ -189,11 +204,11 @@
 
 class Upsample(nn.Upsample):
 
-    def forward(self, x):
+    def forward(self, x, out=None):
         if self.mode == 'nearest' and x.dim() == 4 and self.size is None and isinstance(self.scale_factor, (int, float)):
             if x.is_cuda and self.scale_factor in (0.5, 2.0):
                 from . import ops
-                y = ops.resample2(x, self.scale_factor == 2.0)
+                y = ops.resample2(x, self.scale_factor == 2.0, out)
                 if y is not None:
                     return y
             if self.scale_factor == 0.5 and x.shape[2] % 2 == 0 and x.shape[3] % 2 == 0:
@@ -212,8 +227,8 @@
         super().__init__()
         self.d = dimension
 
-    def forward(self, x):
+    def forward(self, x, out=None):
         if self.d == 1:
             from . import ops
-            return ops.cat_channels(x)
+            return ops.cat_channels(x, out=out)
         return torch.cat(x, self.d)
diff --git a/tam-tr_amd/csrc/bn.hip b/tam-tr_amd/csrc/bn.hip
--- a/tam-tr_amd/csrc/bn.hip
+++ b/tam-tr_amd/csrc/bn.hip
@@ -319,7 +319,7 @@
   }
 }
 
-template <typename T, int V>
+template <typename T, int V, bool LD = false>
 __global__ __launch_bounds__(BN_THREADS) void bncl_apply_kernel(const T* __restrict__ x, const float* __restrict__ mean_rstd,
                                                                  const float* __restrict__ gamma, const float* __restrict__ beta,
                                                                  const T* __restrict__ res, T* __restrict__ y, size_t total, int C, int iters,
@@ -349,17 +349,20 @@
 #pragma unroll
         for (int j = 0; j < V; ++j) v[u][j] += r[j];
       }
-      if (e < end) Vec<T, V>::st(y + (ysg.rows ? seg_addr(e, C, cshift, (size_t)C, ysg) : e), v[u]);
-    }
-  }
-}
-
-template <typename T, int V>
+      if (LD) {
+        if (e < end) Vec<T, V>::st(y + (e >> cshift) * ysg.pitch + (e & (size_t)(C - 1)), v[u]);
+      } else if (e < end) Vec<T, V>::st(y + (ysg.rows ? seg_addr(e, C, cshift, (size_t)C, ysg) : e), v[u]);
+    }
+  }
+}
+
+template <typename T, int V, bool LD = false>
 __global__ __launch_bounds__(BN_THREADS) void bncl2_apply_kernel(const T* __restrict__ x1, const T* __restrict__ x2,
                                                                   const float* __restrict__ mr1, const float* __restrict__ mr2,
                                                                   const float* __restrict__ g1, const float* __restrict__ b1,
                                                                   const float* __restrict__ g2, const float* __restrict__ b2,
-                                                                  T* __restrict__ y, size_t total, int C, int iters, int act) {
+                                                                  T* __restrict__ y, size_t total, int C, int iters, int act,
+                                                                  size_t ldy = 0, int cshift = 0) {
   const size_t piece = (size_t)BN_THREADS * V, start = (size_t)blockIdx.x * iters * piece, end = min(total, start + iters * piece);
   const int c0 = (threadIdx.x % (C / V)) * V;
   const size_t home = start + c0;
@@ -384,7 +387,7 @@
       const size_t e = e0 + (size_t)(it + u) * piece;
 #pragma unroll
       for (int j = 0; j < V; ++j) v[u][j] = act_fwd(fmaf(w[u][j] - m2[j], a2[j], fmaf(v[u][j] - m1[j], a1[j], be[j])), act);
-      if (e < end) Vec<T, V>::st(y + e, v[u]);
+      if (e < end) Vec<T, V>::st(y + (LD ? (e >> cshift) * ldy + (e & (size_t)(C - 1)) : e), v[u]);
     }
   }
 }
@@ -664,7 +667,7 @@
 
 static int bncl_act_fwd_impl(const void* x, const float* gamma, const float* beta, float* running_mean, float* running_var,
                              const void* residual, void* y, float* mean_rstd, float* partials, long long N, int C, float eps,
-                             float momentum, int act, int dtype, void* stream, Seg ysg, int cshift) {
+                             float momentum, int act, int dtype, void* stream, Seg ysg, int cshift, long long ldy = 0) {
   const int rc = bncl_check(x, y, N, C, dtype, act);
   if (rc) return rc;
   if (!gamma || !beta || !mean_rstd || !partials) return TAMTR_EINVAL;
@@ -676,12 +679,16 @@
   else if (V == 8) hipLaunchKernelGGL((bncl_stats_kernel<bf16_t, 8>), dim3(S), dim3(BN_THREADS), 0, s, (const bf16_t*)x, partials, total, C, iters);
   else hipLaunchKernelGGL((bncl_stats_kernel<bf16_t, 4>), dim3(S), dim3(BN_THREADS), 0, s, (const bf16_t*)x, partials, total, C, iters);
   hipLaunchKernelGGL(bn_finalize_kernel, dim3(C), dim3(BN_THREADS), 0, s, partials, mean_rstd, running_mean, running_var, S, eps, momentum);
-  if (dtype == TAMTR_F32)
-    hipLaunchKernelGGL((bncl_apply_kernel<float, 4>), dim3(S), dim3(BN_THREADS), 0, s, (const float*)x, mean_rstd, gamma, beta, (const float*)residual, (float*)y, total, C, iters, act, ysg, cshift);
-  else if (V == 8)
-    hipLaunchKernelGGL((bncl_apply_kernel<bf16_t, 8>), dim3(S), dim3(BN_THREADS), 0, s, (const bf16_t*)x, mean_rstd, gamma, beta, (const bf16_t*)residual, (bf16_t*)y, total, C, iters, act, ysg, cshift);
-  else
-    hipLaunchKernelGGL((bncl_apply_kernel<bf16_t, 4>), dim3(S), dim3(BN_THREADS), 0, s, (const bf16_t*)x, mean_rstd, gamma, beta, (const bf16_t*)residual, (bf16_t*)y, total, C, iters, act, ysg, cshift);
+#define APPLY(T, VV, L)                                                                                                                \
+  hipLaunchKernelGGL((bncl_apply_kernel<T, VV, L>), dim3(S), dim3(BN_THREADS), 0, s, (const T*)x, mean_rstd, gamma, beta, (const T*)residual, \
+                     (T*)y, total, C, iters, act, ysg, cshift)
+  if (ldy) {
+    ysg = Seg{0, (size_t)ldy};
+    if (dtype == TAMTR_F32) APPLY(float, 4, true); else if (V == 8) APPLY(bf16_t, 8, true); else APPLY(bf16_t, 4, true);
+  } else {
+    if (dtype == TAMTR_F32) APPLY(float, 4, false); else if (V == 8) APPLY(bf16_t, 8, false); else APPLY(bf16_t, 4, false);
+  }
+#undef APPLY
   return tamtr_launch_status();
 }
 
@@ -690,6 +697,27 @@
                                   float momentum, int act, int dtype, void* stream) {
   return bncl_act_fwd_impl(x, gamma, beta, running_mean, running_var, residual, y, mean_rstd, partials, N, C, eps, momentum, act, dtype, stream,
                            Seg{0, 0}, 0);
+}
+
+static int bncl_ld_check(long long ldy, int C, int dtype) {
+  if (C <= 0 || ldy < C || ldy > 0x7fffffffLL) return TAMTR_EINVAL;
+  if ((C & (C - 1)) || ldy % bncl_vec(C, dtype)) return TAMTR_EUNSUP;
+  return TAMTR_OK;
+}
+static int bncl_shift(int C) {
+  int cshift = 0;
+  while ((1 << cshift) < C) ++cshift;
+  return cshift;
+}
+
+extern "C" int tamtr_bncl_act_ld_fwd(const void* x, const float* gamma, const float* beta, float* running_mean, float* running_var,
+                                     const void* residual, void* y, long long ldy, float* mean_rstd, float* partials, long long N, int C,
+                                     float eps, float momentum, int act, int dtype, void* stream) {
+  if (dtype != TAMTR_F32 && dtype != TAMTR_BF16) return TAMTR_EINVAL;
+  const int rc = bncl_ld_check(ldy, C, dtype);
+  if (rc) return rc;
+  return bncl_act_fwd_impl(x, gamma, beta, running_mean, running_var, residual, y, mean_rstd, partials, N, C, eps, momentum, act, dtype, stream,
+                           Seg{0, 0}, bncl_shift(C), ldy);
 }
 
 extern "C" int tamtr_bncl_act_seg_fwd(const void* x, const float* gamma, const float* beta, float* running_mean, float* running_var, void* y,
@@ -746,10 +774,10 @@
                            Seg{(unsigned)seg_rows, (size_t)seg_pitch});
 }
 
-extern "C" int tamtr_bncl2_act_fwd(const void* x1, const float* gamma1, const float* beta1, float* running_mean1, float* running_var1,
-                                   const void* x2, const float* gamma2, const float* beta2, float* running_mean2, float* running_var2,
-                                   void* y, float* mean_rstd, float* partials, long long N, int C, float eps, float momentum, int act,
-                                   int dtype, void* stream) {
+static int bncl2_act_fwd_impl(const void* x1, const float* gamma1, const float* beta1, float* running_mean1, float* running_var1,
+                              const void* x2, const float* gamma2, const float* beta2, float* running_mean2, float* running_var2,
+                              void* y, long long ldy, float* mean_rstd, float* partials, long long N, int C, float eps, float momentum, int act,
+                              int dtype, void* stream) {
   int rc = bncl_check(x1, y, N, C, dtype, act);
   if (!rc) rc = bncl_check(x2, y, N, C, dtype, act);
   if (rc) return rc;
@@ -762,16 +790,40 @@
 #define STATS(T, VV, X, P) hipLaunchKernelGGL((bncl_stats_kernel<T, VV>), dim3(S), dim3(BN_THREADS), 0, s, (const T*)X, P, total, C, iters)
 #define APPLY(T, VV)                                                                                                                   \
   hipLaunchKernelGGL((bncl2_apply_kernel<T, VV>), dim3(S), dim3(BN_THREADS), 0, s, (const T*)x1, (const T*)x2, mean_rstd, mr2, gamma1, beta1, \
-                     gamma2, beta2, (T*)y, total, C, iters, act)
+                     gamma2, beta2, (T*)y, total, C, iters, act, (size_t)0, 0)
+#define APPLY_LD(T, VV)                                                                                                                \
+  hipLaunchKernelGGL((bncl2_apply_kernel<T, VV, true>), dim3(S), dim3(BN_THREADS), 0, s, (const T*)x1, (const T*)x2, mean_rstd, mr2, gamma1, \
+                     beta1, gamma2, beta2, (T*)y, total, C, iters, act, (size_t)ldy, bncl_shift(C))
   if (dtype == TAMTR_F32) { STATS(float, 4, x1, partials); STATS(float, 4, x2, part2); }
   else if (V == 8) { STATS(bf16_t, 8, x1, partials); STATS(bf16_t, 8, x2, part2); }
   else { STATS(bf16_t, 4, x1, partials); STATS(bf16_t, 4, x2, part2); }
   hipLaunchKernelGGL(bn_finalize_kernel, dim3(C), dim3(BN_THREADS), 0, s, partials, mean_rstd, running_mean1, running_var1, S, eps, momentum);
   hipLaunchKernelGGL(bn_finalize_kernel, dim3(C), dim3(BN_THREADS), 0, s, part2, mr2, running_mean2, running_var2, S, eps, momentum);
-  if (dtype == TAMTR_F32) APPLY(float, 4); else if (V == 8) APPLY(bf16_t, 8); else APPLY(bf16_t, 4);
+  if (ldy) { if (dtype == TAMTR_F32) APPLY_LD(float, 4); else if (V == 8) APPLY_LD(bf16_t, 8); else APPLY_LD(bf16_t, 4); }
+  else if (dtype == TAMTR_F32) APPLY(float, 4); else if (V == 8) APPLY(bf16_t, 8); else APPLY(bf16_t, 4);
 #undef STATS
 #undef APPLY
+#undef APPLY_LD
   return tamtr_launch_status();
+}
+
+extern "C" int tamtr_bncl2_act_fwd(const void* x1, const float* gamma1, const float* beta1, float* running_mean1, float* running_var1,
+                                   const void* x2, const float* gamma2, const float* beta2, float* running_mean2, float* running_var2,
+                                   void* y, float* mean_rstd, float* partials, long long N, int C, float eps, float momentum, int act,
+                                   int dtype, void* stream) {
+  return bncl2_act_fwd_impl(x1, gamma1, beta1, running_mean1, running_var1, x2, gamma2, beta2, running_mean2, running_var2, y, 0, mean_rstd,
+                            partials, N, C, eps, momentum, act, dtype, stream);
+}
+
+extern "C" int tamtr_bncl2_act_ld_fwd(const void* x1, const float* gamma1, const float* beta1, float* running_mean1, float* running_var1,
+                                      const void* x2, const float* gamma2, const float* beta2, float* running_mean2, float* running_var2,
+                                      void* y, long long ldy, float* mean_rstd, float* partials, long long N, int C, float eps, float momentum,
+                                      int act, int dtype, void* stream) {
+  if (dtype != TAMTR_F32 && dtype != TAMTR_BF16) return TAMTR_EINVAL;
+  const int rc = bncl_ld_check(ldy, C, dtype);
+  if (rc) return rc;
+  return bncl2_act_fwd_impl(x1, gamma1, beta1, running_mean1, running_var1, x2, gamma2, beta2, running_mean2, running_var2, y, ldy, mean_rstd,
+                            partials, N, C, eps, momentum, act, dtype, stream);
 }
 
 extern "C" int tamtr_bncl2_act_bwd(const void* gy, long long ldgy, const void* x1, const void* x2, const float* gamma1, const float* beta1,
diff --git a/tam-tr_amd/csrc/layout.hip b/tam-tr_amd/csrc/layout.hip
--- a/tam-tr_amd/csrc/layout.hip
+++ b/tam-tr_amd/csrc/layout.hip
@@ -54,13 +54,14 @@
   dst[r * ldd + c] = src[r * lds + c];
 }
 
-template <typename T, int V>
+template <typename T, int V, bool LD = false>
 __global__ __launch_bounds__(L_THREADS) void resample2_kernel(const T* __restrict__ src, T* __restrict__ dst, int H, int W, int cv, int mode,
-                                                              size_t n) {
-  const size_t i = (size_t)blockIdx.x * L_THREADS + threadIdx.x;
-  if (i >= n) return;
-  const int c = (int)(i % cv);
-  size_t r = i / cv;
+                                                              size_t n, size_t ldv = 0) {
+  const size_t j = (size_t)blockIdx.x * L_THREADS + threadIdx.x;
+  if (j >= n) return;
+  const int c = (int)(j % cv);
+  size_t r = j / cv;
+  const size_t i = LD ? r * ldv + c : j;
   const int dw_ = (mode == 0) ? 2 * W : (mode == 2) ? W / 2 : W, dh_ = (mode == 0) ? 2 * H : (mode == 2) ? H / 2 : H;
   const int w = (int)(r % dw_); r /= dw_;
   const int h = (int)(r % dh_);
@@ -112,6 +113,22 @@
   return tamtr_launch_status();
 }
 
+extern "C" int tamtr_resample2_ld(const void* src, void* dst, long long ldd, int B, int H, int W, int C, int mode, int dtype, void* stream) {
+  if (!src || !dst || B <= 0 || H <= 0 || W <= 0 || C <= 0 || mode < 0 || mode > 3 || ldd < C) return TAMTR_EINVAL;
+  if (dtype != TAMTR_F32 && dtype != TAMTR_BF16) return TAMTR_EINVAL;
+  const int v = dtype == TAMTR_F32 ? 4 : 8;
+  if (C % v || ldd % v || ((uintptr_t)src | (uintptr_t)dst) % 16 || ((mode == 2 || mode == 3) && ((H | W) & 1))) return TAMTR_EUNSUP;
+  const size_t rows = mode == 0 ? (size_t)B * 2 * H * 2 * W : mode == 2 ? (size_t)B * (H / 2) * (W / 2) : (size_t)B * H * W;
+  const size_t n = rows * (C / v);
+  const unsigned blocks = (unsigned)((n + L_THREADS - 1) / L_THREADS);
+  hipStream_t s = (hipStream_t)stream;
+  if (dtype == TAMTR_F32)
+    hipLaunchKernelGGL((resample2_kernel<uint32_t, 4, true>), dim3(blocks), dim3(L_THREADS), 0, s, (const uint32_t*)src, (uint32_t*)dst, H, W, C / v, mode, n, (size_t)(ldd / v));
+  else
+    hipLaunchKernelGGL((resample2_kernel<uint16_t, 8, true>), dim3(blocks), dim3(L_THREADS), 0, s, (const uint16_t*)src, (uint16_t*)dst, H, W, C / v, mode, n, (size_t)(ldd / v));
+  return tamtr_launch_status();
+}
+
 namespace {
 
 struct CatArgs {
diff --git a/tam-tr_amd/csrc/pool.hip b/tam-tr_amd/csrc/pool.hip
--- a/tam-tr_amd/csrc/pool.hip
+++ b/tam-tr_amd/csrc/pool.hip
@@ -55,6 +55,31 @@
   const size_t o = base(g, q.unit, g.Ho, g.Wo) + off(g, g.Wo, q.c, q.h, q.w);
   Elt<T>::st(y + o, best);
   code[o] = (uint8_t)win;
+}
+
+template <typename T, int KS>
+__global__ __launch_bounds__(P_THREADS) void maxpool_fwd_ld_kernel(const T* __restrict__ x, T* __restrict__ y, uint8_t* __restrict__ code,
+                                                                   PoolGeom g, int ldx, int ldy) {
+  if (KS) { g.k = KS / 16; g.s = KS % 16; g.p = g.k / 2; }
+  Where q;
+  if (!locate(g, g.Ho, g.Wo, q)) return;
+  const T* xp = x + (size_t)q.unit * g.H * g.W * ldx + q.c;
+  const int h0 = q.h * g.s - g.p, w0 = q.w * g.s - g.p;
+  float best = -INFINITY;
+  int win = max(0, -h0) * g.k + max(0, -w0);
+  for (int dh = 0; dh < g.k; ++dh) {
+    const int h = h0 + dh;
+    if (h < 0 || h >= g.H) continue;
+    for (int dw = 0; dw < g.k; ++dw) {
+      const int w = w0 + dw;
+      if (w < 0 || w >= g.W) continue;
+      const float v = Elt<T>::ld(xp + ((size_t)h * g.W + w) * ldx);
+      if (v > best || v != v) { best = v; win = dh * g.k + dw; }
+    }
+  }
+  const size_t pix = ((size_t)q.unit * g.Ho + q.h) * g.Wo + q.w;
+  Elt<T>::st(y + pix * ldy + q.c, best);
+  code[pix * g.C + q.c] = (uint8_t)win;
 }
 
 template <typename T, int KS>
@@ -142,6 +167,24 @@
   return tamtr_launch_status();
 }
 
+extern "C" int tamtr_maxpool_fwd_ld(const void* x, long long ldx, void* y, long long ldy, uint8_t* code, int B, int C, int H, int W, int k, int s,
+                                    int p, int dtype, void* stream) {
+  PoolGeom g;
+  const int rc = pool_geom(g, B, C, H, W, k, s, p, 1);
+  if (rc) return rc;
+  if (!x || !y || !code || (dtype != TAMTR_F32 && dtype != TAMTR_BF16) || ldx < C || ldy < C) return TAMTR_EINVAL;
+  if (ldx > 0x7fffffffLL || ldy > 0x7fffffffLL) return TAMTR_EUNSUP;
+  const dim3 grid = pool_grid(g, B, g.Ho, g.Wo);
+  if (!grid.x) return TAMTR_EUNSUP;
+  hipStream_t st = (hipStream_t)stream;
+  const int ks = (p == k / 2 && ((k == 3 && s == 2) || (k == 5 && s == 1))) ? 16 * k + s : 0;
+#define FWD(T, KS) hipLaunchKernelGGL((maxpool_fwd_ld_kernel<T, KS>), grid, dim3(P_THREADS), 0, st, (const T*)x, (T*)y, code, g, (int)ldx, (int)ldy)
+  if (dtype == TAMTR_F32) { if (ks == 50) FWD(float, 50); else if (ks == 81) FWD(float, 81); else FWD(float, 0); }
+  else { if (ks == 50) FWD(bf16_t, 50); else if (ks == 81) FWD(bf16_t, 81); else FWD(bf16_t, 0); }
+#undef FWD
+  return tamtr_launch_status();
+}
+
 extern "C" int tamtr_maxpool_bwd(const void* gy, const uint8_t* code, const void* addend, void* gx, int B, int C, int H, int W, int k, int s, int p, int nhwc,
                                  int dtype, void* stream) {
   PoolGeom g;
diff --git a/tam-tr_amd/model.py b/tam-tr_amd/model.py
--- a/tam-tr_amd/model.py
+++ b/tam-tr_amd/model.py
@@ -111,6 +111,42 @@
     return names
 
 
+def _row_channels(rows, i):
+    m = rows[i]
+    if isinstance(m, Conv):
+        return m.conv.out_channels
+    if isinstance(m, RepNCSPELAN4):
+        return m.cv4.conv.out_channels
+    if isinstance(m, SPPELAN):
+        return m.cv5.conv.out_channels
+    src = [m.i - 1 if j == -1 else j % m.i for j in ([m.f] if isinstance(m.f, int) else m.f)]
+    return sum(_row_channels(rows, j) for j in src) if isinstance(m, Concat) else _row_channels(rows, src[0])
+
+
+def concat_plan(rows):
+    src = {m.i: [m.i - 1 if j == -1 else j % m.i for j in ([m.f] if isinstance(m.f, int) else m.f)] for m in rows if m.i > 0}
+    readers = {}
+    for i, js in src.items():
+        for j in js:
+            readers.setdefault(j, []).append(i)
+    dest, widths = {}, {}
+    for m in rows:
+        if isinstance(m, Concat) and m.d == 1:
+            widths[m.i] = [_row_channels(rows, j) for j in src[m.i]]
+            for k, j in enumerate(src[m.i]):
+                if readers[j] == [m.i] and isinstance(rows[j], (Conv, Upsample)):
+                    dest[j] = (m.i, sum(widths[m.i][:k]))
+    return dest, widths
+
+
+def _row_out_hw(m, x):
+    H, W = x.shape[2:]
+    if isinstance(m, Upsample):
+        return int(H * m.scale_factor), int(W * m.scale_factor)
+    c = m.conv
+    return tuple((n + 2 * c.padding[a] - c.dilation[a] * (c.kernel_size[a] - 1) - 1) // c.stride[a] + 1 for a, n in ((0, H), (1, W)))
+
+
 class _StaticPart(nn.Module):
 
     def __init__(self, model):
@@ -184,19 +220,29 @@
             counters = ops.begin_bn_counter_batch() if self.training else None
             y = []
             grouped_cast = self.autocast_dtype == torch.bfloat16 and x.is_cuda and torch.is_grad_enabled()
+            dest, widths = concat_plan(self.model[:-1]) if x.is_cuda and ops._CAT_INPLACE else ({}, {})
+            cat_maps = {}
             for m in self.model[:-1]:
                 if m.f != -1:
                     x = y[m.f] if isinstance(m.f, int) else [x if j == -1 else y[j] for j in m.f]
                 args = (x, txt) if isinstance(m, TIAGELAN) else (x,)
+                kw = {}
+                if m.i in dest:
+                    c, off = dest[m.i]
+                    if c not in cat_maps:
+                        cat_maps[c] = ops.cat_buffer(x, widths[c], _row_out_hw(m, x))
+                    kw = {'out': (cat_maps[c], off)}
+                elif m.i in cat_maps:
+                    kw = {'out': cat_maps.pop(m.i)}
                 names = _conv_weight_names(m) if grouped_cast else ()
                 if names:
                     masters = [m.get_parameter(n) for n in names]
                     w16 = _cast_group(masters)
                     for c, p in zip(w16, masters):
                         c._tamtr_master = p
-                    x = torch.func.functional_call(m, dict(zip(names, w16)), args)
+                    x = torch.func.functional_call(m, dict(zip(names, w16)), args, kw)
                 else:
-                    x = m(*args)
+                    x = m(*args, **kw)
                 y.append(x if m.i in self.save else None)
             feats, shapes = head.encode([y[j] for j in head.f], drop_scales)
             if counters is not None:
diff --git a/tam-tr_amd/modules.py b/tam-tr_amd/modules.py
--- a/tam-tr_amd/modules.py
+++ b/tam-tr_amd/modules.py
@@ -54,13 +54,13 @@
         self.attn = MaxSigmoidAttnBlock(c4, c4, nh=nh, ec=c4)
 
     def forward(self, x, guide):
-        y = self.branches(x)
+        y, buf = self.branches(x)
         if self.use_attn_output:
             y[-3] = self.attn(y[-3], guide)
         else:
             with torch.no_grad():
                 self.attn(y[-3].detach(), guide.detach())
-        return self.cv4(ops.cat_channels(y))
+        return self.cv4(ops.cat_channels(y, out=buf))
 
 
 class MLP(nn.Module):
diff --git a/tam-tr_amd/ops.py b/tam-tr_amd/ops.py
--- a/tam-tr_amd/ops.py
+++ b/tam-tr_amd/ops.py
@@ -65,44 +65,97 @@
     return _Relayout.apply(x, True) if (x.is_cuda and _cl_pitch(x)) else x.contiguous()
 
 
+_CAT_INPLACE = _os.environ.get('TAMTR_CAT_INPLACE', '1') != '0'
+
+
+def cat_buffer(x, widths, hw=None):
+    if not (_CAT_INPLACE and x.is_cuda and x.dim() == 4 and x.dtype in (torch.float32, torch.bfloat16) and _cl_pitch(x) and not x.is_contiguous()):
+        return None
+    v = 16 // x.element_size()
+    if any(w <= 0 or w % v for w in widths):
+        return None
+    H, W = hw if hw is not None else x.shape[2:]
+    return torch.empty((x.shape[0], sum(widths), H, W), dtype=x.dtype, device=x.device, memory_format=torch.channels_last)
+
+
+def _out_slot(out, N, C, dtype):
+    if out is None or out[0] is None:
+        return None
+    buf, off = out
+    B, ct, H, W = buf.shape
+    v = 16 // buf.element_size()
+    ok = (buf.dtype == dtype and B * H * W == N and 0 <= off and off + C <= ct and _is_cl(buf) and ct % v == 0 and C % v == 0
+          and (buf.data_ptr() + off * buf.element_size()) % 16 == 0)
+    return (buf, int(off)) if ok else None
+
+
+def _slot_rows(buf, off, C):
+    B, ct, H, W = buf.shape
+    return torch.empty(0, dtype=buf.dtype, device=buf.device).set_(buf.untyped_storage(), buf.storage_offset() + off, (B * H * W, C), (ct, 1))
+
+
+def _slot_map(buf, off, C):
+    B, ct, H, W = buf.shape
+    return torch.empty(0, dtype=buf.dtype, device=buf.device).set_(buf.untyped_storage(), buf.storage_offset() + off, (B, C, H, W),
+                                                                      (H * W * ct, 1, W * ct, ct))
+
+
+def cat_in_place(buf, maps):
+    B, ct, H, W = buf.shape
+    e, off, res = buf.element_size(), 0, []
+    for m in maps:
+        res.append(m.dtype == buf.dtype and m.device == buf.device and tuple(m.shape) == (B, m.shape[1], H, W) and _cl_pitch(m) == ct
+                   and m.data_ptr() == buf.data_ptr() + off * e)
+        off += m.shape[1]
+    return res if off == ct and _is_cl(buf) else [False] * len(maps)
+
+
 class _CatChannels(torch.autograd.Function):
 
     @staticmethod
-    def forward(ctx, *maps):
+    def forward(ctx, dest, *maps):
         B, _, H, W = maps[0].shape
         widths = [m.shape[1] for m in maps]
-        out = torch.empty((B, sum(widths), H, W), dtype=maps[0].dtype, device=maps[0].device, memory_format=torch.channels_last)
         ct, e, v = sum(widths), maps[0].element_size(), 16 // maps[0].element_size()
+        buf = dest[0] if dest is not None else None
+        if buf is not None and (tuple(buf.shape) != (B, ct, H, W) or buf.dtype != maps[0].dtype or buf.device != maps[0].device or not _is_cl(buf)):
+            buf = None
+        placed = cat_in_place(buf, maps) if buf is not None else [False] * len(maps)
+        out = _slot_map(buf, 0, ct) if buf is not None else torch.empty((B, ct, H, W), dtype=maps[0].dtype, device=maps[0].device,
+                                                                         memory_format=torch.channels_last)
         N = B * H * W
         pitches = [_cl_pitch(m) for m in maps]
-        if all(c % v == 0 and ld % v == 0 and m.data_ptr() % 16 == 0 for m, c, ld in zip(maps, widths, pitches)):
-            for i in range(0, len(maps), 4):
-                grp = list(range(i, min(i + 4, len(maps))))
+        offs = [sum(widths[:i]) for i in range(len(maps))]
+        todo = [i for i in range(len(maps)) if not placed[i]]
+        vec = ct % v == 0 and out.data_ptr() % 16 == 0 and all(c % v == 0 for c in widths)
+        if vec and all(pitches[i] % v == 0 and maps[i].data_ptr() % 16 == 0 for i in todo):
+            while todo:
+                grp = [todo.pop(0)]
+                while todo and len(grp) < 4 and todo[0] == grp[-1] + 1:
+                    grp.append(todo.pop(0))
                 n = len(grp)
                 src = (ctypes.c_void_p * n)(*[maps[j].data_ptr() for j in grp])
                 lds = (ctypes.c_longlong * n)(*[pitches[j] for j in grp])
                 cs = (ctypes.c_int * n)(*[widths[j] for j in grp])
                 call('tamtr_cat_rows', ctypes.cast(src, ctypes.c_void_p), ctypes.cast(lds, ctypes.c_void_p), ctypes.cast(cs, ctypes.c_void_p), n,
-                     out.data_ptr() + sum(widths[:i]) * e, ct, N, dtype_code(maps[0]), stream_ptr())
+                     out.data_ptr() + offs[grp[0]] * e, ct, N, dtype_code(maps[0]), stream_ptr())
         else:
-            off = 0
-            for m, c, ld in zip(maps, widths, pitches):
-                call('tamtr_copy_rows', ptr(m), ld, out.data_ptr() + off * e, ct, N, c, dtype_code(m), stream_ptr())
-                off += c
+            for i in todo:
+                call('tamtr_copy_rows', ptr(maps[i]), pitches[i], out.data_ptr() + offs[i] * e, ct, N, widths[i], dtype_code(maps[i]), stream_ptr())
         ctx.widths = widths
         return out
 
     @staticmethod
     def backward(ctx, g):
-        return tuple(g.split(ctx.widths, 1))
-
-
-def cat_channels(maps):
+        return (None,) + tuple(g.split(ctx.widths, 1))
+
+
+def cat_channels(maps, out=None):
     maps = list(maps)
     if len(maps) > 1 and all(m.is_cuda and m.dim() == 4 and m.dtype == maps[0].dtype and m.dtype in (torch.float32, torch.bfloat16)
                              and m.shape[0] == maps[0].shape[0] and m.shape[2:] == maps[0].shape[2:] and _cl_pitch(m) and not m.is_contiguous()
                              for m in maps):
-        return _CatChannels.apply(*maps)
+        return _CatChannels.apply(None if out is None else (out,), *maps)
     return torch.cat(maps, 1)
 
 
@@ -119,7 +172,8 @@
 
 
 def chunk2_channels(x):
-    if x.is_cuda and _is_cl(x) and x.shape[1] % 2 == 0 and x.dtype in (torch.float32, torch.bfloat16) and x.requires_grad:
+    if (x.is_cuda and x.dim() == 4 and _cl_pitch(x) and not x.is_contiguous() and x.shape[1] % 2 == 0 and x.dtype in (torch.float32, torch.bfloat16)
+            and x.requires_grad):
         return _ChunkChannels.apply(x)
     return x.chunk(2, 1)
 
@@ -147,13 +201,18 @@
 class _Resample2(torch.autograd.Function):
 
     @staticmethod
-    def forward(ctx, x, up):
+    def forward(ctx, x, up, out=None):
         B, C, H, W = x.shape
         ctx.cfg = (up, B, C, H, W)
         Ho, Wo = (2 * H, 2 * W) if up else (H // 2, W // 2)
-        out = torch.empty((B, C, Ho, Wo), dtype=x.dtype, device=x.device, memory_format=torch.channels_last)
-        call('tamtr_resample2', ptr(x), ptr(out), B, H, W, C, 0 if up else 2, dtype_code(x), stream_ptr())
-        return out
+        slot = _out_slot(out, B * Ho * Wo, C, x.dtype)
+        if slot is not None and tuple(slot[0].shape[2:]) == (Ho, Wo):
+            y = _slot_map(slot[0], slot[1], C)
+            call('tamtr_resample2_ld', ptr(x), ptr(y), slot[0].shape[1], B, H, W, C, 0 if up else 2, dtype_code(x), stream_ptr())
+            return y
+        y = torch.empty((B, C, Ho, Wo), dtype=x.dtype, device=x.device, memory_format=torch.channels_last)
+        call('tamtr_resample2', ptr(x), ptr(y), B, H, W, C, 0 if up else 2, dtype_code(x), stream_ptr())
+        return y
 
     @staticmethod
     def backward(ctx, g):
@@ -161,13 +220,13 @@
         g = g if _is_cl(g) else (pack_channels(g) if _cl_pitch(g) else g.contiguous(memory_format=torch.channels_last))
         gx = torch.empty((B, C, H, W), dtype=g.dtype, device=g.device, memory_format=torch.channels_last)
         call('tamtr_resample2', ptr(g), ptr(gx), B, H, W, C, 1 if up else 3, dtype_code(g), stream_ptr())
-        return gx, None
-
-
-def resample2(x, up):
+        return gx, None, None
+
+
+def resample2(x, up, out=None):
     v = 8 if x.dtype == torch.bfloat16 else 4
     if x.is_cuda and _is_cl(x) and x.dtype in (torch.float32, torch.bfloat16) and x.shape[1] % v == 0 and (up or (x.shape[2] % 2 == 0 and x.shape[3] % 2 == 0)):
-        return _Resample2.apply(x, bool(up))
+        return _Resample2.apply(x, bool(up), out)
     return None
 
 
@@ -180,17 +239,24 @@
 class _MaxPool(torch.autograd.Function):
 
     @staticmethod
-    def forward(ctx, x, k, s, p):
+    def forward(ctx, x, k, s, p, out=None):
         require_gpu(x)
-        nhwc = _is_cl(x)
+        ldx = 0 if x.is_contiguous() else _cl_pitch(x)
+        nhwc = bool(ldx)
         if not nhwc:
             x = _c(x)
         B, C, H, W = x.shape
         Ho, Wo = (H + 2 * p - k) // s + 1, (W + 2 * p - k) // s + 1
         fmt = torch.channels_last if nhwc else torch.contiguous_format
-        y = torch.empty((B, C, Ho, Wo), dtype=x.dtype, device=x.device, memory_format=fmt)
+        slot = _out_slot(out, B * Ho * Wo, C, x.dtype) if nhwc else None
+        if slot is not None and tuple(slot[0].shape[2:]) != (Ho, Wo):
+            slot = None
+        y = _slot_map(slot[0], slot[1], C) if slot is not None else torch.empty((B, C, Ho, Wo), dtype=x.dtype, device=x.device, memory_format=fmt)
         code = torch.empty((B, C, Ho, Wo), dtype=torch.uint8, device=x.device, memory_format=fmt)
-        call('tamtr_maxpool_fwd', ptr(x), ptr(y), ptr(code), B, C, H, W, k, s, p, int(nhwc), dtype_code(x), stream_ptr())
+        if nhwc and (ldx != C or slot is not None):
+            call('tamtr_maxpool_fwd_ld', ptr(x), ldx, ptr(y), _cl_pitch(y), ptr(code), B, C, H, W, k, s, p, dtype_code(x), stream_ptr())
+        else:
+            call('tamtr_maxpool_fwd', ptr(x), ptr(y), ptr(code), B, C, H, W, k, s, p, int(nhwc), dtype_code(x), stream_ptr())
         ctx.save_for_backward(code)
         ctx.cfg = (B, C, H, W, k, s, p, nhwc, x.dtype)
         return y
@@ -203,12 +269,12 @@
         gy = (pack_channels(gy) if _cl_pitch(gy) else gy.contiguous(memory_format=torch.channels_last)) if nhwc else _c(gy)
         gx = torch.empty((B, C, H, W), dtype=dt, device=gy.device, memory_format=torch.channels_last if nhwc else torch.contiguous_format)
         call('tamtr_maxpool_bwd', ptr(gy), ptr(code), None, ptr(gx), B, C, H, W, k, s, p, int(nhwc), dtype_code(gy), stream_ptr())
-        return gx, None, None, None
-
-
-def max_pool2d(x, k, s, p):
+        return gx, None, None, None, None
+
+
+def max_pool2d(x, k, s, p, out=None):
     if x.is_cuda and x.dim() == 4 and x.dtype in (torch.float32, torch.bfloat16) and k <= 15 and 2 * p <= k:
-        return _MaxPool.apply(x, int(k), int(s), int(p))
+        return _MaxPool.apply(x, int(k), int(s), int(p), out)
     return torch.nn.functional.max_pool2d(x, k, s, p)
 
 
@@ -1812,17 +1878,23 @@
 class _BNActCL(torch.autograd.Function):
 
     @staticmethod
-    def forward(ctx, x, gamma, beta, running_mean, running_var, eps, momentum, silu, residual=None):
+    def forward(ctx, x, gamma, beta, running_mean, running_var, eps, momentum, silu, residual=None, out=None):
         require_gpu(x, gamma, beta)
         x = _c(x)
         N, C = x.shape
         g32, b32 = _c(gamma.float()), _c(beta.float())
-        y = torch.empty_like(x)
         mr = torch.empty(C, 2, device=x.device, dtype=torch.float32)
         part = torch.empty(C * _lib.lib().tamtr_bncl_blocks(N, C, dtype_code(x)) * 3, device=x.device, dtype=torch.float32)
         res = None if residual is None else _c(residual.to(x.dtype))
-        call('tamtr_bncl_act_fwd', ptr(x), ptr(g32), ptr(b32), ptr(running_mean), ptr(running_var), ptr(res), ptr(y), ptr(mr), ptr(part), N, C,
-             float(eps), float(momentum), int(bool(silu)), dtype_code(x), stream_ptr())
+        slot = _out_slot(out, N, C, x.dtype) if C & (C - 1) == 0 else None
+        if slot is not None:
+            y = _slot_rows(slot[0], slot[1], C)
+            call('tamtr_bncl_act_ld_fwd', ptr(x), ptr(g32), ptr(b32), ptr(running_mean), ptr(running_var), ptr(res), ptr(y), y.stride(0), ptr(mr),
+                 ptr(part), N, C, float(eps), float(momentum), int(bool(silu)), dtype_code(x), stream_ptr())
+        else:
+            y = torch.empty_like(x)
+            call('tamtr_bncl_act_fwd', ptr(x), ptr(g32), ptr(b32), ptr(running_mean), ptr(running_var), ptr(res), ptr(y), ptr(mr), ptr(part), N, C,
+                 float(eps), float(momentum), int(bool(silu)), dtype_code(x), stream_ptr())
         ctx.save_for_backward(x, g32, b32, mr)
         ctx.cfg = (int(bool(silu)), gamma.dtype, beta.dtype, None if residual is None else residual.dtype)
         return y
@@ -1839,7 +1911,7 @@
         part = torch.empty(C * _lib.lib().tamtr_bncl_blocks(N, C, dtype_code(x)) * 2 + 2 * C, device=x.device, dtype=torch.float32)
         call('tamtr_bncl_act_bwd', ptr(gy), gy.stride(0), ptr(x), ptr(g32), ptr(b32), ptr(mr), ptr(gx), ptr(gg), ptr(gb), ptr(part), N, C, act,
              dtype_code(x), stream_ptr())
-        return gx, gg.to(g_dt), gb.to(b_dt), None, None, None, None, None, g_res
+        return gx, gg.to(g_dt), gb.to(b_dt), None, None, None, None, None, g_res, None
 
 
 def _gy_rows(gy, x):
@@ -1854,16 +1926,22 @@
 class _BN2ActCL(torch.autograd.Function):
 
     @staticmethod
-    def forward(ctx, x1, ga1, be1, rm1, rv1, x2, ga2, be2, rm2, rv2, eps, momentum, silu):
+    def forward(ctx, x1, ga1, be1, rm1, rv1, x2, ga2, be2, rm2, rv2, eps, momentum, silu, out=None):
         require_gpu(x1, x2, ga1, ga2)
         x1, x2 = _c(x1), _c(x2)
         N, C = x1.shape
         p1 = [_c(t.float()) for t in (ga1, be1, ga2, be2)]
-        y = torch.empty_like(x1)
         mr = torch.empty(2, C, 2, device=x1.device, dtype=torch.float32)
         part = torch.empty(2 * C * _lib.lib().tamtr_bncl_blocks(N, C, dtype_code(x1)) * 3, device=x1.device, dtype=torch.float32)
-        call('tamtr_bncl2_act_fwd', ptr(x1), ptr(p1[0]), ptr(p1[1]), ptr(rm1), ptr(rv1), ptr(x2), ptr(p1[2]), ptr(p1[3]), ptr(rm2), ptr(rv2),
-             ptr(y), ptr(mr), ptr(part), N, C, float(eps), float(momentum), int(bool(silu)), dtype_code(x1), stream_ptr())
+        slot = _out_slot(out, N, C, x1.dtype) if C & (C - 1) == 0 else None
+        if slot is not None:
+            y = _slot_rows(slot[0], slot[1], C)
+            call('tamtr_bncl2_act_ld_fwd', ptr(x1), ptr(p1[0]), ptr(p1[1]), ptr(rm1), ptr(rv1), ptr(x2), ptr(p1[2]), ptr(p1[3]), ptr(rm2), ptr(rv2),
+                 ptr(y), y.stride(0), ptr(mr), ptr(part), N, C, float(eps), float(momentum), int(bool(silu)), dtype_code(x1), stream_ptr())
+        else:
+            y = torch.empty_like(x1)
+            call('tamtr_bncl2_act_fwd', ptr(x1), ptr(p1[0]), ptr(p1[1]), ptr(rm1), ptr(rv1), ptr(x2), ptr(p1[2]), ptr(p1[3]), ptr(rm2), ptr(rv2),
+                 ptr(y), ptr(mr), ptr(part), N, C, float(eps), float(momentum), int(bool(silu)), dtype_code(x1), stream_ptr())
         ctx.save_for_backward(x1, x2, *p1, mr)
         ctx.cfg = (int(bool(silu)), ga1.dtype, be1.dtype, ga2.dtype, be2.dtype)
         return y
@@ -1879,7 +1957,7 @@
         part = torch.empty(C * _lib.lib().tamtr_bncl_blocks(N, C, dtype_code(x1)) * 3 + 3 * C, device=x1.device, dtype=torch.float32)
         call('tamtr_bncl2_act_bwd', ptr(gy), gy.stride(0), ptr(x1), ptr(x2), ptr(g1), ptr(b1), ptr(g2), ptr(b2), ptr(mr), ptr(gx1), ptr(gx2),
              gg[0].data_ptr(), gg[1].data_ptr(), gg[2].data_ptr(), gg[3].data_ptr(), ptr(part), N, C, act, dtype_code(x1), stream_ptr())
-        return (gx1, gg[0].to(dt_g1), gg[1].to(dt_b1), None, None, gx2, gg[2].to(dt_g2), gg[3].to(dt_b2), None, None, None, None, None)
+        return (gx1, gg[0].to(dt_g1), gg[1].to(dt_b1), None, None, gx2, gg[2].to(dt_g2), gg[3].to(dt_b2), None, None, None, None, None, None)
 
 
 class _BNCatCL(torch.autograd.Function):
@@ -1972,19 +2050,19 @@
     return bn.momentum if bn.momentum is not None else 1.0 / float(bn.num_batches_tracked)
 
 
-def bn_act(x, bn, silu, residual=None):
+def bn_act(x, bn, silu, residual=None, out=None):
     mom = _bn_tick(bn)
     rm, rv = (bn.running_mean, bn.running_var) if bn.track_running_stats else (None, None)
     if x.dim() == 2:
-        return _BNActCL.apply(x, bn.weight, bn.bias, rm, rv, bn.eps, mom, silu, residual)
+        return _BNActCL.apply(x, bn.weight, bn.bias, rm, rv, bn.eps, mom, silu, residual, out)
     y = _BNAct.apply(x, bn.weight, bn.bias, rm, rv, bn.eps, mom, silu)
     return y if residual is None else y + residual
 
 
-def bn2_act(x1, bn1, x2, bn2, silu):
+def bn2_act(x1, bn1, x2, bn2, silu, out=None):
     if bn1.eps != bn2.eps or bn1.momentum != bn2.momentum or not (bn1.track_running_stats and bn2.track_running_stats):
         raise _lib.TamtrHipError('bn2_act: the two BatchNorms must share eps / momentum and track running statistics')
     mom = _bn_tick(bn1)
     _bn_tick(bn2)
     return _BN2ActCL.apply(x1, bn1.weight, bn1.bias, bn1.running_mean, bn1.running_var, x2, bn2.weight, bn2.bias, bn2.running_mean,
-                           bn2.running_var, bn1.eps, mom, silu)
+                           bn2.running_var, bn1.eps, mom, silu, out)
```

Measured after the change: 216.9, median of 6. No clear change (+1.0%).
